# succinctlabs/kzg-rs

Hardware: NVIDIA B200
Metric: blobs verified/sec (verify_blob_kzg_proof_batch) (higher is better)
Workload: dtype u32-limb modular integer (Fr 255-bit / Fp 381-bit) + SHA-256

## Files before the change

include/kzgb200.h:

```cpp
#ifndef KZGB200_H
#define KZGB200_H
#include <stddef.h>
#include <stdint.h>
#ifdef __cplusplus
extern "C" {
#endif

#define KZGB200_OK 0
#define KZGB200_BAD_ARGS 1
#define KZGB200_INTERNAL_ERROR 2
#define KZGB200_INVALID_LENGTH 3
#define KZGB200_INVALID_SETUP 5

#define KZGB200_BYTES_PER_BLOB 131072
#define KZGB200_BYTES_PER_COMMITMENT 48
#define KZGB200_BYTES_PER_PROOF 48
#define KZGB200_BYTES_PER_FIELD_ELEMENT 32
#define KZGB200_PARTIAL_BYTES 352

typedef struct kzgb200_ctx kzgb200_ctx;

int kzgb200_create(kzgb200_ctx** out, int device, const uint8_t* g2_points, size_t g2_points_len);
void kzgb200_destroy(kzgb200_ctx* ctx);
const char* kzgb200_last_error(const kzgb200_ctx* ctx);

int kzgb200_verify_kzg_proof(kzgb200_ctx* ctx, const uint8_t* commitment48, const uint8_t* z32, const uint8_t* y32,
                             const uint8_t* proof48, int* ok);

int kzgb200_verify_blob_kzg_proof(kzgb200_ctx* ctx, const uint8_t* blob, const uint8_t* commitment48,
                                  const uint8_t* proof48, int* ok, uint8_t* z_out, uint8_t* y_out);

int kzgb200_verify_blob_kzg_proof_batch(kzgb200_ctx* ctx, const uint8_t* blobs, size_t n_blobs,
                                        const uint8_t* commitments, size_t n_commitments,
                                        const uint8_t* proofs, size_t n_proofs, int* ok,
                                        uint8_t* z_out, uint8_t* y_out);
int kzgb200_verify_blob_kzg_proof_batch_device(kzgb200_ctx* ctx, const uint8_t* d_blobs, const uint8_t* d_commitments,
                                               const uint8_t* d_proofs, size_t n, int* ok,
                                               uint8_t* d_z_out, uint8_t* d_y_out);

int kzgb200_verify_kzg_proof_many(kzgb200_ctx* ctx, const uint8_t* commitments, const uint8_t* zs, const uint8_t* ys,
                                  const uint8_t* proofs, size_t m, uint8_t* verdicts);

int kzgb200_verify_kzg_proof_batch(kzgb200_ctx* ctx, const uint8_t* commitments104, const uint8_t* zs32, const uint8_t* ys32,
                                   const uint8_t* proofs104, size_t n, int* ok);

int kzgb200_verify_blob_kzg_proof_batch_each(kzgb200_ctx* ctx, const uint8_t* blobs, const uint8_t* commitments, const uint8_t* proofs,
                                             size_t n, uint8_t* verdicts, uint8_t* z_out, uint8_t* y_out);

int kzgb200_compute_challenge(kzgb200_ctx* ctx, const uint8_t* blob, const uint8_t* commitment48, uint8_t* z_out32);
int kzgb200_evaluate_polynomial_in_evaluation_form(kzgb200_ctx* ctx, const uint8_t* blob, const uint8_t* z32, uint8_t* y_out32);

typedef struct kzgb200_group kzgb200_group;
int kzgb200_group_create(kzgb200_group** out, const int* device_ids, int n_devices, const uint8_t* g2_points, size_t g2_points_len,
                         size_t max_blobs_per_device);
int kzgb200_group_join(kzgb200_group** out, const char* session, int rank, int world, int device, const uint8_t* g2_points,
                       size_t g2_points_len, size_t max_blobs_per_rank);
void kzgb200_group_destroy(kzgb200_group* g);
int kzgb200_group_size(const kzgb200_group* g);
int kzgb200_group_local_members(const kzgb200_group* g);
kzgb200_ctx* kzgb200_group_context(kzgb200_group* g, int local_index);
const char* kzgb200_group_last_error(const kzgb200_group* g);
int kzgb200_group_uses_peer_stores(const kzgb200_group* g, int local_index);
int kzgb200_group_verify_blob_kzg_proof_batch(kzgb200_group* g, const uint8_t* blobs, size_t n_blobs, const uint8_t* commitments,
                                              size_t n_commitments, const uint8_t* proofs, size_t n_proofs, int* ok, uint8_t* z_out,
                                              uint8_t* y_out);
int kzgb200_group_verify_shards(kzgb200_group* g, const uint8_t* const* blobs, const uint8_t* const* commitments,
                                const uint8_t* const* proofs, const size_t* n_local, int device_pointers, int* ok,
                                uint8_t* const* z_out, uint8_t* const* y_out);
int kzgb200_group_last_partials(kzgb200_group* g, uint8_t* out, size_t n_ranks);
int kzgb200_group_host_protocol_test(const char* session, int rank, int world, const uint8_t* commitments, const uint8_t* zy,
                                     const uint8_t* proofs, size_t n_local, size_t chunk, uint8_t* digest_out32);

#define KZGB200_TRANSCRIPT_EXACT 0
#define KZGB200_TRANSCRIPT_TREE 1
#define KZGB200_TRANSCRIPT_EXACT_DEVICE 2
int kzgb200_set_transcript_mode(kzgb200_ctx* ctx, int mode);
int kzgb200_last_r(kzgb200_ctx* ctx, uint8_t* r_out32);
int kzgb200_host_sha256(const uint8_t* msg, size_t len, uint8_t* out32, int force_portable);

int kzgb200_last_partial(kzgb200_ctx* ctx, uint8_t* out352);

int kzgb200_harness_generate(kzgb200_ctx* ctx, uint64_t seed, size_t n, int degree, const uint8_t* tau_powers48,
                             uint8_t* d_blobs, uint8_t* d_commitments, uint8_t* d_proofs);
int kzgb200_load_g1_lagrange(kzgb200_ctx* ctx, const uint8_t* g1_lagrange, size_t n_points);
int kzgb200_blob_to_kzg_commitment_batch(kzgb200_ctx* ctx, const uint8_t* d_blobs, size_t n, uint8_t* d_commitments_out);
int kzgb200_compute_blob_kzg_proof_batch(kzgb200_ctx* ctx, const uint8_t* d_blobs, const uint8_t* d_commitments, size_t n,
                                         uint8_t* d_proofs_out);

int kzgb200_load_cell_setup(kzgb200_ctx* ctx, const uint8_t* g1_monomial48, size_t n_points, const uint8_t* g2_tau64_96);
int kzgb200_verify_cell_kzg_proof_batch(kzgb200_ctx* ctx, const uint8_t* commitments, const uint64_t* cell_indices, const uint8_t* cells,
                                        const uint8_t* proofs, size_t n, int* ok);
int kzgb200_verify_cell_kzg_proof_batch_device(kzgb200_ctx* ctx, const uint8_t* d_commitments, const uint64_t* d_cell_indices,
                                               const uint8_t* d_cells, const uint8_t* d_proofs, size_t n, int* ok);
int kzgb200_compute_cells(kzgb200_ctx* ctx, const uint8_t* blob, uint8_t* cells_out);
int kzgb200_compute_cells_batch_device(kzgb200_ctx* ctx, const uint8_t* d_blobs, size_t n, uint8_t* d_cells);
int kzgb200_harness_generate_cells(kzgb200_ctx* ctx, uint64_t seed, size_t n_blobs, int degree, const uint8_t* tau_powers48,
                                   uint8_t* d_cells, uint8_t* d_commitments, uint8_t* d_proofs);

int kzgb200_load_cell_proof_setup(kzgb200_ctx* ctx, const uint8_t* g1_lagrange48, size_t n_points);
int kzgb200_cell_proof_monomial(kzgb200_ctx* ctx, uint8_t* out48, size_t n_points);
int kzgb200_compute_cells_and_kzg_proofs(kzgb200_ctx* ctx, const uint8_t* blob, uint8_t* cells_out, uint8_t* proofs_out);
int kzgb200_compute_cells_and_kzg_proofs_batch_device(kzgb200_ctx* ctx, const uint8_t* d_blobs, size_t n, uint8_t* d_cells, uint8_t* d_proofs);
int kzgb200_recover_cells_and_kzg_proofs(kzgb200_ctx* ctx, const uint64_t* cell_indices, const uint8_t* cells, size_t n_cells,
                                         uint8_t* cells_out, uint8_t* proofs_out);
int kzgb200_recover_cells_and_kzg_proofs_batch_device(kzgb200_ctx* ctx, const uint64_t* cell_indices, size_t n_cells, const uint8_t* d_cells,
                                                      size_t n_blobs, uint8_t* d_cells_out, uint8_t* d_proofs_out);

int kzgb200_set_profiling(kzgb200_ctx* ctx, int on);
int kzgb200_set_slab_tail(kzgb200_ctx* ctx, int on);
int kzgb200_get_phase_ms(kzgb200_ctx* ctx, float* out8);
int kzgb200_debug_final_ticks(kzgb200_ctx* ctx, long long* out14);
int kzgb200_debug_engine_selftest(kzgb200_ctx* ctx, uint32_t seed, int rounds, uint32_t* mismatches32, int* n_programs);
void* kzgb200_stream(kzgb200_ctx* ctx);

typedef struct kzgb200_pipeline kzgb200_pipeline;
int kzgb200_pipeline_create(kzgb200_pipeline** out, int device, const uint8_t* g2_points, size_t g2_points_len, int depth);
void kzgb200_pipeline_destroy(kzgb200_pipeline* p);
int kzgb200_pipeline_depth(const kzgb200_pipeline* p);
kzgb200_ctx* kzgb200_pipeline_context(kzgb200_pipeline* p, int slot);
int kzgb200_pipeline_submit(kzgb200_pipeline* p, const uint8_t* blobs, size_t n_blobs, const uint8_t* commitments,
                            size_t n_commitments, const uint8_t* proofs, size_t n_proofs, uint8_t* z_out, uint8_t* y_out,
                            uint64_t* ticket);
int kzgb200_pipeline_submit_device(kzgb200_pipeline* p, const uint8_t* d_blobs, const uint8_t* d_commitments,
                                   const uint8_t* d_proofs, size_t n, uint8_t* d_z_out, uint8_t* d_y_out, uint64_t* ticket);
int kzgb200_pipeline_wait(kzgb200_pipeline* p, uint64_t ticket, int* ok);

void* kzgb200_alloc_pinned(size_t bytes);
void kzgb200_free_pinned(void* p);

#ifdef __cplusplus
}
#endif
#endif
```

kzg_rs_b200/csrc/common.cuh:

```cuda
#pragma once
#include <cuda_runtime.h>
#include "sha256.cuh"
#include "verify.cuh"
#include "vliw.cuh"
#include "vliw29.cuh"
#include "glv.cuh"

namespace kzgb200 {

constexpr int kFieldElementsPerBlob = 4096;
constexpr int kBytesPerBlob = 4096 * 32;
constexpr uint32_t kErrBlob = 1, kErrCommitment = 2, kErrProof = 4, kErrScalar = 8;
struct ZY { Fr z, y; };

struct DeviceTables {
    Fr twiddle[2048];
    Fr twiddle_po[128][32];
    PairingTables pairing;
    vliw29::LineCoeffs29 lines29[2][kMillerSteps];
    G1Affine gen_table[64][15];
    uint32_t setup_ok;
};

#ifndef KSHA_THREADS
#define KSHA_THREADS 32
#endif
constexpr int kShaThreads = KSHA_THREADS;
constexpr int kEvalThreads = 128;
constexpr int kLeavesPerThread = kFieldElementsPerBlob / kEvalThreads;
constexpr int kTreeGroup = 16;
constexpr int kTreeMid = 32;
constexpr int kWindows = 16, kBuckets = 256, kMsmSets = 3, kDigitRows = 4 * kWindows;
constexpr int kMinSlice = 8, kMsmRows = kMsmSets * 2 * kWindows;
constexpr int kWinLanes = kBuckets;
constexpr int kWinSmemBytes = kWinLanes * 144;
constexpr int kCombineThreads = 544;
constexpr int kCombineSmemBytes = 48 * 1024;
constexpr int kFinalThreads = 64;
constexpr int kPairThreads = 768;
constexpr int kManyThreads = 512, kManyGroups = 28;
constexpr int kManyCtasPerSm = 1;
constexpr int kManyWarps = 4;
constexpr int kHarnessMaxDegree = 16;
constexpr int kLagWindows = 32, kLagEntries = 255;
constexpr int kCellsPerExtBlob = 128, kFieldElementsPerCell = 64, kBytesPerCell = 2048;
constexpr int kCellNttThreads = 512;
constexpr int kCellNttSmemBytes = kFieldElementsPerBlob * 32;
constexpr int kCellAggSlices = 16;
constexpr int kCellHarnessMaxDegree = 192;

__device__ __forceinline__ Fr load_fe_be(const uint4* p) {
    uint4 hi = __ldg(p), lo = __ldg(p + 1);
    Fr f;
    f.l[7] = sha_bswap(hi.x); f.l[6] = sha_bswap(hi.y); f.l[5] = sha_bswap(hi.z); f.l[4] = sha_bswap(hi.w);
    f.l[3] = sha_bswap(lo.x); f.l[2] = sha_bswap(lo.y); f.l[1] = sha_bswap(lo.z); f.l[0] = sha_bswap(lo.w);
    return f;
}
__device__ __forceinline__ Fr ldg_fr(const Fr* p) {
    const uint4* q = reinterpret_cast<const uint4*>(p);
    uint4 a = __ldg(q), b = __ldg(q + 1);
    Fr f;
    f.l[0] = a.x; f.l[1] = a.y; f.l[2] = a.z; f.l[3] = a.w; f.l[4] = b.x; f.l[5] = b.y; f.l[6] = b.z; f.l[7] = b.w;
    return f;
}

struct Partial {
    G1 a, b;
    Fr ry;
    uint32_t err;
    uint32_t pad[7];
};

struct FinalSmem {
    G1 sm[kFinalThreads];
    unsigned char pad[20 * 1024];
};
struct PairSmem {
    f29::F29 regs[vliw29::kTotalRegs];
    vliw29::SharedTables stab;
};
struct FinalPts { G1Affine pts[2]; uint32_t go; };

constexpr int kManyStride = vliw::kTotalRegsThr * 12 + 1;
constexpr int kManySmemBytes = kManyGroups * kManyStride * 4 + (int)sizeof(vliw::SharedTables) + vliw::kNumSharedRegs * (int)sizeof(Fp) +
                               kManyGroups * (2 * (int)sizeof(G1Affine) + 2) + 64;
struct CellTables {
    Fr w4096[2048], w4096_inv[2048];
    Fr coset[4096];
    Fr shift64[kCellsPerExtBlob];
    Fr shift_inv[kCellsPerExtBlob];
    Fr w64_inv[kFieldElementsPerCell / 2];
    Fr omega8192, inv64;
    G1Affine tau_tab[kFieldElementsPerCell][4];
    LineCoeffs tau64_lines[kMillerSteps];
    vliw29::LineCoeffs29 lines29[kMillerSteps];
    uint32_t ok;
};
constexpr int kFk20Bases = kFieldElementsPerCell * kCellsPerExtBlob;
constexpr int kFk20Windows = 16, kFk20Entries = 255;
constexpr size_t kFk20TablePoints = (size_t)kFk20Bases * kFk20Windows * kFk20Entries;
constexpr int kExtElements = 2 * kFieldElementsPerBlob;
struct ProofTables {
    Fr w8192[kFieldElementsPerBlob], w8192_inv[kFieldElementsPerBlob];
    Fr pow7[kExtElements];
    Fr pow7_inv[kFieldElementsPerBlob];
    Fr s7_64;
};
__global__ void setup_tables_kernel(DeviceTables* T, const uint8_t* g2_points);
__global__ void setup_lines29_kernel(DeviceTables* T);
constexpr int kChallengeSlabs = 8;
void launch_challenge(int stages, cudaStream_t st, const uint8_t* blobs, const uint8_t* commitments, int n, Fr* z_mont, ZY* zy, Fr* zpow,
                      const uint8_t* slab_flags = nullptr);
__global__ void eval_kernel(const uint8_t* __restrict__ blobs, int n, const Fr* __restrict__ zpow, const DeviceTables* __restrict__ T,
                            ZY* __restrict__ zy, uint32_t* __restrict__ status);
__global__ void g1_decompress_kernel(const uint8_t* __restrict__ commitments, const uint8_t* __restrict__ proofs, int n, G1Affine* __restrict__ C,
                                     G1Affine* __restrict__ P, uint32_t* __restrict__ status, bool with_subgroup_check);
__global__ void g1_subgroup_kernel(const G1Affine* __restrict__ C, const G1Affine* __restrict__ P, int n, uint32_t* __restrict__ status);
__global__ void transcript_schedule_kernel(const uint8_t* __restrict__ commitments, const ZY* __restrict__ zy, const uint8_t* __restrict__ proofs,
                                           uint64_t n, uint32_t* __restrict__ wk, uint64_t first_blk, uint64_t blk_count);
__global__ void transcript_chain_kernel(const uint32_t* __restrict__ wk_all, uint64_t n, Fr* __restrict__ r_mont, uint32_t* __restrict__ state,
                                        uint64_t first_blk, uint64_t blk_count);
__global__ void transcript_words_kernel(const uint8_t* __restrict__ commitments, const ZY* __restrict__ zy, const uint8_t* __restrict__ proofs,
                                        uint64_t first_entry, uint64_t entry_count, uint32_t* __restrict__ words);
__global__ void transcript_tree_leaf_words_kernel(const uint32_t* __restrict__ words, uint64_t n, uint32_t* __restrict__ digests,
                                                  uint64_t first_group, uint64_t group_count);
__global__ void r_from_digest_kernel(const uint32_t* __restrict__ digest, Fr* __restrict__ r_mont);
__global__ void z_setup_kernel(const uint8_t* __restrict__ z_be32, int n, Fr* __restrict__ z_mont, ZY* __restrict__ zy, Fr* __restrict__ zpow,
                               uint32_t* __restrict__ status);
__global__ void import_parsed_kernel(const uint8_t* __restrict__ c104, const uint8_t* __restrict__ p104, const uint8_t* __restrict__ z32,
                                     const uint8_t* __restrict__ y32, int n, G1Affine* __restrict__ C, G1Affine* __restrict__ P,
                                     uint8_t* __restrict__ c48, uint8_t* __restrict__ p48, Fr* __restrict__ z_mont, ZY* __restrict__ zy);
__global__ void msm_scalars_kernel(const Fr* __restrict__ z_mont, const ZY* __restrict__ zy, const Fr* __restrict__ r_mont, uint64_t offset, int n,
                                   uint8_t* __restrict__ digits, Fr* __restrict__ ry);
__global__ void msm_sort_kernel(const uint8_t* __restrict__ digits, int n, uint32_t* __restrict__ order, uint32_t* __restrict__ start);
void launch_msm_bucket(int ctas_per_sm, int n, int slice, cudaStream_t st, const G1Affine* C, const G1Affine* P, const uint32_t* order,
                       const uint32_t* start, G1* halfsum, G1* part);
void launch_msm_bucket_join(int lanes, int n, int slice, cudaStream_t st, const uint32_t* start, const G1* halfsum, const G1* part, G1* buckets);
__global__ void msm_window_kernel(const G1* __restrict__ buckets, G1* __restrict__ windows);
__global__ void msm_combine_kernel(const G1* __restrict__ windows, const Fr* __restrict__ ry, const uint32_t* __restrict__ status, int n,
                                   const DeviceTables* __restrict__ T, Partial* __restrict__ out, uint32_t* flag, uint32_t epoch);
__global__ void wait_flags_kernel(const uint32_t* flags, int count, uint32_t epoch, uint32_t* __restrict__ timed_out);
__global__ void batch_final_kernel(const Partial* __restrict__ parts, int nparts, const DeviceTables* __restrict__ T, uint32_t* __restrict__ result,
                                   FinalPts* __restrict__ out);
__global__ void single_final_kernel(const G1Affine* __restrict__ C, const G1Affine* __restrict__ P, const ZY* __restrict__ zy,
                                    const uint32_t* __restrict__ status, const DeviceTables* __restrict__ T, uint32_t* __restrict__ result,
                                    FinalPts* __restrict__ out);
__global__ void pairing_check_kernel(const FinalPts* __restrict__ in, const DeviceTables* __restrict__ T, const vliw29::LineCoeffs29* __restrict__ lines_b,
                                     uint32_t* __restrict__ result, long long* __restrict__ ticks);
__global__ void engine_selftest_kernel(uint32_t seed, int rounds, f29::F29* __restrict__ ref, uint32_t* __restrict__ mismatches);
inline void launch_batch_final(cudaStream_t st, const Partial* parts, int nparts, const DeviceTables* T, uint32_t* result, unsigned char* scratch512,
                               bool ticks, const vliw29::LineCoeffs29* lines_b = nullptr) {
    FinalPts* fp = reinterpret_cast<FinalPts*>(scratch512 + 256);
    batch_final_kernel<<<1, kFinalThreads, sizeof(FinalSmem), st>>>(parts, nparts, T, result, fp);
    pairing_check_kernel<<<1, kPairThreads, sizeof(PairSmem), st>>>(fp, T, lines_b, result, ticks ? reinterpret_cast<long long*>(scratch512 + 128) : nullptr);
}
__global__ void many_lhs_kernel(const uint8_t* __restrict__ z32, const uint8_t* __restrict__ y32, const G1Affine* __restrict__ C,
                                const G1Affine* __restrict__ P, size_t m, const DeviceTables* __restrict__ T, G1Affine* __restrict__ X,
                                uint32_t* __restrict__ status);
__global__ void many_lhs_zy_kernel(const ZY* __restrict__ zy, const G1Affine* __restrict__ C, const G1Affine* __restrict__ P, size_t m,
                                   const DeviceTables* __restrict__ T, G1Affine* __restrict__ X, const uint32_t* __restrict__ status);
__global__ void many_pairing_kernel(const G1Affine* __restrict__ X, const G1Affine* __restrict__ P, const uint32_t* __restrict__ status, size_t m,
                                    const DeviceTables* __restrict__ T, uint8_t* __restrict__ verdicts);
__global__ void many_pairing_warp_kernel(const G1Affine* __restrict__ X, const G1Affine* __restrict__ P, size_t m, const DeviceTables* __restrict__ T,
                                         uint8_t* __restrict__ verdicts);
__global__ void export_scalars_kernel(const ZY* __restrict__ zy, int n, uint8_t* __restrict__ z_out, uint8_t* __restrict__ y_out);
__global__ void r_to_raw_kernel(const Fr* __restrict__ r_mont, ZY* __restrict__ out);
__global__ void status_or_kernel(const uint32_t* __restrict__ status, int n, uint32_t* __restrict__ out);
__global__ void harness_parse_points_kernel(const uint8_t* bytes, int n, G1Affine* out, uint32_t* bad);
__global__ void harness_blob_kernel(uint64_t seed, int n, int D, const DeviceTables* __restrict__ T, uint8_t* __restrict__ blobs);
__global__ void harness_commit_kernel(uint64_t seed, int n, int D, const G1Affine* __restrict__ M, const Fr* __restrict__ z_mont,
                                      uint8_t* __restrict__ out, int want_proof);
__global__ void lag_parse_kernel(const uint8_t* __restrict__ bytes, G1Affine* __restrict__ out, uint32_t* __restrict__ bad);
__global__ void lag_table_kernel(const G1Affine* __restrict__ L, G1* __restrict__ table);
__global__ void blob_scalars_kernel(const uint8_t* __restrict__ blobs, int n, Fr* __restrict__ scalars, uint32_t* __restrict__ status);
__global__ void quotient_kernel(const uint8_t* __restrict__ blobs, int n, const Fr* __restrict__ z_mont, const ZY* __restrict__ zy,
                                const DeviceTables* __restrict__ T, Fr* __restrict__ scalars);
__global__ void lag_msm_kernel(const Fr* __restrict__ scalars, int n, const G1* __restrict__ table, uint8_t* __restrict__ out48);
__global__ void cell_setup_kernel(CellTables* T, const uint8_t* __restrict__ g2_tau64);
__global__ void cell_setup_points_kernel(CellTables* T, const uint8_t* __restrict__ g1_monomial48);
__global__ void cell_setup_lines29_kernel(CellTables* T);
__global__ void compute_cells_kernel(const uint8_t* __restrict__ blobs, int n, const CellTables* __restrict__ T, uint8_t* __restrict__ cells,
                                     uint32_t* __restrict__ status);
__global__ void compute_cells_coeffs_kernel(const uint8_t* __restrict__ blobs, int n, const CellTables* __restrict__ T, uint8_t* __restrict__ cells,
                                            uint32_t* __restrict__ status, Fr* __restrict__ coeffs);
__global__ void proof_setup_kernel(ProofTables* P);
__global__ void mono_load_kernel(const uint8_t* __restrict__ lag48, G1* __restrict__ a, uint32_t* __restrict__ bad);
__global__ void mono_level_kernel(G1* __restrict__ a, int len, const CellTables* __restrict__ T);
__global__ void mono_finish_kernel(const G1* __restrict__ a, const CellTables* __restrict__ T, G1Affine* __restrict__ mono, uint32_t* __restrict__ bad);
__global__ void mono_compress_kernel(const G1Affine* __restrict__ mono, int n, uint8_t* __restrict__ out48);
__global__ void fk20_w_kernel(const G1Affine* __restrict__ mono, const CellTables* __restrict__ T, G1Affine* __restrict__ W);
__global__ void fk20_table_kernel(const G1Affine* __restrict__ W, G1Affine* __restrict__ tab);
__global__ void fk20_scalars_kernel(const Fr* __restrict__ coeffs, const CellTables* __restrict__ T, Fr* __restrict__ U);
__global__ void fk20_products_kernel(const Fr* __restrict__ U, const G1Affine* __restrict__ tab, G1* __restrict__ V);
__global__ void fk20_proofs_kernel(const G1* __restrict__ V, const CellTables* __restrict__ T, uint8_t* __restrict__ proofs);
__global__ void recover_z_kernel(const uint32_t* __restrict__ missing, int n_missing, const CellTables* __restrict__ T, const ProofTables* __restrict__ P,
                                 Fr* __restrict__ zvals);
__global__ void recover_load_kernel(const uint8_t* __restrict__ cells, int n_cells, const int* __restrict__ pos, const Fr* __restrict__ zvals, int nb,
                                    Fr* __restrict__ A, uint32_t* __restrict__ status);
__global__ void recover_ntt_inv_kernel(Fr* __restrict__ A, const CellTables* __restrict__ T);
__global__ void recover_ntt_div_kernel(Fr* __restrict__ A, const CellTables* __restrict__ T, const Fr* __restrict__ zvals);
__global__ void recover_mid_kernel(Fr* __restrict__ A, const ProofTables* __restrict__ P, int nb);
__global__ void recover_final_kernel(const Fr* __restrict__ A, const ProofTables* __restrict__ P, int nb, Fr* __restrict__ coeffs);
__global__ void recover_blob_kernel(const Fr* __restrict__ coeffs, const CellTables* __restrict__ T, uint8_t* __restrict__ blobs);
__global__ void cell_points_kernel(const uint8_t* __restrict__ bytes, int count, G1Affine* __restrict__ out, uint32_t* __restrict__ status, uint32_t flag);
__global__ void cell_check_kernel(const uint8_t* __restrict__ cells, int n, uint32_t* __restrict__ status);
__global__ void cell_scalars_kernel(const uint32_t* __restrict__ meta, int n, const G1Affine* __restrict__ U, const uint32_t* __restrict__ ustatus,
                                    const CellTables* __restrict__ T, Fr* __restrict__ z_mont, ZY* __restrict__ zy, G1Affine* __restrict__ C,
                                    uint32_t* __restrict__ status);
__global__ void cell_rpow_kernel(const Fr* __restrict__ r_mont, int n, Fr* __restrict__ rk);
__global__ void cell_agg_kernel(const uint8_t* __restrict__ cells, const uint32_t* __restrict__ meta, int n, const Fr* __restrict__ rk, Fr* __restrict__ agg);
__global__ void cell_interp_kernel(const Fr* __restrict__ agg, const uint32_t* __restrict__ meta, int n, const CellTables* __restrict__ T,
                                   Fr* __restrict__ coeffs);
__global__ void cell_rli_kernel(const Fr* __restrict__ coeffs, const CellTables* __restrict__ T, Partial* __restrict__ out);
__global__ void cell_harness_terms_kernel(uint64_t seed, int n, int D, const G1Affine* __restrict__ M, G1* __restrict__ terms);
__global__ void cell_harness_sums_kernel(int n, const G1* __restrict__ terms, G1* __restrict__ sums);
__global__ void cell_harness_points_kernel(int n, const G1* __restrict__ sums, const CellTables* __restrict__ T, uint8_t* __restrict__ commitments,
                                           uint8_t* __restrict__ proofs);
__global__ void cell_harness_eval_kernel(uint64_t seed, int n, int D, const CellTables* __restrict__ T, uint8_t* __restrict__ cells);

}
```

kzg_rs_b200/csrc/k_msm.cu:

```cuda
#include "common.cuh"
#include "coop.cuh"

namespace kzgb200 {

__global__ void __launch_bounds__(128) msm_scalars_kernel(const Fr* __restrict__ z_mont, const ZY* __restrict__ zy, const Fr* __restrict__ r_mont,
                                                          uint64_t offset, int n, uint8_t* __restrict__ digits ,
                                                          Fr* __restrict__ ry) {
    int i = blockIdx.x * blockDim.x + threadIdx.x;
    if (i >= n) return;
    uint64_t e = offset + (uint64_t)i;
    uint32_t ee[2] = {(uint32_t)e, (uint32_t)(e >> 32)};
    Fr ri = r_mont->pow(ee, 64);
    Fr ri_raw = ri.to_raw();
    Fr rz_raw = (ri * z_mont[i]).to_raw();
    ry[i] = ri * zy[i].y;
    uint32_t h[2][2][4];
    glv_split(ri_raw.l, h[0][0], h[0][1]);
    glv_split(rz_raw.l, h[1][0], h[1][1]);
    for (int kind = 0; kind < 2; kind++)
        for (int half = 0; half < 2; half++)
            for (int w = 0; w < kWindows; w++)
                digits[((size_t)(kind * 2 + half) * kWindows + w) * n + i] = (uint8_t)(h[kind][half][w >> 2] >> (8 * (w & 3)));
}
__global__ void __launch_bounds__(256) msm_sort_kernel(const uint8_t* __restrict__ digits, int n, uint32_t* __restrict__ order,
                                                       uint32_t* __restrict__ start) {
    __shared__ uint32_t hist[kBuckets], cursor[kBuckets];
    int row_id = blockIdx.x, t = threadIdx.x;
    const uint8_t* row = digits + (size_t)row_id * n;
    uint32_t* ord = order + (size_t)row_id * n;
    uint32_t* st = start + (size_t)row_id * (kBuckets + 1);
    hist[t] = 0;
    __syncthreads();
    for (int i = t; i < n; i += blockDim.x) atomicAdd(&hist[row[i]], 1u);
    __syncthreads();
    if (t == 0) {
        uint32_t acc = 0;
        for (int b = 0; b < kBuckets; b++) { cursor[b] = acc; st[b] = acc; acc += hist[b]; }
        st[kBuckets] = acc;
    }
    __syncthreads();
    for (int i = t; i < n; i += blockDim.x) ord[atomicAdd(&cursor[row[i]], 1u)] = (uint32_t)i;
}
__device__ __forceinline__ G1Affine ldg_point(const G1Affine* p) {
    const uint32_t* w = reinterpret_cast<const uint32_t*>(p);
    G1Affine a;
#pragma unroll
    for (int k = 0; k < 12; k++) { a.x.l[k] = __ldg(w + k); a.y.l[k] = __ldg(w + 12 + k); }
    a.inf = __ldg(w + 24);
    return a;
}
template <int kCtasPerSm>
__global__ void __launch_bounds__(128, kCtasPerSm) msm_bucket_kernel(const G1Affine* __restrict__ C, const G1Affine* __restrict__ P, int n,
                                                         const uint32_t* __restrict__ order, const uint32_t* __restrict__ start,
                                                         G1* __restrict__ halfsum , G1* __restrict__ part , int slice) {
    const int slices = (n + slice - 1) / slice;
    int tid = blockIdx.x * blockDim.x + threadIdx.x;
    if (tid >= kMsmRows * slices) return;
    int row = tid / slices, s = tid % slices;
    int w = row % kWindows, half = (row / kWindows) & 1, set = row / (2 * kWindows);
    const G1Affine* pts = set == 1 ? C : P;
    int digit_row = ((set == 2 ? 1 : 0) * 2 + half) * kWindows + w;
    const uint32_t* ord = order + (size_t)digit_row * n;
    const uint32_t* st = start + (size_t)digit_row * (kBuckets + 1);
    const uint32_t pos0 = (uint32_t)s * slice, end0 = pos0 + slice < (uint32_t)n ? pos0 + slice : (uint32_t)n;
    int b = 0;
#pragma unroll
    for (int step = 128; step >= 1; step >>= 1) if (b + step <= 255 && __ldg(st + b + step) <= pos0) b += step;
    uint32_t next_boundary = __ldg(st + b + 1);
    G1 acc = G1::identity();
    bool first = true;
    auto flush = [&](int bb) {
        uint32_t lo = __ldg(st + bb), hi = __ldg(st + bb + 1);
        if (bb != 0 && hi > lo) {
            if (lo >= pos0 && hi <= end0) halfsum[(size_t)row * kBuckets + bb] = acc;
            else part[((size_t)row * slices + s) * 2 + (first ? 0 : 1)] = acc;
        }
        first = false;
        acc = G1::identity();
    };
    const uint32_t beta_l[12] = KZG_FP_BETA_M;
    const Fp beta = fp_const(beta_l);
    G1Affine nxt = ldg_point(pts + __ldg(ord + pos0));
    for (uint32_t k = pos0; k < end0; k++) {
        G1Affine q = nxt;
        if (k + 1 < end0) nxt = ldg_point(pts + __ldg(ord + k + 1));
        while (k >= next_boundary) { flush(b); b++; next_boundary = __ldg(st + b + 1); }
        if (b != 0) {
            if (half && !q.inf) { q.x = q.x * beta; q.y = q.y.neg(); }
            acc = acc.add_mixed(q);
        }
    }
    flush(b);
}
void launch_msm_bucket(int ctas_per_sm, int n, int slice, cudaStream_t st, const G1Affine* C, const G1Affine* P, const uint32_t* order,
                       const uint32_t* start, G1* halfsum, G1* part) {
    const int slices = (n + slice - 1) / slice, grid = (kMsmRows * slices + 127) / 128;
    if (ctas_per_sm >= 4) msm_bucket_kernel<4><<<grid, 128, 0, st>>>(C, P, n, order, start, halfsum, part, slice);
    else if (ctas_per_sm == 3) msm_bucket_kernel<3><<<grid, 128, 0, st>>>(C, P, n, order, start, halfsum, part, slice);
    else msm_bucket_kernel<2><<<grid, 128, 0, st>>>(C, P, n, order, start, halfsum, part, slice);
}
__device__ __forceinline__ G1 shfl_xor_point(const G1& p, int m) {
    G1 r;
#pragma unroll
    for (int k = 0; k < 12; k++) {
        r.x.l[k] = __shfl_xor_sync(0xffffffffu, p.x.l[k], m);
        r.y.l[k] = __shfl_xor_sync(0xffffffffu, p.y.l[k], m);
        r.z.l[k] = __shfl_xor_sync(0xffffffffu, p.z.l[k], m);
    }
    return r;
}
template <int kJoinLanes>
__global__ void __launch_bounds__(128) msm_bucket_join_kernel(int n, const uint32_t* __restrict__ start, const G1* __restrict__ halfsum,
                                                              const G1* __restrict__ part, G1* __restrict__ buckets , int slice) {
    const int slices = (n + slice - 1) / slice;
    const uint32_t usl = (uint32_t)slice;
    const int gt = blockIdx.x * blockDim.x + threadIdx.x;
    const int tid = gt / kJoinLanes, j = gt % kJoinLanes;
    int b = tid % kBuckets, w = (tid / kBuckets) % kWindows, set = tid / (kBuckets * kWindows);
    G1 acc = G1::identity();
    if (b != 0) {
        uint32_t lo[2], s0[2], cnt[2];
        int row[2];
#pragma unroll
        for (int half = 0; half < 2; half++) {
            row[half] = (set * 2 + half) * kWindows + w;
            const int digit_row = ((set == 2 ? 1 : 0) * 2 + half) * kWindows + w;
            const uint32_t* st = start + (size_t)digit_row * (kBuckets + 1);
            const uint32_t l = __ldg(st + b), h = __ldg(st + b + 1);
            lo[half] = l; s0[half] = l / usl;
            cnt[half] = h > l ? (h - 1) / usl - l / usl + 1 : 0u;
        }
        const uint32_t total = cnt[0] + cnt[1];
        for (uint32_t i = (uint32_t)j; i < total; i += kJoinLanes) {
            const int half = i >= cnt[0] ? 1 : 0;
            const uint32_t k = half ? i - cnt[0] : i;
            const G1* src;
            if (cnt[half] == 1) src = halfsum + (size_t)row[half] * kBuckets + b;
            else {
                const uint32_t s = s0[half] + k;
                const int slot = (k == 0 && lo[half] != s0[half] * usl) ? 1 : 0;
                src = part + ((size_t)row[half] * slices + s) * 2 + slot;
            }
            acc = acc.add(*src);
        }
    }
#pragma unroll 1
    for (int m = 1; m < kJoinLanes; m <<= 1) {
        const G1 o = shfl_xor_point(acc, m);
        if ((j & (2 * m - 1)) == 0) acc = acc.add(o);
    }
    if (j == 0) buckets[tid] = acc;
}
void launch_msm_bucket_join(int lanes, int n, int slice, cudaStream_t st, const uint32_t* start, const G1* halfsum, const G1* part, G1* buckets) {
    const int items = kMsmSets * kWindows * kBuckets;
    if (lanes >= 8) msm_bucket_join_kernel<8><<<items * 8 / 128, 128, 0, st>>>(n, start, halfsum, part, buckets, slice);
    else if (lanes >= 4) msm_bucket_join_kernel<4><<<items * 4 / 128, 128, 0, st>>>(n, start, halfsum, part, buckets, slice);
    else msm_bucket_join_kernel<2><<<items * 2 / 128, 128, 0, st>>>(n, start, halfsum, part, buckets, slice);
}
static_assert(sizeof(G1) * kWinLanes == kWinSmemBytes, "keep kWinSmemBytes (common.cuh) in step with G1");
__global__ void __launch_bounds__(kWinLanes) msm_window_kernel(const G1* __restrict__ buckets, G1* __restrict__ windows ) {
    extern __shared__ __align__(16) unsigned char dyn_smem[];
    G1* sm = reinterpret_cast<G1*>(dyn_smem);
    const int l = threadIdx.x, sw = blockIdx.x;
    G1 mine = buckets[(size_t)sw * kBuckets + l];
#pragma unroll 1
    for (int d = 1; d < kWinLanes; d <<= 1) {
        sm[l] = mine;
        __syncthreads();
        if (l + d < kWinLanes) mine = mine.add(sm[l + d]);
        __syncthreads();
    }
    sm[l] = l ? mine : G1::identity();
    __syncthreads();
#pragma unroll 1
    for (int span = kWinLanes / 2; span >= 1; span >>= 1) {
        if (l < span) sm[l] = sm[l].add(sm[l + span]);
        __syncthreads();
    }
    if (l == 0) windows[sw] = sm[0];
}
constexpr int kCombEngine = 384, kCombHelpers = 160;
constexpr int kCombRegs = 96;
static_assert(kCombEngine + kCombHelpers == kCombineThreads, "thread split of msm_combine_kernel");
struct CombineSmem {
    f29::F29 regs[kMsmSets][kCombRegs];
    f29::F29 win[kMsmSets][kWindows][3];
    vliw29::SharedTables stab;
};
static_assert(sizeof(CombineSmem) <= kCombineSmemBytes, "keep kCombineSmemBytes (common.cuh) in step with CombineSmem");
__global__ void __launch_bounds__(kCombineThreads) msm_combine_kernel(const G1* __restrict__ windows, const Fr* __restrict__ ry, const uint32_t* __restrict__ status,
                                                                      int n, const DeviceTables* __restrict__ T, Partial* __restrict__ out, uint32_t* flag, uint32_t epoch) {
    extern __shared__ __align__(16) unsigned char dyn_smem[];
    CombineSmem& S = *reinterpret_cast<CombineSmem*>(dyn_smem);
    __shared__ uint32_t s_err, s_fallback;
    __shared__ uint8_t s_wid[kMsmSets][kWindows];
    __shared__ Fr s_ry[kCombHelpers];
    __shared__ CoopPoint cp[3];
    __shared__ G1 s_sg[64];
    const int t = threadIdx.x;
    if (t == 0) { s_err = 0; s_fallback = 0; }
    __syncthreads();
    if (t < kCombEngine) {
        auto ebar = [] { asm volatile("bar.sync 2, %0;" ::"n"(kCombEngine) : "memory"); };
        {
            const vliw29::Tables src = vliw29::default_tables();
            for (int i = t; i < vliw29::kNumMul * 4; i += kCombEngine) (&S.stab.mul[0][0])[i] = (&src.mul[0][0])[i];
            for (int i = t; i < vliw29::kNumLin * 4; i += kCombEngine) (&S.stab.lin[0][0])[i] = (&src.lin[0][0])[i];
            for (int i = t; i < vliw29::kNumTerm; i += kCombEngine) S.stab.term[i] = src.term[i];
            for (int i = t; i < vliw29::kNumLevel; i += kCombEngine) S.stab.level[i] = src.level[i];
            for (int i = t; i < vliw29::kNumPrograms; i += kCombEngine) S.stab.prog[i] = src.prog[i];
            if (t < 16) S.stab.p29[t] = t < 14 ? (int32_t)f29::p29_rt(t) : 0;
        }
        for (int i = t; i < kMsmSets * kWindows * 3; i += kCombEngine) {
            const int sw = i / 3, c = i % 3;
            const G1& w = windows[sw];
            S.win[sw / kWindows][sw % kWindows][c] = f29::from_fp(c == 0 ? w.x : (c == 1 ? w.y : w.z));
            if (c == 2) s_wid[sw / kWindows][sw % kWindows] = w.z.is_zero() ? 1 : 0;
        }
        for (int i = t; i < kMsmSets * kCombRegs; i += kCombEngine) S.regs[i / kCombRegs][i % kCombRegs] = f29::f29_zero();
        ebar();
        vliw29::Lanes L{t, kCombEngine, vliw29::Tables{S.stab.mul, S.stab.lin, S.stab.term, S.stab.level, S.stab.prog}, nullptr, S.stab.p29};
        L.groups = kMsmSets; L.gstride = kCombRegs; L.bar_id = 2; L.bar_threads = kCombEngine;
        f29::F29* regs = &S.regs[0][0];
        bool acc_id[kMsmSets] = {true, true, true};
        for (int w = kWindows - 1; w >= 0; w--) {
            if (w != kWindows - 1) for (int k = 0; k < 8; k++) vliw29::run(vliw29::kProg_g1_dbl, regs, L);
            for (int i = t; i < kMsmSets * 3 * 4; i += kCombEngine) {
                const int g = i / 12, c = (i / 4) % 3, q = i % 4;
                reinterpret_cast<uint4*>(&S.regs[g][3 + c])[q] = reinterpret_cast<const uint4*>(&S.win[g][w][c])[q];
                reinterpret_cast<uint4*>(&S.regs[g][90 + c])[q] = reinterpret_cast<const uint4*>(&S.regs[g][c])[q];
            }
            ebar();
            vliw29::run(vliw29::kProg_g1_add, regs, L);
            for (int i = t; i < kMsmSets * 3 * 4; i += kCombEngine) {
                const int g = i / 12, c = (i / 4) % 3, q = i % 4;
                if (s_wid[g][w]) reinterpret_cast<uint4*>(&S.regs[g][c])[q] = reinterpret_cast<const uint4*>(&S.regs[g][90 + c])[q];
                else if (acc_id[g]) reinterpret_cast<uint4*>(&S.regs[g][c])[q] = reinterpret_cast<const uint4*>(&S.regs[g][3 + c])[q];
            }
            if (t < kMsmSets && !s_wid[t][w] && !acc_id[t]) {
                if (vliw29::canonical_signed(S.regs[t][6]).is_zero()) s_fallback = 1;
            }
#pragma unroll
            for (int g = 0; g < kMsmSets; g++) acc_id[g] = acc_id[g] && s_wid[g][w];
            ebar();
        }
        if (t < kMsmSets * 3) {
            const int g = t / 3, c = t % 3;
            Fp v = Fp::from_raw(vliw29::canonical_signed(S.regs[g][c]));
            if (acc_id[g]) v = c == 2 ? Fp::zero() : Fp::one();
            cp[g].v[c] = v;
        }
        ebar();
        if (s_fallback && t < 32 * kMsmSets) {
            const int warp = t >> 5, lane = t & 31;
            CoopPoint* s = &cp[warp];
            __syncwarp();
            if (lane == 0) { s->v[0] = Fp::one(); s->v[1] = Fp::one(); s->v[2] = Fp::zero(); }
            __syncwarp();
            for (int w = kWindows - 1; w >= 0; w--) {
                if (w != kWindows - 1) for (int k = 0; k < 8; k++) coop_dbl(s, lane);
                coop_add(s, windows[warp * kWindows + w], lane);
            }
        }
    } else {
        const int h = t - kCombEngine;
        uint32_t e = 0;
        Fr acc_ry = Fr::zero();
        for (int i = h; i < n; i += kCombHelpers) { e |= status[i]; acc_ry = acc_ry.add_inl(ry[i]); }
        if (e) atomicOr(&s_err, e);
        s_ry[h] = acc_ry;
        asm volatile("bar.sync 1, %0;" ::"n"(kCombHelpers) : "memory");
        for (int span = 128; span >= 1; span >>= 1) {
            if (h < span && h + span < kCombHelpers) s_ry[h] = s_ry[h].add_inl(s_ry[h + span]);
            asm volatile("bar.sync 1, %0;" ::"n"(kCombHelpers) : "memory");
        }
        if (h < 64) {
            const Fr sv = s_ry[0];
            const uint32_t d = (sv.l[h / 8] >> (4 * (h % 8))) & 15u;
            s_sg[h] = d ? G1::from_affine(T->gen_table[h][d - 1]) : G1::identity();
        }
        asm volatile("bar.sync 1, %0;" ::"n"(kCombHelpers) : "memory");
        for (int span = 32; span >= 1; span >>= 1) {
            if (h < span) s_sg[h] = s_sg[h].add(s_sg[h + span]);
            asm volatile("bar.sync 1, %0;" ::"n"(kCombHelpers) : "memory");
        }
    }
    __syncthreads();
    const int warp = t >> 5, lane = t & 31;
    if (warp == 1) {
        G1 q = {cp[2].v[0], cp[2].v[1], cp[2].v[2]};
        coop_add(&cp[1], q, lane);
        coop_add(&cp[1], s_sg[0].neg(), lane);
    }
    if (warp < 2 && lane == 0) { G1 r = {cp[warp].v[0], cp[warp].v[1], cp[warp].v[2]}; if (warp == 1) out->b = r; else out->a = r; }
    if (t == 0) { out->ry = Fr::zero(); out->err = s_err; }
    if (flag) {
        __threadfence_system();
        __syncthreads();
        if (t == 0) { *reinterpret_cast<volatile uint32_t*>(flag) = epoch; __threadfence_system(); }
    }
}

}
```

kzg_rs_b200/csrc/kzgb200.cu:

```cuda
#include <new>
#include "runtime.cuh"

using namespace kzgb200;

namespace kzgb200 {
CopyPool::CopyPool(int nthreads) {
    for (int i = 0; i < nthreads; i++) threads.emplace_back([this] {
        uint64_t seen = 0;
        for (;;) {
            {
                std::unique_lock<std::mutex> lk(m);
                cv.wait(lk, [&] { return stop || gen != seen; });
                if (stop) return;
                seen = gen;
            }
            work(seen);
        }
    });
}
CopyPool::~CopyPool() {
    { std::lock_guard<std::mutex> lk(m); stop = true; }
    cv.notify_all();
    for (auto& t : threads) t.join();
}
bool CopyPool::grab(size_t* off, size_t* len) {
    std::lock_guard<std::mutex> lk(m);
    if (next >= pieces) return false;
    *off = next++ * piece;
    *len = bytes - *off < piece ? bytes - *off : piece;
    return true;
}
void CopyPool::work(uint64_t) {
    size_t off, len, mine = 0;
    while (grab(&off, &len)) { memcpy(dst + off, src + off, len); mine++; }
    if (mine) {
        std::lock_guard<std::mutex> lk(m);
        done += mine;
        if (done == pieces) cv_done.notify_all();
    }
}
void CopyPool::copy(uint8_t* d, const uint8_t* s, size_t n) {
    if (!n) return;
    {
        std::lock_guard<std::mutex> lk(m);
        dst = d; src = s; bytes = n; pieces = (n + piece - 1) / piece; next = 0; done = 0; gen++;
    }
    cv.notify_all();
    work(0);
    std::unique_lock<std::mutex> lk(m);
    cv_done.wait(lk, [&] { return done == pieces; });
}

void phase_begin(kzgb200_ctx* ctx, int ph, cudaStream_t st) { if (ctx->profile && !ctx->ph_started[ph]) { cudaEventRecord(ctx->ev_s[ph], st); ctx->ph_started[ph] = true; } }
void phase_end(kzgb200_ctx* ctx, int ph, cudaStream_t st) { if (ctx->profile) cudaEventRecord(ctx->ev_e[ph], st); }
void collect_phase_times(kzgb200_ctx* ctx) {
    if (!ctx->profile) return;
    cudaDeviceSynchronize();
    for (int i = 0; i < 8; i++) { ctx->phase_ms[i] = 0; if (ctx->ph_started[i]) cudaEventElapsedTime(&ctx->phase_ms[i], ctx->ev_s[i], ctx->ev_e[i]); }
}

int ensure_capacity(kzgb200_ctx* ctx, size_t n, bool need_blob_staging) {
    if (n > ctx->cap) {
        size_t c = n;
        CK(regrow(ctx->d_c, c * 48)); CK(regrow(ctx->d_p, c * 48));
        CK(regrow(ctx->d_z_mont, c)); CK(regrow(ctx->d_zy, c)); CK(regrow(ctx->d_zpow, c * 13));
        CK(regrow(ctx->d_C, c)); CK(regrow(ctx->d_P, c));
        CK(regrow(ctx->d_status, c)); CK(regrow(ctx->d_ry, c));
        CK(regrow(ctx->d_digits, c * kDigitRows)); CK(regrow(ctx->d_order, c * kDigitRows));
        CK(regrow(ctx->d_zout, c * 32)); CK(regrow(ctx->d_yout, c * 32));
        CK(regrow(ctx->d_part, (size_t)kMsmRows * ((c + kMinSlice - 1) / kMinSlice) * 2));
        ctx->cap = c;
    }
    if (n > ctx->host_cap) {
        for (uint8_t** p : {&ctx->h_zy, &ctx->h_c, &ctx->h_p}) { if (*p) cudaFreeHost(*p); *p = nullptr; }
        CK(cudaMallocHost(&ctx->h_zy, n * 64)); CK(cudaMallocHost(&ctx->h_c, n * 48)); CK(cudaMallocHost(&ctx->h_p, n * 48));
        ctx->host_cap = n;
    }
    if (need_blob_staging && n > ctx->blob_cap) {
        CK(regrow(ctx->d_blobs, n * (size_t)kBytesPerBlob));
        ctx->blob_cap = n;
    }
    return KZGB200_OK;
}

void hash_transcript_header(HostSha256* s, uint64_t n) {
    uint8_t hdr[32] = {'R', 'C', 'K', 'Z', 'G', 'B', 'A', 'T', 'C', 'H', '_', '_', '_', 'V', '1', '_', 0, 0, 0, 0, 0, 0, 0x10, 0x00};
    for (int i = 0; i < 8; i++) hdr[24 + i] = (uint8_t)(n >> (56 - 8 * i));
    host_sha256_init(s);
    host_sha256_update(s, hdr, 32);
}
void hash_entries(HostSha256* s, const uint8_t* c, const uint8_t* zy, const uint8_t* p, size_t lo, size_t cnt) {
    uint8_t buf[64 * 160];
    for (size_t i = lo; i < lo + cnt;) {
        size_t m = lo + cnt - i < 64 ? lo + cnt - i : 64;
        for (size_t k = 0; k < m; k++, i++) {
            uint8_t* e = buf + 160 * k;
            memcpy(e, c + 48 * i, 48);
            memcpy(e + 48, zy + 64 * i, 64);
            memcpy(e + 112, p + 48 * i, 48);
        }
        host_sha256_update(s, buf, 160 * m);
    }
}
static size_t tree_groups(size_t n) { return (n + kTreeGroup - 1) / kTreeGroup; }
static int transcript_begin(kzgb200_ctx* ctx, size_t n, const uint8_t* d_c, const uint8_t* d_p, const uint8_t* hc, const uint8_t* hp) {
    ctx->tr_n = n; ctx->tr_done = 0; ctx->tr_next_chunk = 0; ctx->tr_enqueued = 0; ctx->tr_active = true;
    ctx->tr_c = hc; ctx->tr_p = hp;
    const int mode = ctx->transcript_mode;
    size_t words = 0;
    if (mode == KZGB200_TRANSCRIPT_TREE) words = n * 40 + tree_groups(n) * 8;
    else if (mode == KZGB200_TRANSCRIPT_EXACT_DEVICE) words = ((32 + n * 160 + 9 + 63) / 64) * 64;
    if (words > ctx->wk_cap) { CK(regrow(ctx->d_wk, words)); ctx->wk_cap = words; }
    if (mode == KZGB200_TRANSCRIPT_EXACT_DEVICE) return KZGB200_OK;
    hash_transcript_header(&ctx->tr_sha, n);
    if (mode == KZGB200_TRANSCRIPT_EXACT && !hc) {
        CK(cudaStreamWaitEvent(ctx->s_d2h, ctx->ev_begin, 0));
        CK(cudaMemcpyAsync(ctx->h_c, d_c, n * 48, cudaMemcpyDeviceToHost, ctx->s_d2h));
        CK(cudaMemcpyAsync(ctx->h_p, d_p, n * 48, cudaMemcpyDeviceToHost, ctx->s_d2h));
        ctx->tr_c = ctx->h_c; ctx->tr_p = ctx->h_p;
    }
    return KZGB200_OK;
}
static int transcript_enqueue_chunk(kzgb200_ctx* ctx, int c, const uint8_t* d_c, const uint8_t* d_p) {
    const size_t n = ctx->tr_n, lo = ctx->chunks[c].lo, cnt = ctx->chunks[c].cnt, end = lo + cnt;
    switch (ctx->transcript_mode) {
    case KZGB200_TRANSCRIPT_EXACT:
        CK(cudaStreamWaitEvent(ctx->s_d2h, ctx->ev_zy[c], 0));
        CK(cudaMemcpyAsync(ctx->h_zy + lo * 64, ctx->d_zy + lo, cnt * 64, cudaMemcpyDeviceToHost, ctx->s_d2h));
        CK(cudaEventRecord(ctx->ev_zyh[c], ctx->s_d2h));
        break;
    case KZGB200_TRANSCRIPT_TREE: {
        size_t g0 = lo / kTreeGroup, g1 = end >= n ? tree_groups(n) : end / kTreeGroup;
        uint32_t *words = ctx->d_wk, *digests = ctx->d_wk + n * 40;
        transcript_words_kernel<<<(unsigned)((cnt * 40 + 255) / 256), 256, 0, ctx->stream>>>(d_c, ctx->d_zy, d_p, lo, cnt, words);
        if (g1 > g0) transcript_tree_leaf_words_kernel<<<(unsigned)((g1 - g0 + 63) / 64), 64, 0, ctx->stream>>>(words, (uint64_t)n, digests, g0, g1 - g0);
        CK(cudaEventRecord(ctx->ev_leaf, ctx->stream));
        CK(cudaStreamWaitEvent(ctx->s_d2h, ctx->ev_leaf, 0));
        if (g1 > g0) CK(cudaMemcpyAsync(ctx->h_zy + g0 * 32, digests + g0 * 8, (g1 - g0) * 32, cudaMemcpyDeviceToHost, ctx->s_d2h));
        CK(cudaEventRecord(ctx->ev_zyh[c], ctx->s_d2h));
        break;
    }
    default: {
        size_t nblk = (32 + n * 160 + 9 + 63) / 64;
        size_t ready = end >= n ? nblk : (32 + end * 160) / 64;
        if (ready > ctx->tr_done) {
            size_t k = ready - ctx->tr_done;
            transcript_schedule_kernel<<<(unsigned)((k + 127) / 128), 128, 0, ctx->stream>>>(d_c, ctx->d_zy, d_p, (uint64_t)n, ctx->d_wk, ctx->tr_done, k);
            transcript_chain_kernel<<<1, 32, 0, ctx->stream>>>(ctx->d_wk, (uint64_t)n, ctx->d_r, ctx->d_chain_state, ctx->tr_done, k);
            ctx->tr_done = ready;
        }
    }
    }
    CK(cudaGetLastError());
    ctx->tr_enqueued = c + 1;
    return KZGB200_OK;
}
int transcript_progress(kzgb200_ctx* ctx, bool block) {
    if (!ctx->tr_active) return KZGB200_OK;
    if (ctx->transcript_mode == KZGB200_TRANSCRIPT_EXACT_DEVICE) { ctx->tr_next_chunk = ctx->tr_enqueued; return KZGB200_OK; }
    while (ctx->tr_next_chunk < ctx->tr_enqueued) {
        int c = ctx->tr_next_chunk;
        if (block) CK(cudaEventSynchronize(ctx->ev_zyh[c]));
        else {
            cudaError_t e = cudaEventQuery(ctx->ev_zyh[c]);
            if (e == cudaErrorNotReady) break;
            CK(e);
        }
        size_t lo = ctx->chunks[c].lo, cnt = ctx->chunks[c].cnt, end = lo + cnt;
        if (ctx->chunk_sink) ctx->chunk_sink(ctx->chunk_sink_arg, c);
        else if (ctx->transcript_mode == KZGB200_TRANSCRIPT_EXACT) hash_entries(&ctx->tr_sha, ctx->tr_c, ctx->h_zy, ctx->tr_p, lo, cnt);
        else {
            size_t g0 = lo / kTreeGroup, g1 = end >= ctx->tr_n ? tree_groups(ctx->tr_n) : end / kTreeGroup;
            host_sha256_update(&ctx->tr_sha, ctx->h_zy + g0 * 32, (g1 - g0) * 32);
        }
        ctx->tr_next_chunk++;
    }
    return KZGB200_OK;
}
int upload_r_digest(kzgb200_ctx* ctx, const uint8_t digest[32]) {
    memcpy(ctx->h_digest, digest, 32);
    CK(cudaMemcpyAsync(ctx->d_digest, ctx->h_digest, 32, cudaMemcpyHostToDevice, ctx->stream));
    r_from_digest_kernel<<<1, 1, 0, ctx->stream>>>(ctx->d_digest, ctx->d_r);
    CK(cudaGetLastError());
    return KZGB200_OK;
}
int transcript_finish(kzgb200_ctx* ctx) {
    if (ctx->transcript_mode != KZGB200_TRANSCRIPT_EXACT_DEVICE) {
        uint8_t digest[32];
        host_sha256_final(&ctx->tr_sha, digest);
        int rc = upload_r_digest(ctx, digest);
        if (rc) return rc;
    }
    phase_end(ctx, kPhTranscript, ctx->stream);
    ctx->tr_active = false;
    return KZGB200_OK;
}

static int plan_chunks(kzgb200_ctx* ctx, size_t n, bool host_blobs, bool transcript) {
    int k = 0;
    if (host_blobs) {
        size_t chunk = (n + kMaxChunks - 1) / kMaxChunks;
        if (chunk < kMinChunk) chunk = kMinChunk;
        chunk = (chunk + kTreeGroup - 1) / kTreeGroup * kTreeGroup;
        for (size_t lo = 0; lo < n; lo += chunk) ctx->chunks[k++] = {lo, n - lo < chunk ? n - lo : chunk};
    } else if (!transcript || n < 2048 || ctx->transcript_mode == KZGB200_TRANSCRIPT_TREE) {
        ctx->chunks[k++] = {0, n};
    } else if (ctx->transcript_mode == KZGB200_TRANSCRIPT_EXACT_DEVICE) {
        size_t chunk = ((n + 7) / 8 + kTreeGroup - 1) / kTreeGroup * kTreeGroup;
        for (size_t lo = 0; lo < n; lo += chunk) ctx->chunks[k++] = {lo, n - lo < chunk ? n - lo : chunk};
    } else {
        size_t lo = 0, quarter = n / 4 / kTreeGroup * kTreeGroup;
        while (lo < n) {
            size_t rem = n - lo, take = k < 3 ? quarter : rem / 2 / kTreeGroup * kTreeGroup;
            if (take < 256) take = 256;
            if (rem - (take < rem ? take : rem) < 256 || k == kMaxChunks - 1) take = rem;
            ctx->chunks[k++] = {lo, take};
            lo += take;
        }
    }
    ctx->nchunks = k;
    return k;
}
static bool host_pointer_is_pinned(const void* p) {
    cudaPointerAttributes a;
    if (cudaPointerGetAttributes(&a, p) != cudaSuccess) { cudaGetLastError(); return false; }
    return a.type == cudaMemoryTypeHost;
}
static int h2d_blobs(kzgb200_ctx* ctx, uint8_t* d_dst, const uint8_t* h_src, size_t bytes, bool direct) {
    if (direct) { CK(cudaMemcpyAsync(d_dst, h_src, bytes, cudaMemcpyHostToDevice, ctx->s_copy)); return KZGB200_OK; }
    if (!ctx->pool) {
        unsigned hw = std::thread::hardware_concurrency();
        int t = hw >= 16 ? 7 : (hw >= 8 ? 3 : 1);
        if (const char* v = getenv("KZGB200_COPY_THREADS")) t = atoi(v) > 0 ? atoi(v) - 1 : 0;
        ctx->pool = new CopyPool(t);
        for (int b = 0; b < kzgb200_ctx::kStageBufs; b++) {
            CK(cudaMallocHost(&ctx->h_stage[b], kzgb200_ctx::kStageBytes));
            CK(cudaEventCreateWithFlags(&ctx->ev_stage[b], cudaEventDisableTiming));
        }
    }
    for (size_t off = 0; off < bytes; off += kzgb200_ctx::kStageBytes) {
        size_t len = bytes - off < kzgb200_ctx::kStageBytes ? bytes - off : kzgb200_ctx::kStageBytes;
        int b = ctx->stage_next;
        ctx->stage_next = (b + 1) % kzgb200_ctx::kStageBufs;
        CK(cudaEventSynchronize(ctx->ev_stage[b]));
        ctx->pool->copy(ctx->h_stage[b], h_src + off, len);
        CK(cudaMemcpyAsync(d_dst + off, ctx->h_stage[b], len, cudaMemcpyHostToDevice, ctx->s_copy));
        CK(cudaEventRecord(ctx->ev_stage[b], ctx->s_copy));
        int rc = transcript_progress(ctx, false);
        if (rc) return rc;
    }
    return KZGB200_OK;
}
int launch_phase1(kzgb200_ctx* ctx, const uint8_t* d_blobs, const uint8_t* h_blobs, const uint8_t* d_c, const uint8_t* d_p, size_t n,
                  bool transcript, bool defer_subgroup, const uint8_t* hc, const uint8_t* hp) {
    for (int i = 0; i < 8; i++) ctx->ph_started[i] = false;
    const int nchunks = plan_chunks(ctx, n, h_blobs != nullptr, transcript);
    ctx->tr_next_chunk = 0; ctx->tr_enqueued = 0; ctx->tr_active = false;
    CK(cudaStreamWaitEvent(ctx->stream, ctx->ev_parse, 0));
    CK(cudaMemsetAsync(ctx->d_status, 0, n * sizeof(uint32_t), ctx->stream));
    CK(cudaEventRecord(ctx->ev_begin, ctx->stream));
    if (transcript) { int rc = transcript_begin(ctx, n, d_c, d_p, hc, hp); if (rc) return rc; }
    bool direct = true, registered = false;
    if (h_blobs) {
        CK(cudaStreamWaitEvent(ctx->s_copy, ctx->ev_begin, 0));
        if (!host_pointer_is_pinned(h_blobs)) {
            direct = ctx->pageable_mode != 0;
            if (ctx->pageable_mode == 2) registered = cudaHostRegister(const_cast<uint8_t*>(h_blobs), n * (size_t)kBytesPerBlob, cudaHostRegisterDefault) == cudaSuccess;
            if (ctx->pageable_mode == 2 && !registered) cudaGetLastError();
        }
    }
    auto launch_parse = [&]() -> int {
        CK(cudaStreamWaitEvent(ctx->s_aux, ctx->ev_begin, 0));
        phase_begin(ctx, kPhParse, ctx->s_aux);
        g1_decompress_kernel<<<(2 * (int)n + 127) / 128, 128, 0, ctx->s_aux>>>(d_c, d_p, (int)n, ctx->d_C, ctx->d_P, ctx->d_status, ctx->parse_fused != 0);
        CK(cudaEventRecord(ctx->ev_decomp, ctx->s_aux));
        if (defer_subgroup && !ctx->parse_fused) { ctx->subgroup_pending = true; phase_end(ctx, kPhParse, ctx->s_aux); return KZGB200_OK; }
        if (!ctx->parse_fused) g1_subgroup_kernel<<<(2 * (int)n + 255) / 256, 256, 0, ctx->s_aux>>>(ctx->d_C, ctx->d_P, (int)n, ctx->d_status);
        phase_end(ctx, kPhParse, ctx->s_aux);
        CK(cudaEventRecord(ctx->ev_parse, ctx->s_aux));
        return KZGB200_OK;
    };
    if (ctx->parse_first) { int rc = launch_parse(); if (rc) return rc; }
    if (!h_blobs) {
        cudaStream_t s0 = ctx->s_work[0];
        CK(cudaStreamWaitEvent(s0, ctx->ev_begin, 0));
        phase_begin(ctx, kPhChallenge, s0);
        launch_challenge(ctx->sha_stages, s0, d_blobs, d_c, (int)n, ctx->d_z_mont, ctx->d_zy, ctx->d_zpow);
        phase_end(ctx, kPhChallenge, s0);
        CK(cudaEventRecord(ctx->ev_sha_all, s0));
        if (!ctx->parse_first) { int rc = launch_parse(); if (rc) return rc; }
        for (int c = 0; c < nchunks; c++) {
            size_t lo = ctx->chunks[c].lo, cnt = ctx->chunks[c].cnt;
            cudaStream_t sw = ctx->s_work[c & 1];
            if (c & 1) CK(cudaStreamWaitEvent(sw, ctx->ev_sha_all, 0));
            phase_begin(ctx, kPhEval, sw);
            eval_kernel<<<(int)cnt, kEvalThreads, 0, sw>>>(d_blobs + lo * kBytesPerBlob, (int)cnt, ctx->d_zpow + lo * 13, ctx->tables, ctx->d_zy + lo, ctx->d_status + lo);
            if (c == nchunks - 1) phase_end(ctx, kPhEval, sw);
            CK(cudaEventRecord(ctx->ev_zy[c], sw));
            CK(cudaStreamWaitEvent(ctx->stream, ctx->ev_zy[c], 0));
            if (transcript && c == nchunks - 1) phase_begin(ctx, kPhTranscript, ctx->stream);
            if (transcript) { int rc = transcript_enqueue_chunk(ctx, c, d_c, d_p); if (rc) return rc; }
        }
    } else {
        for (int c = 0; c < nchunks; c++) {
            size_t lo = ctx->chunks[c].lo, cnt = ctx->chunks[c].cnt;
            cudaStream_t sw = ctx->s_work[c % kWorkStreams];
            int rc = KZGB200_OK;
            const bool slabs = direct && ctx->slab_tail && nchunks > 1 && c == nchunks - 1 && cnt >= 64;
            uint8_t* slab_flags = ctx->d_scratch + 480;
            if (slabs) {
                const size_t sb = kBytesPerBlob / kChallengeSlabs;
                CK(cudaMemcpyAsync(slab_flags, ctx->h_flags, kChallengeSlabs, cudaMemcpyHostToDevice, ctx->s_copy));
                for (int q = 0; q < kChallengeSlabs; q++) {
                    CK(cudaMemcpy2DAsync(const_cast<uint8_t*>(d_blobs) + lo * kBytesPerBlob + q * sb, kBytesPerBlob, h_blobs + lo * kBytesPerBlob + q * sb,
                                         kBytesPerBlob, sb, cnt, cudaMemcpyHostToDevice, ctx->s_copy));
                    CK(cudaMemcpyAsync(slab_flags + q, ctx->h_flags + 8, 1, cudaMemcpyHostToDevice, ctx->s_copy));
                    if (q == 0) CK(cudaEventRecord(ctx->ev_h2d[c], ctx->s_copy));
                }
            } else {
                rc = h2d_blobs(ctx, const_cast<uint8_t*>(d_blobs) + lo * kBytesPerBlob, h_blobs + lo * kBytesPerBlob, cnt * (size_t)kBytesPerBlob, direct);
                if (rc) return rc;
                CK(cudaEventRecord(ctx->ev_h2d[c], ctx->s_copy));
            }
            CK(cudaStreamWaitEvent(sw, ctx->ev_h2d[c], 0));
            CK(cudaStreamWaitEvent(sw, ctx->ev_begin, 0));
            phase_begin(ctx, kPhChallenge, sw);
            launch_challenge(ctx->sha_stages, sw, d_blobs + lo * kBytesPerBlob, d_c + lo * 48, (int)cnt, ctx->d_z_mont + lo,
                             ctx->d_zy + lo, ctx->d_zpow + lo * 13, slabs ? slab_flags : nullptr);
            phase_end(ctx, kPhChallenge, sw);
            phase_begin(ctx, kPhEval, sw);
            eval_kernel<<<(int)cnt, kEvalThreads, 0, sw>>>(d_blobs + lo * kBytesPerBlob, (int)cnt, ctx->d_zpow + lo * 13, ctx->tables, ctx->d_zy + lo, ctx->d_status + lo);
            phase_end(ctx, kPhEval, sw);
            CK(cudaEventRecord(ctx->ev_zy[c], sw));
            CK(cudaStreamWaitEvent(ctx->stream, ctx->ev_zy[c], 0));
            if (c == 0 && !ctx->parse_first) { rc = launch_parse(); if (rc) return rc; }
            if (transcript && c == nchunks - 1) phase_begin(ctx, kPhTranscript, ctx->stream);
            if (transcript) { rc = transcript_enqueue_chunk(ctx, c, d_c, d_p); if (rc) return rc; }
        }
    }
    CK(cudaStreamWaitEvent(ctx->stream, ctx->ev_decomp, 0));
    CK(cudaGetLastError());
    if (registered) {
        CK(cudaStreamSynchronize(ctx->s_copy));
        cudaHostUnregister(const_cast<uint8_t*>(h_blobs));
    }
    ctx->cur_c = d_c; ctx->cur_p = d_p; ctx->cur_n = n;
    return KZGB200_OK;
}
static int msm_slice_len(const kzgb200_ctx* ctx, int n) {
    if (ctx->msm_slice > 0) return ctx->msm_slice < kMinSlice ? kMinSlice : ctx->msm_slice;
    const double wave = (double)ctx->msm_occ * ctx->num_sms * 128, work = (double)kMsmRows * n;
    int waves = (int)(work / 16.0 / wave + 0.5);
    if (waves < 1) waves = 1;
    int slice = (int)((work + waves * wave - 1) / (waves * wave));
    return slice < kMinSlice ? kMinSlice : slice;
}
int launch_lincomb(kzgb200_ctx* ctx, size_t offset, Partial* d_out, bool wait_subgroup, uint32_t* d_flag, uint32_t epoch) {
    int n = (int)ctx->cur_n;
    phase_begin(ctx, kPhLincomb, ctx->stream);
    msm_scalars_kernel<<<(n + 127) / 128, 128, 0, ctx->stream>>>(ctx->d_z_mont, ctx->d_zy, ctx->d_r, (uint64_t)offset, n, ctx->d_digits, ctx->d_ry);
    msm_sort_kernel<<<kDigitRows, 256, 0, ctx->stream>>>(ctx->d_digits, n, ctx->d_order, ctx->d_start);
    {
        const int slice = msm_slice_len(ctx, n);
        launch_msm_bucket(ctx->msm_occ, n, slice, ctx->stream, ctx->d_C, ctx->d_P, ctx->d_order, ctx->d_start, ctx->d_halfsum, ctx->d_part);
        launch_msm_bucket_join(ctx->msm_join, n, slice, ctx->stream, ctx->d_start, ctx->d_halfsum, ctx->d_part, ctx->d_buckets);
    }
    phase_end(ctx, kPhLincomb, ctx->stream);
    phase_begin(ctx, kPhReduce, ctx->stream);
    msm_window_kernel<<<kMsmSets * kWindows, kWinLanes, kWinSmemBytes, ctx->stream>>>(ctx->d_buckets, ctx->d_windows);
    if (ctx->subgroup_pending) {
        CK(cudaEventRecord(ctx->ev_bucket, ctx->stream));
        CK(cudaStreamWaitEvent(ctx->s_aux, ctx->ev_bucket, 0));
        if (ctx->profile) cudaEventRecord(ctx->ev_s[7], ctx->s_aux);
        g1_subgroup_kernel<<<ctx->num_sms - kTailSms, 256, kTailHogSmem, ctx->s_aux>>>(ctx->d_C, ctx->d_P, n, ctx->d_status);
        if (ctx->profile) { cudaEventRecord(ctx->ev_e[7], ctx->s_aux); ctx->ph_started[7] = true; }
        CK(cudaEventRecord(ctx->ev_parse, ctx->s_aux));
        ctx->subgroup_pending = false;
    }
    if (wait_subgroup) CK(cudaStreamWaitEvent(ctx->stream, ctx->ev_parse, 0));
    msm_combine_kernel<<<1, kCombineThreads, kCombineSmemBytes, ctx->stream>>>(ctx->d_windows, ctx->d_ry, ctx->d_status, n, ctx->tables, d_out, d_flag, epoch);
    phase_end(ctx, kPhReduce, ctx->stream);
    CK(cudaGetLastError());
    return KZGB200_OK;
}
int read_result(kzgb200_ctx* ctx, int* ok) {
    CK(cudaMemcpyAsync(ctx->h_result, ctx->d_result, 12, cudaMemcpyDeviceToHost, ctx->stream));
    CK(cudaStreamSynchronize(ctx->stream));
    if (ctx->h_result[0] == kBadArgs || ctx->h_result[2]) return KZGB200_BAD_ARGS;
    *ok = ctx->h_result[0] == kTrue ? 1 : 0;
    return KZGB200_OK;
}
int export_zy(kzgb200_ctx* ctx, size_t n, uint8_t* d_z, uint8_t* d_y) {
    if (!d_z && !d_y) return KZGB200_OK;
    export_scalars_kernel<<<((int)n + 127) / 128, 128, 0, ctx->stream>>>(ctx->d_zy, (int)n, d_z, d_y);
    CK(cudaGetLastError());
    return KZGB200_OK;
}
}

extern "C" int kzgb200_create(kzgb200_ctx** out, int device, const uint8_t* g2_points, size_t g2_points_len) {
    if (!out) return KZGB200_BAD_ARGS;
    *out = nullptr;
    if (!g2_points || g2_points_len != 192) return KZGB200_INVALID_SETUP;
    kzgb200_ctx* ctx = new (std::nothrow) kzgb200_ctx();
    if (!ctx) return KZGB200_INTERNAL_ERROR;
    ctx->device = device;
    DeviceGuard dev;
    auto fail = [&](int rc) { fprintf(stderr, "kzgb200_create: %s\n", ctx->err); kzgb200_destroy(ctx); return rc; };
    int rc = [&]() -> int {
        CK(cudaSetDevice(device));
        CK(cudaDeviceGetAttribute(&ctx->num_sms, cudaDevAttrMultiProcessorCount, device));
        int prio_lo = 0, prio_hi = 0;
        CK(cudaDeviceGetStreamPriorityRange(&prio_lo, &prio_hi));
        CK(cudaStreamCreateWithPriority(&ctx->stream, cudaStreamNonBlocking, prio_hi));
        { const char* v = getenv("KZGB200_PARSE_PRIO"); CK(cudaStreamCreateWithPriority(&ctx->s_aux, cudaStreamNonBlocking, v && atoi(v) ? prio_hi : prio_lo)); }
        if (const char* v = getenv("KZGB200_PARSE_FIRST")) ctx->parse_first = atoi(v);
        if (const char* v = getenv("KZGB200_PARSE_FUSED")) ctx->parse_fused = atoi(v);
        if (const char* v = getenv("KZGB200_DEFER_SUBGROUP")) ctx->defer_subgroup = atoi(v);
        if (const char* v = getenv("KZGB200_SHA_STAGES")) ctx->sha_stages = atoi(v);
        if (const char* v = getenv("KZGB200_SLAB_TAIL")) ctx->slab_tail = atoi(v) != 0;
        if (const char* v = getenv("KZGB200_PAGEABLE")) ctx->pageable_mode = !strcmp(v, "direct") ? 1 : (!strcmp(v, "register") ? 2 : 0);
        if (const char* v = getenv("KZGB200_MSM_SLICE")) ctx->msm_slice = atoi(v);
        if (const char* v = getenv("KZGB200_MSM_JOIN")) ctx->msm_join = atoi(v);
        if (const char* v = getenv("KZGB200_MSM_OCC")) { int o = atoi(v); if (o >= 2 && o <= 4) ctx->msm_occ = o; }
        if (const char* v = getenv("KZGB200_TRANSCRIPT")) ctx->transcript_mode = !strcmp(v, "tree") ? KZGB200_TRANSCRIPT_TREE : (!strcmp(v, "device") ? KZGB200_TRANSCRIPT_EXACT_DEVICE : KZGB200_TRANSCRIPT_EXACT);
        CK(cudaFuncSetAttribute(g1_subgroup_kernel, cudaFuncAttributeMaxDynamicSharedMemorySize, kTailHogSmem));
        CK(cudaStreamCreateWithFlags(&ctx->s_copy, cudaStreamNonBlocking));
        CK(cudaStreamCreateWithPriority(&ctx->s_d2h, cudaStreamNonBlocking, prio_hi));
        for (auto& w : ctx->s_work) CK(cudaStreamCreateWithPriority(&w, cudaStreamNonBlocking, prio_hi));
        for (cudaEvent_t* e : {&ctx->ev_begin, &ctx->ev_parse, &ctx->ev_decomp, &ctx->ev_bucket, &ctx->ev_sha_all, &ctx->ev_leaf})
            CK(cudaEventCreateWithFlags(e, cudaEventDisableTiming));
        for (auto& e : ctx->ev_h2d) CK(cudaEventCreateWithFlags(&e, cudaEventDisableTiming));
        for (auto& e : ctx->ev_zy) CK(cudaEventCreateWithFlags(&e, cudaEventDisableTiming));
        for (auto& e : ctx->ev_zyh) CK(cudaEventCreateWithFlags(&e, cudaEventDisableTiming));
        CK(cudaMalloc(&ctx->d_chain_state, 32));
        CK(cudaMalloc(&ctx->d_scratch, 512));
        CK(cudaMalloc(&ctx->d_digest, 32));
        CK(cudaFuncSetAttribute(batch_final_kernel, cudaFuncAttributeMaxDynamicSharedMemorySize, (int)sizeof(FinalSmem)));
        CK(cudaFuncSetAttribute(single_final_kernel, cudaFuncAttributeMaxDynamicSharedMemorySize, (int)sizeof(FinalSmem)));
        CK(cudaFuncSetAttribute(pairing_check_kernel, cudaFuncAttributeMaxDynamicSharedMemorySize, (int)sizeof(PairSmem)));
        CK(cudaFuncSetAttribute(msm_combine_kernel, cudaFuncAttributeMaxDynamicSharedMemorySize, kCombineSmemBytes));
        CK(cudaFuncSetAttribute(many_pairing_kernel, cudaFuncAttributeMaxDynamicSharedMemorySize, kManySmemBytes));
        CK(cudaFuncSetAttribute(many_pairing_warp_kernel, cudaFuncAttributeMaxDynamicSharedMemorySize, kManySmemBytes));
        CK(cudaMalloc(&ctx->tables, sizeof(DeviceTables)));
        CK(cudaMalloc(&ctx->d_r, sizeof(Fr)));
        CK(cudaMalloc(&ctx->d_partial, sizeof(Partial)));
        CK(cudaMalloc(&ctx->d_result, 16));
        CK(cudaMalloc(&ctx->d_start, kDigitRows * (kBuckets + 1) * sizeof(uint32_t)));
        CK(cudaMalloc(&ctx->d_buckets, kMsmSets * kWindows * kBuckets * sizeof(G1)));
        CK(cudaMalloc(&ctx->d_halfsum, kMsmRows * kBuckets * sizeof(G1)));
        CK(cudaMalloc(&ctx->d_windows, kMsmSets * kWindows * sizeof(G1)));
        CK(cudaMallocHost(&ctx->h_result, 16));
        CK(cudaMallocHost(&ctx->h_flags, 16));
        memset(ctx->h_flags, 0, 8); memset(ctx->h_flags + 8, 1, 8);
        CK(cudaMallocHost(&ctx->h_digest, 32));
        CK(cudaMallocHost(&ctx->h_partial, sizeof(Partial)));
        uint8_t* d_g2 = nullptr;
        CK(cudaMalloc(&d_g2, 192));
        CK(cudaMemcpyAsync(d_g2, g2_points, 192, cudaMemcpyHostToDevice, ctx->stream));
        setup_tables_kernel<<<(8192 + 4096) / 128, 128, 0, ctx->stream>>>(ctx->tables, d_g2);
        setup_lines29_kernel<<<(2 * kMillerSteps * 6 + 127) / 128, 128, 0, ctx->stream>>>(ctx->tables);
        CK(cudaGetLastError());
        uint32_t ok = 0;
        CK(cudaMemcpyAsync(&ok, &ctx->tables->setup_ok, 4, cudaMemcpyDeviceToHost, ctx->stream));
        CK(cudaStreamSynchronize(ctx->stream));
        cudaFree(d_g2);
        return ok ? KZGB200_OK : KZGB200_INVALID_SETUP;
    }();
    if (rc != KZGB200_OK) return fail(rc);
    *out = ctx;
    return KZGB200_OK;
}

static void cell_destroy(kzgb200_ctx* ctx);
extern "C" void kzgb200_destroy(kzgb200_ctx* ctx) {
    if (!ctx) return;
    DeviceGuard dev(ctx->device);
    cudaDeviceSynchronize();
    cell_destroy(ctx);
    delete ctx->pool;
    for (cudaStream_t st : {ctx->s_aux, ctx->s_copy, ctx->s_d2h, ctx->s_work[0], ctx->s_work[1], ctx->s_work[2], ctx->s_work[3]}) if (st) cudaStreamDestroy(st);
    for (cudaEvent_t e : {ctx->ev_begin, ctx->ev_parse, ctx->ev_decomp, ctx->ev_bucket, ctx->ev_sha_all, ctx->ev_leaf}) if (e) cudaEventDestroy(e);
    for (auto e : ctx->ev_h2d) if (e) cudaEventDestroy(e);
    for (auto e : ctx->ev_zy) if (e) cudaEventDestroy(e);
    for (auto e : ctx->ev_zyh) if (e) cudaEventDestroy(e);
    for (auto e : ctx->ev_s) if (e) cudaEventDestroy(e);
    for (auto e : ctx->ev_e) if (e) cudaEventDestroy(e);
    for (auto e : ctx->ev_stage) if (e) cudaEventDestroy(e);
    void* ptrs[] = {ctx->tables, ctx->d_blobs, ctx->d_c, ctx->d_p, ctx->d_z_mont, ctx->d_zy, ctx->d_C, ctx->d_P, ctx->d_status,
                    ctx->d_ry, ctx->d_r, ctx->d_partial, ctx->d_result, ctx->d_zout, ctx->d_yout, ctx->d_many, ctx->d_wk,
                    ctx->d_digits, ctx->d_order, ctx->d_start, ctx->d_buckets, ctx->d_halfsum, ctx->d_part, ctx->d_windows, ctx->d_lag_table, ctx->d_scalars, ctx->d_zpow,
                    ctx->d_chain_state, ctx->d_scratch, ctx->d_digest};
    for (void* p : ptrs) if (p) cudaFree(p);
    void* hptrs[] = {ctx->h_flags, ctx->h_result, ctx->h_digest, ctx->h_partial, ctx->h_zy, ctx->h_c, ctx->h_p, ctx->h_stage[0], ctx->h_stage[1], ctx->h_stage[2], ctx->h_stage[3]};
    for (void* p : hptrs) if (p) cudaFreeHost(p);
    if (ctx->stream) cudaStreamDestroy(ctx->stream);
    delete ctx;
}

extern "C" const char* kzgb200_last_error(const kzgb200_ctx* ctx) { return ctx ? ctx->err : "null context"; }

constexpr size_t kManyBytesPerTuple = 3 * sizeof(G1Affine) + 4 + 160 + 4;
static int launch_many_pairings(kzgb200_ctx* ctx, const G1Affine* X, const G1Affine* P, const uint32_t* status, size_t m, uint8_t* dv) {
    size_t nbatch = (m + kManyGroups - 1) / kManyGroups;
    const size_t slots = (size_t)ctx->num_sms * kManyCtasPerSm;
    unsigned grid = (unsigned)(nbatch < slots ? nbatch : slots);
    many_pairing_kernel<<<grid, kManyThreads, kManySmemBytes, ctx->stream>>>(X, P, status, m, ctx->tables, dv);
    size_t nw = (m + kManyWarps - 1) / kManyWarps;
    many_pairing_warp_kernel<<<(unsigned)(nw < (size_t)ctx->num_sms ? nw : (size_t)ctx->num_sms), 32 * kManyWarps, kManySmemBytes, ctx->stream>>>(X, P, m, ctx->tables, dv);
    CK(cudaGetLastError());
    return KZGB200_OK;
}
static int batch_locked(kzgb200_ctx* ctx, const uint8_t* d_blobs, const uint8_t* h_blobs, const uint8_t* d_c, const uint8_t* d_p, size_t n, int* ok,
                        uint8_t* d_z_out, uint8_t* d_y_out, const uint8_t* hc, const uint8_t* hp) {
    const bool defer = n >= 2 && ctx->defer_subgroup;
    int rc = launch_phase1(ctx, d_blobs, h_blobs, d_c, d_p, n, n >= 2, defer, hc, hp);
    if (rc) return rc;
    if ((rc = export_zy(ctx, n, d_z_out, d_y_out))) return rc;
    if (n == 1) {
        phase_begin(ctx, kPhFinal, ctx->stream);
        CK(cudaStreamWaitEvent(ctx->stream, ctx->ev_parse, 0));
        FinalPts* fp = reinterpret_cast<FinalPts*>(ctx->d_scratch + 256);
        single_final_kernel<<<1, kFinalThreads, sizeof(FinalSmem), ctx->stream>>>(ctx->d_C, ctx->d_P, ctx->d_zy, ctx->d_status, ctx->tables, ctx->d_result, fp);
        pairing_check_kernel<<<1, kPairThreads, sizeof(PairSmem), ctx->stream>>>(fp, ctx->tables, nullptr, ctx->d_result, nullptr);
    } else {
        if ((rc = transcript_progress(ctx, true))) return rc;
        if ((rc = transcript_finish(ctx))) return rc;
        if ((rc = launch_lincomb(ctx, 0, ctx->d_partial, !defer))) return rc;
        phase_begin(ctx, kPhFinal, ctx->stream);
        launch_batch_final(ctx->stream, ctx->d_partial, 1, ctx->tables, ctx->d_result, ctx->d_scratch, true);
    }
    phase_end(ctx, kPhFinal, ctx->stream);
    CK(cudaStreamWaitEvent(ctx->stream, ctx->ev_parse, 0));
    status_or_kernel<<<1, 256, 0, ctx->stream>>>(ctx->d_status, (int)n, ctx->d_result + 2);
    CK(cudaGetLastError());
    rc = read_result(ctx, ok);
    collect_phase_times(ctx);
    return rc;
}

extern "C" int kzgb200_verify_blob_kzg_proof_batch_device(kzgb200_ctx* ctx, const uint8_t* d_blobs, const uint8_t* d_commitments,
                                                          const uint8_t* d_proofs, size_t n, int* ok, uint8_t* d_z_out, uint8_t* d_y_out) {
    if (!ctx || !ok || n == 0 || n > 0x7fffffff / 2) return KZGB200_BAD_ARGS;
    std::lock_guard<std::mutex> g(ctx->lock);
    DeviceGuard dev(ctx->device);
    int rc = ensure_capacity(ctx, n, false);
    if (rc) return rc;
    return batch_locked(ctx, d_blobs, nullptr, d_commitments, d_proofs, n, ok, d_z_out, d_y_out, nullptr, nullptr);
}

extern "C" int kzgb200_verify_blob_kzg_proof_batch(kzgb200_ctx* ctx, const uint8_t* blobs, size_t n_blobs, const uint8_t* commitments,
                                                   size_t n_commitments, const uint8_t* proofs, size_t n_proofs, int* ok,
                                                   uint8_t* z_out, uint8_t* y_out) {
    if (!ctx || !ok) return KZGB200_BAD_ARGS;
    if (n_blobs == 0) { *ok = 1; return KZGB200_OK; }
    if (n_blobs == 1) {
        if (n_commitments < 1 || n_proofs < 1) return KZGB200_BAD_ARGS;
    } else {
        if (n_blobs != n_commitments) return KZGB200_INVALID_LENGTH;
        if (n_blobs != n_proofs) return KZGB200_INVALID_LENGTH;
    }
    if (n_blobs > 0x7fffffff / 2) return KZGB200_BAD_ARGS;
    std::lock_guard<std::mutex> g(ctx->lock);
    DeviceGuard dev(ctx->device);
    size_t n = n_blobs;
    int rc = ensure_capacity(ctx, n, true);
    if (rc) return rc;
    CK(cudaMemcpyAsync(ctx->d_c, commitments, n * 48, cudaMemcpyHostToDevice, ctx->stream));
    CK(cudaMemcpyAsync(ctx->d_p, proofs, n * 48, cudaMemcpyHostToDevice, ctx->stream));
    rc = batch_locked(ctx, ctx->d_blobs, blobs, ctx->d_c, ctx->d_p, n, ok, z_out ? ctx->d_zout : nullptr, y_out ? ctx->d_yout : nullptr, commitments, proofs);
    if (rc == KZGB200_OK) {
        if (z_out) CK(cudaMemcpyAsync(z_out, ctx->d_zout, n * 32, cudaMemcpyDeviceToHost, ctx->stream));
        if (y_out) CK(cudaMemcpyAsync(y_out, ctx->d_yout, n * 32, cudaMemcpyDeviceToHost, ctx->stream));
        CK(cudaStreamSynchronize(ctx->stream));
    }
    return rc;
}

extern "C" int kzgb200_verify_blob_kzg_proof(kzgb200_ctx* ctx, const uint8_t* blob, const uint8_t* commitment48, const uint8_t* proof48,
                                             int* ok, uint8_t* z_out, uint8_t* y_out) {
    return kzgb200_verify_blob_kzg_proof_batch(ctx, blob, 1, commitment48, 1, proof48, 1, ok, z_out, y_out);
}

extern "C" int kzgb200_verify_blob_kzg_proof_batch_each(kzgb200_ctx* ctx, const uint8_t* blobs, const uint8_t* commitments, const uint8_t* proofs,
                                                        size_t n, uint8_t* verdicts, uint8_t* z_out, uint8_t* y_out) {
    if (!ctx || (n && (!blobs || !commitments || !proofs || !verdicts)) || n > 0x7fffffff / 2) return KZGB200_BAD_ARGS;
    if (n == 0) return KZGB200_OK;
    std::lock_guard<std::mutex> g(ctx->lock);
    DeviceGuard dev(ctx->device);
    int rc = ensure_capacity(ctx, n, true);
    if (rc) return rc;
    CK(cudaMemcpyAsync(ctx->d_c, commitments, n * 48, cudaMemcpyHostToDevice, ctx->stream));
    CK(cudaMemcpyAsync(ctx->d_p, proofs, n * 48, cudaMemcpyHostToDevice, ctx->stream));
    if ((rc = launch_phase1(ctx, ctx->d_blobs, blobs, ctx->d_c, ctx->d_p, n, n >= 2, false, commitments, proofs))) return rc;
    if ((rc = export_zy(ctx, n, z_out ? ctx->d_zout : nullptr, y_out ? ctx->d_yout : nullptr))) return rc;
    int ok = 0;
    bool all_true = false;
    if (n >= 2) {
        if ((rc = transcript_progress(ctx, true))) return rc;
        if ((rc = transcript_finish(ctx))) return rc;
        if ((rc = launch_lincomb(ctx, 0, ctx->d_partial, true))) return rc;
        launch_batch_final(ctx->stream, ctx->d_partial, 1, ctx->tables, ctx->d_result, ctx->d_scratch, false);
        status_or_kernel<<<1, 256, 0, ctx->stream>>>(ctx->d_status, (int)n, ctx->d_result + 2);
        CK(cudaGetLastError());
        rc = read_result(ctx, &ok);
        if (rc != KZGB200_OK && rc != KZGB200_BAD_ARGS) return rc;
        all_true = rc == KZGB200_OK && ok == 1;
    }
    if (all_true) memset(verdicts, 1, n);
    else {
        CK(cudaStreamWaitEvent(ctx->stream, ctx->ev_parse, 0));
        if (n > ctx->many_cap) { CK(regrow(ctx->d_many, n * kManyBytesPerTuple)); ctx->many_cap = n; }
        G1Affine* X = reinterpret_cast<G1Affine*>(ctx->d_many);
        uint8_t* dv = ctx->d_many + n * sizeof(G1Affine);
        many_lhs_zy_kernel<<<(unsigned)((n + 127) / 128), 128, 0, ctx->stream>>>(ctx->d_zy, ctx->d_C, ctx->d_P, n, ctx->tables, X, ctx->d_status);
        if ((rc = launch_many_pairings(ctx, X, ctx->d_P, ctx->d_status, n, dv))) return rc;
        CK(cudaMemcpyAsync(verdicts, dv, n, cudaMemcpyDeviceToHost, ctx->stream));
    }
    if (z_out) CK(cudaMemcpyAsync(z_out, ctx->d_zout, n * 32, cudaMemcpyDeviceToHost, ctx->stream));
    if (y_out) CK(cudaMemcpyAsync(y_out, ctx->d_yout, n * 32, cudaMemcpyDeviceToHost, ctx->stream));
    CK(cudaStreamSynchronize(ctx->stream));
    return KZGB200_OK;
}

extern "C" int kzgb200_verify_kzg_proof_batch(kzgb200_ctx* ctx, const uint8_t* commitments104, const uint8_t* zs32, const uint8_t* ys32,
                                              const uint8_t* proofs104, size_t n, int* ok) {
    if (!ctx || !ok || (n && (!commitments104 || !zs32 || !ys32 || !proofs104)) || n > 0x7fffffff / 2) return KZGB200_BAD_ARGS;
    if (n == 0) { *ok = 1; return KZGB200_OK; }
    std::lock_guard<std::mutex> g(ctx->lock);
    DeviceGuard dev(ctx->device);
    int rc = ensure_capacity(ctx, n, false);
    if (rc) return rc;
    if (n > ctx->many_cap) { CK(regrow(ctx->d_many, n * kManyBytesPerTuple)); ctx->many_cap = n; }
    uint8_t *dc = ctx->d_many, *dp = dc + n * 104, *dz = dp + n * 104, *dy = dz + n * 32;
    for (int i = 0; i < 8; i++) ctx->ph_started[i] = false;
    CK(cudaStreamWaitEvent(ctx->stream, ctx->ev_parse, 0));
    CK(cudaMemcpyAsync(dc, commitments104, n * 104, cudaMemcpyHostToDevice, ctx->stream));
    CK(cudaMemcpyAsync(dp, proofs104, n * 104, cudaMemcpyHostToDevice, ctx->stream));
    CK(cudaMemcpyAsync(dz, zs32, n * 32, cudaMemcpyHostToDevice, ctx->stream));
    CK(cudaMemcpyAsync(dy, ys32, n * 32, cudaMemcpyHostToDevice, ctx->stream));
    CK(cudaMemsetAsync(ctx->d_status, 0, n * sizeof(uint32_t), ctx->stream));
    import_parsed_kernel<<<(unsigned)((2 * n + 127) / 128), 128, 0, ctx->stream>>>(dc, dp, dz, dy, (int)n, ctx->d_C, ctx->d_P, ctx->d_c, ctx->d_p, ctx->d_z_mont, ctx->d_zy);
    CK(cudaGetLastError());
    CK(cudaEventRecord(ctx->ev_begin, ctx->stream));
    ctx->chunks[0] = {0, n}; ctx->nchunks = 1;
    ctx->cur_c = ctx->d_c; ctx->cur_p = ctx->d_p; ctx->cur_n = n; ctx->subgroup_pending = false;
    if ((rc = transcript_begin(ctx, n, ctx->d_c, ctx->d_p, nullptr, nullptr))) return rc;
    CK(cudaEventRecord(ctx->ev_zy[0], ctx->stream));
    if ((rc = transcript_enqueue_chunk(ctx, 0, ctx->d_c, ctx->d_p))) return rc;
    if ((rc = transcript_progress(ctx, true))) return rc;
    if ((rc = transcript_finish(ctx))) return rc;
    if ((rc = launch_lincomb(ctx, 0, ctx->d_partial, false))) return rc;
    launch_batch_final(ctx->stream, ctx->d_partial, 1, ctx->tables, ctx->d_result, ctx->d_scratch, false);
    CK(cudaMemsetAsync(ctx->d_result + 2, 0, 4, ctx->stream));
    CK(cudaGetLastError());
    return read_result(ctx, ok);
}

extern "C" int kzgb200_compute_challenge(kzgb200_ctx* ctx, const uint8_t* blob, const uint8_t* commitment48, uint8_t* z_out32) {
    if (!ctx || !blob || !commitment48 || !z_out32) return KZGB200_BAD_ARGS;
    std::lock_guard<std::mutex> g(ctx->lock);
    DeviceGuard dev(ctx->device);
    int rc = ensure_capacity(ctx, 1, true);
    if (rc) return rc;
    CK(cudaStreamWaitEvent(ctx->stream, ctx->ev_parse, 0));
    CK(cudaMemcpyAsync(ctx->d_blobs, blob, kBytesPerBlob, cudaMemcpyHostToDevice, ctx->stream));
    CK(cudaMemcpyAsync(ctx->d_c, commitment48, 48, cudaMemcpyHostToDevice, ctx->stream));
    launch_challenge(ctx->sha_stages, ctx->stream, ctx->d_blobs, ctx->d_c, 1, ctx->d_z_mont, ctx->d_zy, ctx->d_zpow);
    export_scalars_kernel<<<1, 32, 0, ctx->stream>>>(ctx->d_zy, 1, ctx->d_zout, nullptr);
    CK(cudaGetLastError());
    CK(cudaMemcpyAsync(z_out32, ctx->d_zout, 32, cudaMemcpyDeviceToHost, ctx->stream));
    CK(cudaStreamSynchronize(ctx->stream));
    return KZGB200_OK;
}
extern "C" int kzgb200_evaluate_polynomial_in_evaluation_form(kzgb200_ctx* ctx, const uint8_t* blob, const uint8_t* z32, uint8_t* y_out32) {
    if (!ctx || !blob || !z32 || !y_out32) return KZGB200_BAD_ARGS;
    std::lock_guard<std::mutex> g(ctx->lock);
    DeviceGuard dev(ctx->device);
    int rc = ensure_capacity(ctx, 1, true);
    if (rc) return rc;
    CK(cudaStreamWaitEvent(ctx->stream, ctx->ev_parse, 0));
    CK(cudaMemcpyAsync(ctx->d_blobs, blob, kBytesPerBlob, cudaMemcpyHostToDevice, ctx->stream));
    CK(cudaMemcpyAsync(ctx->d_zout, z32, 32, cudaMemcpyHostToDevice, ctx->stream));
    CK(cudaMemsetAsync(ctx->d_status, 0, 4, ctx->stream));
    z_setup_kernel<<<1, 32, 0, ctx->stream>>>(ctx->d_zout, 1, ctx->d_z_mont, ctx->d_zy, ctx->d_zpow, ctx->d_status);
    eval_kernel<<<1, kEvalThreads, 0, ctx->stream>>>(ctx->d_blobs, 1, ctx->d_zpow, ctx->tables, ctx->d_zy, ctx->d_status);
    export_scalars_kernel<<<1, 32, 0, ctx->stream>>>(ctx->d_zy, 1, nullptr, ctx->d_yout);
    CK(cudaGetLastError());
    CK(cudaMemcpyAsync(y_out32, ctx->d_yout, 32, cudaMemcpyDeviceToHost, ctx->stream));
    CK(cudaMemcpyAsync(ctx->h_result, ctx->d_status, 4, cudaMemcpyDeviceToHost, ctx->stream));
    CK(cudaStreamSynchronize(ctx->stream));
    return ctx->h_result[0] ? KZGB200_BAD_ARGS : KZGB200_OK;
}

extern "C" int kzgb200_verify_kzg_proof_many(kzgb200_ctx* ctx, const uint8_t* commitments, const uint8_t* zs, const uint8_t* ys,
                                             const uint8_t* proofs, size_t m, uint8_t* verdicts) {
    if (!ctx || (m && (!commitments || !zs || !ys || !proofs || !verdicts))) return KZGB200_BAD_ARGS;
    if (m == 0) return KZGB200_OK;
    std::lock_guard<std::mutex> g(ctx->lock);
    DeviceGuard dev(ctx->device);
    const size_t kChunk = (size_t)1 << 20, c = m < kChunk ? m : kChunk;
    if (c > ctx->many_cap) { CK(regrow(ctx->d_many, c * kManyBytesPerTuple)); ctx->many_cap = c; }
    G1Affine *dC = reinterpret_cast<G1Affine*>(ctx->d_many), *dP = dC + c, *dX = dP + c;
    uint32_t* dst = reinterpret_cast<uint32_t*>(dX + c);
    uint8_t *dc = reinterpret_cast<uint8_t*>(dst + c), *dp = dc + c * 48, *dz = dp + c * 48, *dy = dz + c * 32, *dv = dy + c * 32;
    CK(cudaStreamWaitEvent(ctx->stream, ctx->ev_parse, 0));
    for (int i = 0; i < 8; i++) ctx->ph_started[i] = false;
    for (size_t lo = 0; lo < m; lo += c) {
        size_t cnt = m - lo < c ? m - lo : c;
        CK(cudaMemcpyAsync(dc, commitments + lo * 48, cnt * 48, cudaMemcpyHostToDevice, ctx->stream));
        CK(cudaMemcpyAsync(dz, zs + lo * 32, cnt * 32, cudaMemcpyHostToDevice, ctx->stream));
        CK(cudaMemcpyAsync(dy, ys + lo * 32, cnt * 32, cudaMemcpyHostToDevice, ctx->stream));
        CK(cudaMemcpyAsync(dp, proofs + lo * 48, cnt * 48, cudaMemcpyHostToDevice, ctx->stream));
        CK(cudaMemsetAsync(dst, 0, cnt * 4, ctx->stream));
        phase_begin(ctx, kPhParse, ctx->stream);
        g1_decompress_kernel<<<(unsigned)((2 * cnt + 127) / 128), 128, 0, ctx->stream>>>(dc, dp, (int)cnt, dC, dP, dst, false);
        g1_subgroup_kernel<<<(unsigned)((2 * cnt + 255) / 256), 256, 0, ctx->stream>>>(dC, dP, (int)cnt, dst);
        phase_end(ctx, kPhParse, ctx->stream);
        phase_begin(ctx, kPhLincomb, ctx->stream);
        many_lhs_kernel<<<(unsigned)((cnt + 127) / 128), 128, 0, ctx->stream>>>(dz, dy, dC, dP, cnt, ctx->tables, dX, dst);
        phase_end(ctx, kPhLincomb, ctx->stream);
        phase_begin(ctx, kPhFinal, ctx->stream);
        { int rc = launch_many_pairings(ctx, dX, dP, dst, cnt, dv); if (rc) return rc; }
        phase_end(ctx, kPhFinal, ctx->stream);
        CK(cudaMemcpyAsync(verdicts + lo, dv, cnt, cudaMemcpyDeviceToHost, ctx->stream));
    }
    CK(cudaStreamSynchronize(ctx->stream));
    collect_phase_times(ctx);
    return KZGB200_OK;
}

extern "C" int kzgb200_verify_kzg_proof(kzgb200_ctx* ctx, const uint8_t* commitment48, const uint8_t* z32, const uint8_t* y32,
                                        const uint8_t* proof48, int* ok) {
    if (!ok) return KZGB200_BAD_ARGS;
    uint8_t v = 0;
    int rc = kzgb200_verify_kzg_proof_many(ctx, commitment48, z32, y32, proof48, 1, &v);
    if (rc) return rc;
    if (v == kBadArgs) return KZGB200_BAD_ARGS;
    *ok = v == kTrue;
    return KZGB200_OK;
}

extern "C" int kzgb200_host_sha256(const uint8_t* msg, size_t len, uint8_t* out32, int force_portable) {
    host_sha256_force_portable(force_portable);
    HostSha256 s;
    host_sha256_init(&s);
    host_sha256_update(&s, msg, len);
    host_sha256_final(&s, out32);
    int used = host_sha256_uses_shani();
    host_sha256_force_portable(0);
    return used;
}

extern "C" int kzgb200_harness_generate(kzgb200_ctx* ctx, uint64_t seed, size_t n, int degree, const uint8_t* tau_powers48,
                                        uint8_t* d_blobs, uint8_t* d_commitments, uint8_t* d_proofs) {
    if (!ctx || n == 0 || degree < 2 || degree > kHarnessMaxDegree || !tau_powers48) return KZGB200_BAD_ARGS;
    std::lock_guard<std::mutex> g(ctx->lock);
    DeviceGuard dev(ctx->device);
    int rc = ensure_capacity(ctx, n, false);
    if (rc) return rc;
    uint8_t* d_bytes = nullptr; G1Affine* d_M = nullptr; uint32_t* d_bad = nullptr; uint32_t bad = 0;
    CK(cudaMalloc(&d_bytes, degree * 48)); CK(cudaMalloc(&d_M, degree * sizeof(G1Affine))); CK(cudaMalloc(&d_bad, 4));
    CK(cudaMemsetAsync(d_bad, 0, 4, ctx->stream));
    CK(cudaMemcpyAsync(d_bytes, tau_powers48, degree * 48, cudaMemcpyHostToDevice, ctx->stream));
    harness_parse_points_kernel<<<1, 32, 0, ctx->stream>>>(d_bytes, degree, d_M, d_bad);
    int ni = (int)n;
    harness_blob_kernel<<<ni, 128, 0, ctx->stream>>>(seed, ni, degree, ctx->tables, d_blobs);
    harness_commit_kernel<<<(ni + 63) / 64, 64, 0, ctx->stream>>>(seed, ni, degree, d_M, nullptr, d_commitments, 0);
    launch_challenge(ctx->sha_stages, ctx->stream, d_blobs, d_commitments, ni, ctx->d_z_mont, ctx->d_zy, ctx->d_zpow);
    harness_commit_kernel<<<(ni + 63) / 64, 64, 0, ctx->stream>>>(seed, ni, degree, d_M, ctx->d_z_mont, d_proofs, 1);
    CK(cudaGetLastError());
    CK(cudaMemcpyAsync(&bad, d_bad, 4, cudaMemcpyDeviceToHost, ctx->stream));
    CK(cudaStreamSynchronize(ctx->stream));
    cudaFree(d_bytes); cudaFree(d_M); cudaFree(d_bad);
    return bad ? KZGB200_BAD_ARGS : KZGB200_OK;
}
extern "C" int kzgb200_set_transcript_mode(kzgb200_ctx* ctx, int mode) {
    if (!ctx || (mode != KZGB200_TRANSCRIPT_EXACT && mode != KZGB200_TRANSCRIPT_TREE && mode != KZGB200_TRANSCRIPT_EXACT_DEVICE)) return KZGB200_BAD_ARGS;
    std::lock_guard<std::mutex> g(ctx->lock);
    ctx->transcript_mode = mode;
    return KZGB200_OK;
}
extern "C" int kzgb200_last_r(kzgb200_ctx* ctx, uint8_t* r_out32) {
    if (!ctx || !r_out32) return KZGB200_BAD_ARGS;
    std::lock_guard<std::mutex> g(ctx->lock);
    DeviceGuard dev(ctx->device);
    ZY* tmp = reinterpret_cast<ZY*>(ctx->d_scratch);
    uint8_t* d_out = ctx->d_scratch + sizeof(ZY);
    r_to_raw_kernel<<<1, 1, 0, ctx->stream>>>(ctx->d_r, tmp);
    export_scalars_kernel<<<1, 1, 0, ctx->stream>>>(tmp, 1, d_out, nullptr);
    CK(cudaGetLastError());
    CK(cudaMemcpyAsync(r_out32, d_out, 32, cudaMemcpyDeviceToHost, ctx->stream));
    CK(cudaStreamSynchronize(ctx->stream));
    return KZGB200_OK;
}
extern "C" int kzgb200_last_partial(kzgb200_ctx* ctx, uint8_t* out352) {
    if (!ctx || !out352) return KZGB200_BAD_ARGS;
    std::lock_guard<std::mutex> g(ctx->lock);
    DeviceGuard dev(ctx->device);
    CK(cudaMemcpyAsync(out352, ctx->d_partial, sizeof(Partial), cudaMemcpyDeviceToHost, ctx->stream));
    CK(cudaStreamSynchronize(ctx->stream));
    return KZGB200_OK;
}
extern "C" int kzgb200_set_profiling(kzgb200_ctx* ctx, int on) {
    if (!ctx) return KZGB200_BAD_ARGS;
    std::lock_guard<std::mutex> g(ctx->lock);
    DeviceGuard dev(ctx->device);
    if (on) { for (auto& e : ctx->ev_s) if (!e) CK(cudaEventCreate(&e)); for (auto& e : ctx->ev_e) if (!e) CK(cudaEventCreate(&e)); }
    ctx->profile = on != 0;
    return KZGB200_OK;
}
extern "C" int kzgb200_get_phase_ms(kzgb200_ctx* ctx, float* out7) {
    if (!ctx || !out7) return KZGB200_BAD_ARGS;
    for (int i = 0; i < 8; i++) out7[i] = ctx->phase_ms[i];
    return KZGB200_OK;
}
extern "C" int kzgb200_load_g1_lagrange(kzgb200_ctx* ctx, const uint8_t* g1_lagrange, size_t n_points) {
    if (!ctx || !g1_lagrange || n_points != (size_t)kFieldElementsPerBlob) return KZGB200_INVALID_SETUP;
    std::lock_guard<std::mutex> g(ctx->lock);
    DeviceGuard dev(ctx->device);
    if (ctx->d_lag_table) return KZGB200_OK;
    uint8_t* d_bytes = nullptr; G1Affine* d_L = nullptr; uint32_t* d_bad = nullptr; uint32_t bad = 0;
    CK(cudaMalloc(&d_bytes, n_points * 48)); CK(cudaMalloc(&d_L, n_points * sizeof(G1Affine))); CK(cudaMalloc(&d_bad, 4));
    CK(cudaMalloc(&ctx->d_lag_table, (size_t)kFieldElementsPerBlob * kLagWindows * kLagEntries * sizeof(G1)));
    CK(cudaMemsetAsync(d_bad, 0, 4, ctx->stream));
    CK(cudaMemcpyAsync(d_bytes, g1_lagrange, n_points * 48, cudaMemcpyHostToDevice, ctx->stream));
    lag_parse_kernel<<<(kFieldElementsPerBlob + 127) / 128, 128, 0, ctx->stream>>>(d_bytes, d_L, d_bad);
    lag_table_kernel<<<(kFieldElementsPerBlob * kLagWindows + 127) / 128, 128, 0, ctx->stream>>>(d_L, ctx->d_lag_table);
    CK(cudaGetLastError());
    CK(cudaMemcpyAsync(&bad, d_bad, 4, cudaMemcpyDeviceToHost, ctx->stream));
    CK(cudaStreamSynchronize(ctx->stream));
    cudaFree(d_bytes); cudaFree(d_L); cudaFree(d_bad);
    if (bad) { cudaFree(ctx->d_lag_table); ctx->d_lag_table = nullptr; return KZGB200_INVALID_SETUP; }
    return KZGB200_OK;
}
static int commit_or_prove(kzgb200_ctx* ctx, const uint8_t* d_blobs, const uint8_t* d_commitments, size_t n, uint8_t* d_out, int want_proof) {
    if (!ctx->d_lag_table) return KZGB200_INVALID_SETUP;
    const size_t kChunk = 1024;
    int rc = ensure_capacity(ctx, n < kChunk ? n : kChunk, false);
    if (rc) return rc;
    if (!ctx->d_scalars) CK(cudaMalloc(&ctx->d_scalars, kChunk * (size_t)kFieldElementsPerBlob * sizeof(Fr)));
    uint32_t any_bad = 0;
    for (size_t lo = 0; lo < n; lo += kChunk) {
        int cnt = (int)(n - lo < kChunk ? n - lo : kChunk);
        const uint8_t* blobs = d_blobs + lo * kBytesPerBlob;
        CK(cudaMemsetAsync(ctx->d_status, 0, cnt * sizeof(uint32_t), ctx->stream));
        if (!want_proof) {
            blob_scalars_kernel<<<(unsigned)(((size_t)cnt * kFieldElementsPerBlob + 127) / 128), 128, 0, ctx->stream>>>(blobs, cnt, ctx->d_scalars, ctx->d_status);
        } else {
            launch_challenge(ctx->sha_stages, ctx->stream, blobs, d_commitments + lo * 48, cnt, ctx->d_z_mont, ctx->d_zy, ctx->d_zpow);
            eval_kernel<<<cnt, kEvalThreads, 0, ctx->stream>>>(blobs, cnt, ctx->d_zpow, ctx->tables, ctx->d_zy, ctx->d_status);
            quotient_kernel<<<cnt, kEvalThreads, 0, ctx->stream>>>(blobs, cnt, ctx->d_z_mont, ctx->d_zy, ctx->tables, ctx->d_scalars);
        }
        lag_msm_kernel<<<cnt, 256, 0, ctx->stream>>>(ctx->d_scalars, cnt, ctx->d_lag_table, d_out + lo * 48);
        status_or_kernel<<<1, 256, 0, ctx->stream>>>(ctx->d_status, cnt, ctx->d_result);
        CK(cudaGetLastError());
        CK(cudaMemcpyAsync(ctx->h_result, ctx->d_result, 4, cudaMemcpyDeviceToHost, ctx->stream));
        CK(cudaStreamSynchronize(ctx->stream));
        any_bad |= ctx->h_result[0];
    }
    return any_bad ? KZGB200_BAD_ARGS : KZGB200_OK;
}
extern "C" int kzgb200_blob_to_kzg_commitment_batch(kzgb200_ctx* ctx, const uint8_t* d_blobs, size_t n, uint8_t* d_commitments_out) {
    if (!ctx || !d_blobs || !d_commitments_out || n == 0) return KZGB200_BAD_ARGS;
    std::lock_guard<std::mutex> g(ctx->lock);
    DeviceGuard dev(ctx->device);
    return commit_or_prove(ctx, d_blobs, nullptr, n, d_commitments_out, 0);
}
extern "C" int kzgb200_compute_blob_kzg_proof_batch(kzgb200_ctx* ctx, const uint8_t* d_blobs, const uint8_t* d_commitments, size_t n,
                                                    uint8_t* d_proofs_out) {
    if (!ctx || !d_blobs || !d_commitments || !d_proofs_out || n == 0) return KZGB200_BAD_ARGS;
    std::lock_guard<std::mutex> g(ctx->lock);
    DeviceGuard dev(ctx->device);
    return commit_or_prove(ctx, d_blobs, d_commitments, n, d_proofs_out, 1);
}
extern "C" int kzgb200_debug_final_ticks(kzgb200_ctx* ctx, long long* out14) {
    if (!ctx || !out14) return KZGB200_BAD_ARGS;
    std::lock_guard<std::mutex> g(ctx->lock);
    DeviceGuard dev(ctx->device);
    CK(cudaMemcpy(out14, ctx->d_scratch + 128, 112, cudaMemcpyDeviceToHost));
    return KZGB200_OK;
}
extern "C" int kzgb200_set_slab_tail(kzgb200_ctx* ctx, int on) {
    if (!ctx) return KZGB200_BAD_ARGS;
    std::lock_guard<std::mutex> g(ctx->lock);
    ctx->slab_tail = on != 0;
    return KZGB200_OK;
}
extern "C" int kzgb200_debug_engine_selftest(kzgb200_ctx* ctx, uint32_t seed, int rounds, uint32_t* mismatches32, int* n_programs) {
    if (!ctx || !mismatches32 || !n_programs || rounds < 1) return KZGB200_BAD_ARGS;
    std::lock_guard<std::mutex> g(ctx->lock);
    DeviceGuard dev(ctx->device);
    f29::F29* d_ref = nullptr; uint32_t* d_mis = nullptr;
    CK(cudaMalloc(&d_ref, sizeof(f29::F29) * vliw29::kTotalRegs));
    CK(cudaMalloc(&d_mis, 32 * sizeof(uint32_t)));
    CK(cudaMemsetAsync(d_mis, 0, 32 * sizeof(uint32_t), ctx->stream));
    CK(cudaFuncSetAttribute(engine_selftest_kernel, cudaFuncAttributeMaxDynamicSharedMemorySize, (int)sizeof(PairSmem)));
    engine_selftest_kernel<<<1, kPairThreads, sizeof(PairSmem), ctx->stream>>>(seed, rounds, d_ref, d_mis);
    CK(cudaGetLastError());
    CK(cudaMemcpyAsync(mismatches32, d_mis, 32 * sizeof(uint32_t), cudaMemcpyDeviceToHost, ctx->stream));
    CK(cudaStreamSynchronize(ctx->stream));
    cudaFree(d_ref); cudaFree(d_mis);
    *n_programs = vliw29::kNumPrograms;
    static_assert(vliw29::kNumPrograms <= 32, "mismatch array");
    return KZGB200_OK;
}
extern "C" void* kzgb200_stream(kzgb200_ctx* ctx) { return ctx ? (void*)ctx->stream : nullptr; }

extern "C" void* kzgb200_alloc_pinned(size_t bytes) {
    void* p = nullptr;
    return cudaMallocHost(&p, bytes) == cudaSuccess ? p : nullptr;
}
extern "C" void kzgb200_free_pinned(void* p) { if (p) cudaFreeHost(p); }

static void proof_destroy(CellCtx* c) {
    void* d[] = {c->ptables, c->d_mono, c->d_fk_tab, c->d_pcoef, c->d_fkU, c->d_A, c->d_V, c->d_rblobs, c->d_rin, c->d_pout, c->d_pos, c->d_missing, c->d_z};
    for (void* p : d) if (p) cudaFree(p);
    c->ptables = nullptr; c->d_mono = c->d_fk_tab = nullptr; c->d_pcoef = c->d_fkU = c->d_A = c->d_z = nullptr; c->d_V = nullptr;
    c->d_rblobs = c->d_rin = c->d_pout = nullptr; c->d_pos = nullptr; c->d_missing = nullptr; c->proof_cap = 0;
}
static void cell_destroy(kzgb200_ctx* ctx) {
    CellCtx* c = ctx->cells;
    if (!c) return;
    void* d[] = {c->tables, c->d_cells, c->d_p, c->d_uc, c->d_meta, c->d_ustatus, c->d_U, c->d_rk, c->d_agg, c->d_coeffs, c->d_part, c->d_ext};
    for (void* p : d) if (p) cudaFree(p);
    void* h[] = {c->h_meta, c->h_uc, c->h_c, c->h_cells, c->h_p, c->h_idx};
    for (void* p : h) if (p) cudaFreeHost(p);
    for (cudaEvent_t e : {c->ev_r, c->ev_rli}) if (e) cudaEventDestroy(e);
    proof_destroy(c);
    delete c;
    ctx->cells = nullptr;
}

extern "C" int kzgb200_load_cell_setup(kzgb200_ctx* ctx, const uint8_t* g1_monomial48, size_t n_points, const uint8_t* g2_tau64_96) {
    if (!ctx) return KZGB200_BAD_ARGS;
    if (!g1_monomial48 || n_points < (size_t)kFieldElementsPerCell || !g2_tau64_96) return KZGB200_INVALID_SETUP;
    std::lock_guard<std::mutex> g(ctx->lock);
    DeviceGuard dev(ctx->device);
    if (ctx->cells) return KZGB200_OK;
    CellCtx* c = new (std::nothrow) CellCtx();
    if (!c) return KZGB200_INTERNAL_ERROR;
    ctx->cells = c;
    uint8_t* d_bytes = nullptr;
    uint32_t ok = 0;
    int rc = [&]() -> int {
        CK(cudaMalloc(&c->tables, sizeof(CellTables)));
        CK(cudaMalloc(&d_bytes, kFieldElementsPerCell * 48 + 96));
        CK(cudaMemcpyAsync(d_bytes, g1_monomial48, kFieldElementsPerCell * 48, cudaMemcpyHostToDevice, ctx->stream));
        CK(cudaMemcpyAsync(d_bytes + kFieldElementsPerCell * 48, g2_tau64_96, 96, cudaMemcpyHostToDevice, ctx->stream));
        cell_setup_kernel<<<4096 / 128, 128, 0, ctx->stream>>>(c->tables, d_bytes + kFieldElementsPerCell * 48);
        cell_setup_points_kernel<<<kFieldElementsPerCell * 4 / 64, 64, 0, ctx->stream>>>(c->tables, d_bytes);
        cell_setup_lines29_kernel<<<(kMillerSteps * 6 + 127) / 128, 128, 0, ctx->stream>>>(c->tables);
        CK(cudaGetLastError());
        CK(cudaMemcpyAsync(&ok, &c->tables->ok, 4, cudaMemcpyDeviceToHost, ctx->stream));
        CK(cudaStreamSynchronize(ctx->stream));
        CK(cudaFuncSetAttribute(compute_cells_kernel, cudaFuncAttributeMaxDynamicSharedMemorySize, kCellNttSmemBytes));
        CK(cudaMalloc(&c->d_agg, (size_t)kCellsPerExtBlob * kCellAggSlices * kFieldElementsPerCell * sizeof(Fr)));
        CK(cudaMalloc(&c->d_coeffs, (size_t)kCellsPerExtBlob * kFieldElementsPerCell * sizeof(Fr)));
        CK(cudaMalloc(&c->d_part, 2 * sizeof(Partial)));
        CK(cudaEventCreateWithFlags(&c->ev_r, cudaEventDisableTiming));
        CK(cudaEventCreateWithFlags(&c->ev_rli, cudaEventDisableTiming));
        return KZGB200_OK;
    }();
    if (d_bytes) cudaFree(d_bytes);
    if (rc == KZGB200_OK && !ok) rc = KZGB200_INVALID_SETUP;
    if (rc != KZGB200_OK) cell_destroy(ctx);
    return rc;
}

static int cell_capacity(kzgb200_ctx* ctx, size_t n, bool host_inputs, bool device_inputs) {
    CellCtx* c = ctx->cells;
    int rc = ensure_capacity(ctx, n, false);
    if (rc) return rc;
    if (n > c->cap) {
        CK(regrow(c->d_meta, 3 * n + kCellsPerExtBlob + 1)); CK(regrow(c->d_ustatus, n)); CK(regrow(c->d_uc, n * 48));
        CK(regrow(c->d_U, n)); CK(regrow(c->d_rk, n));
        if (c->d_cells) { cudaFree(c->d_cells); c->d_cells = nullptr; }
        if (c->d_p) { cudaFree(c->d_p); c->d_p = nullptr; }
        c->cap = n;
        c->slot.assign(1, 0);
    }
    if (host_inputs && !c->d_cells) { CK(cudaMalloc(&c->d_cells, c->cap * kBytesPerCell)); CK(cudaMalloc(&c->d_p, c->cap * 48)); }
    if (n > c->host_cap) {
        for (void* p : {(void*)c->h_meta, (void*)c->h_uc, (void*)c->h_c, (void*)c->h_cells, (void*)c->h_p, (void*)c->h_idx}) if (p) cudaFreeHost(p);
        c->h_meta = nullptr; c->h_uc = c->h_c = c->h_cells = c->h_p = nullptr; c->h_idx = nullptr;
        CK(cudaMallocHost(&c->h_meta, (3 * n + kCellsPerExtBlob + 1) * 4)); CK(cudaMallocHost(&c->h_uc, n * 48));
        c->host_cap = n;
    }
    if (device_inputs && !c->h_cells) {
        CK(cudaMallocHost(&c->h_c, c->host_cap * 48)); CK(cudaMallocHost(&c->h_cells, c->host_cap * kBytesPerCell));
        CK(cudaMallocHost(&c->h_p, c->host_cap * 48)); CK(cudaMallocHost(&c->h_idx, c->host_cap * 8));
    }
    return KZGB200_OK;
}

static size_t cell_plan(CellCtx* c, const uint8_t* commitments, const uint64_t* idx, size_t n) {
    uint32_t* meta = c->h_meta;
    uint32_t *cidx = meta + n, *order = meta + 2 * n, *start = meta + 3 * n;
    size_t tsize = 1;
    while (tsize < 2 * n) tsize <<= 1;
    if (c->slot.size() < tsize) c->slot.resize(tsize);
    std::fill(c->slot.begin(), c->slot.begin() + tsize, 0u);
    size_t m = 0;
    for (size_t k = 0; k < n; k++) {
        const uint8_t* key = commitments + 48 * k;
        uint64_t h;
        memcpy(&h, key + 8, 8);
        size_t s = (size_t)(h * 0x9e3779b97f4a7c15ull) & (tsize - 1);
        for (;; s = (s + 1) & (tsize - 1)) {
            const uint32_t u = c->slot[s];
            if (!u) { c->slot[s] = (uint32_t)(m + 1); memcpy(c->h_uc + 48 * m, key, 48); cidx[k] = (uint32_t)m++; break; }
            if (!memcmp(c->h_uc + 48 * (u - 1), key, 48)) { cidx[k] = u - 1; break; }
        }
        meta[k] = (uint32_t)idx[k];
    }
    for (int i = 0; i <= kCellsPerExtBlob; i++) start[i] = 0;
    for (size_t k = 0; k < n; k++) start[meta[k] + 1]++;
    for (int i = 0; i < kCellsPerExtBlob; i++) start[i + 1] += start[i];
    std::vector<uint32_t> cur(start, start + kCellsPerExtBlob);
    for (size_t k = 0; k < n; k++) order[cur[meta[k]]++] = (uint32_t)k;
    return m;
}
static void cell_transcript(uint8_t digest[32], const uint8_t* uc, size_t m, const uint32_t* cidx, const uint64_t* idx, const uint8_t* cells,
                            const uint8_t* proofs, size_t n) {
    HostSha256 s;
    host_sha256_init(&s);
    uint8_t hdr[48] = {'R', 'C', 'K', 'Z', 'G', 'C', 'B', 'A', 'T', 'C', 'H', '_', '_', 'V', '1', '_'};
    const uint64_t v[4] = {(uint64_t)kFieldElementsPerBlob, (uint64_t)kFieldElementsPerCell, (uint64_t)m, (uint64_t)n};
    for (int w = 0; w < 4; w++) for (int i = 0; i < 8; i++) hdr[16 + 8 * w + i] = (uint8_t)(v[w] >> (56 - 8 * i));
    host_sha256_update(&s, hdr, 48);
    host_sha256_update(&s, uc, m * 48);
    constexpr size_t kEntry = 16 + kBytesPerCell + 48, kBatch = 16;
    std::vector<uint8_t> buf(kEntry * kBatch);
    for (size_t k = 0; k < n;) {
        size_t cnt = n - k < kBatch ? n - k : kBatch;
        for (size_t e = 0; e < cnt; e++, k++) {
            uint8_t* p = buf.data() + kEntry * e;
            for (int i = 0; i < 8; i++) { p[i] = (uint8_t)((uint64_t)cidx[k] >> (56 - 8 * i)); p[8 + i] = (uint8_t)(idx[k] >> (56 - 8 * i)); }
            memcpy(p + 16, cells + k * kBytesPerCell, kBytesPerCell);
            memcpy(p + 16 + kBytesPerCell, proofs + 48 * k, 48);
        }
        host_sha256_update(&s, buf.data(), kEntry * cnt);
    }
    host_sha256_final(&s, digest);
}

static int cell_verify_locked(kzgb200_ctx* ctx, const uint8_t* hc, const uint64_t* hidx, const uint8_t* hcells, const uint8_t* hp,
                              const uint8_t* d_cells, const uint8_t* d_p, size_t n, int* ok, bool copy_inputs) {
    CellCtx* c = ctx->cells;
    for (size_t k = 0; k < n; k++) if (hidx[k] >= (uint64_t)kCellsPerExtBlob) return KZGB200_BAD_ARGS;
    const size_t m = cell_plan(c, hc, hidx, n);
    uint8_t digest[32];
    std::thread hasher(cell_transcript, digest, c->h_uc, m, c->h_meta + n, hidx, hcells, hp, n);
    const int ni = (int)n, mi = (int)m;
    int rc = [&]() -> int {
        for (int i = 0; i < 8; i++) ctx->ph_started[i] = false;
        CK(cudaStreamWaitEvent(ctx->stream, ctx->ev_parse, 0));
        CK(cudaMemsetAsync(ctx->d_status, 0, n * sizeof(uint32_t), ctx->stream));
        CK(cudaMemsetAsync(c->d_ustatus, 0, m * sizeof(uint32_t), ctx->stream));
        CK(cudaMemcpyAsync(c->d_meta, c->h_meta, (3 * n + kCellsPerExtBlob + 1) * 4, cudaMemcpyHostToDevice, ctx->stream));
        CK(cudaMemcpyAsync(c->d_uc, c->h_uc, m * 48, cudaMemcpyHostToDevice, ctx->stream));
        if (copy_inputs) {
            CK(cudaMemcpyAsync(c->d_p, hp, n * 48, cudaMemcpyHostToDevice, ctx->stream));
            CK(cudaMemcpyAsync(c->d_cells, hcells, n * kBytesPerCell, cudaMemcpyHostToDevice, ctx->stream));
            d_cells = c->d_cells; d_p = c->d_p;
        }
        phase_begin(ctx, kPhParse, ctx->stream);
        cell_points_kernel<<<(mi + 127) / 128, 128, 0, ctx->stream>>>(c->d_uc, mi, c->d_U, c->d_ustatus, kErrCommitment);
        cell_points_kernel<<<(ni + 127) / 128, 128, 0, ctx->stream>>>(d_p, ni, ctx->d_P, ctx->d_status, kErrProof);
        cell_check_kernel<<<(unsigned)(((size_t)n * kFieldElementsPerCell + 255) / 256), 256, 0, ctx->stream>>>(d_cells, ni, ctx->d_status);
        cell_scalars_kernel<<<(ni + 127) / 128, 128, 0, ctx->stream>>>(c->d_meta, ni, c->d_U, c->d_ustatus, c->tables, ctx->d_z_mont, ctx->d_zy,
                                                                        ctx->d_C, ctx->d_status);
        phase_end(ctx, kPhParse, ctx->stream);
        CK(cudaGetLastError());
        return KZGB200_OK;
    }();
    hasher.join();
    if (rc) return rc;
    phase_begin(ctx, kPhTranscript, ctx->stream);
    if ((rc = upload_r_digest(ctx, digest))) return rc;
    phase_end(ctx, kPhTranscript, ctx->stream);
    CK(cudaEventRecord(c->ev_r, ctx->stream));
    CK(cudaStreamWaitEvent(ctx->s_aux, c->ev_r, 0));
    cell_rpow_kernel<<<(ni + 127) / 128, 128, 0, ctx->s_aux>>>(ctx->d_r, ni, c->d_rk);
    cell_agg_kernel<<<dim3(kCellsPerExtBlob, kCellAggSlices), kFieldElementsPerCell, 0, ctx->s_aux>>>(d_cells, c->d_meta, ni, c->d_rk, c->d_agg);
    cell_interp_kernel<<<kCellsPerExtBlob, kFieldElementsPerCell, 0, ctx->s_aux>>>(c->d_agg, c->d_meta, ni, c->tables, c->d_coeffs);
    cell_rli_kernel<<<1, 256, 0, ctx->s_aux>>>(c->d_coeffs, c->tables, c->d_part + 1);
    CK(cudaGetLastError());
    CK(cudaEventRecord(c->ev_rli, ctx->s_aux));
    ctx->cur_c = nullptr; ctx->cur_p = d_p; ctx->cur_n = n; ctx->subgroup_pending = false;
    if ((rc = launch_lincomb(ctx, 0, c->d_part, false))) return rc;
    CK(cudaStreamWaitEvent(ctx->stream, c->ev_rli, 0));
    phase_begin(ctx, kPhFinal, ctx->stream);
    launch_batch_final(ctx->stream, c->d_part, 2, ctx->tables, ctx->d_result, ctx->d_scratch, false, c->tables->lines29);
    phase_end(ctx, kPhFinal, ctx->stream);
    CK(cudaGetLastError());
    rc = read_result(ctx, ok);
    collect_phase_times(ctx);
    return rc;
}

extern "C" int kzgb200_verify_cell_kzg_proof_batch(kzgb200_ctx* ctx, const uint8_t* commitments, const uint64_t* cell_indices, const uint8_t* cells,
                                                   const uint8_t* proofs, size_t n, int* ok) {
    if (!ctx || !ok || (n && (!commitments || !cell_indices || !cells || !proofs)) || n > 0x7fffffff / 2) return KZGB200_BAD_ARGS;
    if (!ctx->cells) return KZGB200_INVALID_SETUP;
    if (n == 0) { *ok = 1; return KZGB200_OK; }
    std::lock_guard<std::mutex> g(ctx->lock);
    DeviceGuard dev(ctx->device);
    int rc = cell_capacity(ctx, n, true, false);
    if (rc) return rc;
    return cell_verify_locked(ctx, commitments, cell_indices, cells, proofs, nullptr, nullptr, n, ok, true);
}

extern "C" int kzgb200_verify_cell_kzg_proof_batch_device(kzgb200_ctx* ctx, const uint8_t* d_commitments, const uint64_t* d_cell_indices,
                                                          const uint8_t* d_cells, const uint8_t* d_proofs, size_t n, int* ok) {
    if (!ctx || !ok || (n && (!d_commitments || !d_cell_indices || !d_cells || !d_proofs)) || n > 0x7fffffff / 2) return KZGB200_BAD_ARGS;
    if (!ctx->cells) return KZGB200_INVALID_SETUP;
    if (n == 0) { *ok = 1; return KZGB200_OK; }
    std::lock_guard<std::mutex> g(ctx->lock);
    DeviceGuard dev(ctx->device);
    int rc = cell_capacity(ctx, n, false, true);
    if (rc) return rc;
    CellCtx* c = ctx->cells;
    CK(cudaStreamWaitEvent(ctx->s_d2h, ctx->ev_parse, 0));
    CK(cudaMemcpyAsync(c->h_idx, d_cell_indices, n * 8, cudaMemcpyDeviceToHost, ctx->s_d2h));
    CK(cudaMemcpyAsync(c->h_c, d_commitments, n * 48, cudaMemcpyDeviceToHost, ctx->s_d2h));
    CK(cudaMemcpyAsync(c->h_p, d_proofs, n * 48, cudaMemcpyDeviceToHost, ctx->s_d2h));
    CK(cudaMemcpyAsync(c->h_cells, d_cells, n * kBytesPerCell, cudaMemcpyDeviceToHost, ctx->s_d2h));
    CK(cudaStreamSynchronize(ctx->s_d2h));
    return cell_verify_locked(ctx, c->h_c, c->h_idx, c->h_cells, c->h_p, d_cells, d_proofs, n, ok, false);
}

static int compute_cells_locked(kzgb200_ctx* ctx, const uint8_t* d_blobs, size_t n, uint8_t* d_out) {
    int rc = ensure_capacity(ctx, n, false);
    if (rc) return rc;
    CK(cudaStreamWaitEvent(ctx->stream, ctx->ev_parse, 0));
    CK(cudaMemsetAsync(ctx->d_status, 0, n * sizeof(uint32_t), ctx->stream));
    compute_cells_kernel<<<(unsigned)n, kCellNttThreads, kCellNttSmemBytes, ctx->stream>>>(d_blobs, (int)n, ctx->cells->tables, d_out, ctx->d_status);
    status_or_kernel<<<1, 256, 0, ctx->stream>>>(ctx->d_status, (int)n, ctx->d_result);
    CK(cudaGetLastError());
    CK(cudaMemcpyAsync(ctx->h_result, ctx->d_result, 4, cudaMemcpyDeviceToHost, ctx->stream));
    CK(cudaStreamSynchronize(ctx->stream));
    return ctx->h_result[0] ? KZGB200_BAD_ARGS : KZGB200_OK;
}
extern "C" int kzgb200_compute_cells(kzgb200_ctx* ctx, const uint8_t* blob, uint8_t* cells_out) {
    if (!ctx || !blob || !cells_out) return KZGB200_BAD_ARGS;
    if (!ctx->cells) return KZGB200_INVALID_SETUP;
    std::lock_guard<std::mutex> g(ctx->lock);
    DeviceGuard dev(ctx->device);
    int rc = ensure_capacity(ctx, 1, true);
    if (rc) return rc;
    CellCtx* c = ctx->cells;
    if (!c->d_ext) CK(cudaMalloc(&c->d_ext, (size_t)kCellsPerExtBlob * kBytesPerCell));
    CK(cudaStreamWaitEvent(ctx->stream, ctx->ev_parse, 0));
    CK(cudaMemcpyAsync(ctx->d_blobs, blob, kBytesPerBlob, cudaMemcpyHostToDevice, ctx->stream));
    if ((rc = compute_cells_locked(ctx, ctx->d_blobs, 1, c->d_ext))) return rc;
    CK(cudaMemcpyAsync(cells_out, c->d_ext, (size_t)kCellsPerExtBlob * kBytesPerCell, cudaMemcpyDeviceToHost, ctx->stream));
    CK(cudaStreamSynchronize(ctx->stream));
    return KZGB200_OK;
}
extern "C" int kzgb200_compute_cells_batch_device(kzgb200_ctx* ctx, const uint8_t* d_blobs, size_t n, uint8_t* d_cells) {
    if (!ctx || (n && (!d_blobs || !d_cells)) || n > 0x7fffffff / 2) return KZGB200_BAD_ARGS;
    if (!ctx->cells) return KZGB200_INVALID_SETUP;
    if (n == 0) return KZGB200_OK;
    std::lock_guard<std::mutex> g(ctx->lock);
    DeviceGuard dev(ctx->device);
    return compute_cells_locked(ctx, d_blobs, n, d_cells);
}

extern "C" int kzgb200_harness_generate_cells(kzgb200_ctx* ctx, uint64_t seed, size_t n_blobs, int degree, const uint8_t* tau_powers48,
                                              uint8_t* d_cells, uint8_t* d_commitments, uint8_t* d_proofs) {
    if (!ctx || n_blobs == 0 || n_blobs > (1u << 20) || degree <= 2 * kFieldElementsPerCell || degree > kCellHarnessMaxDegree || !tau_powers48 ||
        !d_cells || !d_commitments || !d_proofs)
        return KZGB200_BAD_ARGS;
    if (!ctx->cells) return KZGB200_INVALID_SETUP;
    std::lock_guard<std::mutex> g(ctx->lock);
    DeviceGuard dev(ctx->device);
    const int n = (int)n_blobs;
    uint8_t* d_bytes = nullptr; G1Affine* d_M = nullptr; uint32_t* d_bad = nullptr; G1 *d_terms = nullptr, *d_sums = nullptr;
    uint32_t bad = 0;
    int rc = [&]() -> int {
        CK(cudaMalloc(&d_bytes, degree * 48)); CK(cudaMalloc(&d_M, degree * sizeof(G1Affine))); CK(cudaMalloc(&d_bad, 4));
        CK(cudaMalloc(&d_terms, (size_t)n * 6 * 64 * sizeof(G1))); CK(cudaMalloc(&d_sums, (size_t)n * 6 * sizeof(G1)));
        CK(cudaMemsetAsync(d_bad, 0, 4, ctx->stream));
        CK(cudaMemcpyAsync(d_bytes, tau_powers48, degree * 48, cudaMemcpyHostToDevice, ctx->stream));
        harness_parse_points_kernel<<<(degree + 31) / 32, 32, 0, ctx->stream>>>(d_bytes, degree, d_M, d_bad);
        cell_harness_eval_kernel<<<dim3(kCellsPerExtBlob * kFieldElementsPerCell / 128, n), 128, 0, ctx->stream>>>(seed, n, degree, ctx->cells->tables, d_cells);
        cell_harness_terms_kernel<<<(n * 6 * 64 + 127) / 128, 128, 0, ctx->stream>>>(seed, n, degree, d_M, d_terms);
        cell_harness_sums_kernel<<<(n * 6 + 127) / 128, 128, 0, ctx->stream>>>(n, d_terms, d_sums);
        cell_harness_points_kernel<<<(n * (kCellsPerExtBlob + 1) + 127) / 128, 128, 0, ctx->stream>>>(n, d_sums, ctx->cells->tables, d_commitments, d_proofs);
        CK(cudaGetLastError());
        CK(cudaMemcpyAsync(&bad, d_bad, 4, cudaMemcpyDeviceToHost, ctx->stream));
        CK(cudaStreamSynchronize(ctx->stream));
        return KZGB200_OK;
    }();
    for (void* p : {(void*)d_bytes, (void*)d_M, (void*)d_bad, (void*)d_terms, (void*)d_sums}) if (p) cudaFree(p);
    if (rc) return rc;
    return bad ? KZGB200_BAD_ARGS : KZGB200_OK;
}

constexpr size_t kProofChunk = 512;

extern "C" int kzgb200_load_cell_proof_setup(kzgb200_ctx* ctx, const uint8_t* g1_lagrange48, size_t n_points) {
    if (!ctx) return KZGB200_BAD_ARGS;
    if (!g1_lagrange48 || n_points != (size_t)kFieldElementsPerBlob) return KZGB200_INVALID_SETUP;
    std::lock_guard<std::mutex> g(ctx->lock);
    DeviceGuard dev(ctx->device);
    CellCtx* c = ctx->cells;
    if (!c) return KZGB200_INVALID_SETUP;
    if (c->d_fk_tab) return KZGB200_OK;
    uint8_t* d_bytes = nullptr; G1* d_a = nullptr; G1Affine* d_W = nullptr; uint32_t* d_bad = nullptr;
    uint32_t bad = 0;
    int rc = [&]() -> int {
        CK(cudaMalloc(&c->ptables, sizeof(ProofTables)));
        CK(cudaMalloc(&c->d_mono, kFieldElementsPerBlob * sizeof(G1Affine)));
        CK(cudaMalloc(&d_bytes, kFieldElementsPerBlob * 48)); CK(cudaMalloc(&d_a, kFieldElementsPerBlob * sizeof(G1)));
        CK(cudaMalloc(&d_W, kFk20Bases * sizeof(G1Affine))); CK(cudaMalloc(&d_bad, 4));
        CK(cudaMemsetAsync(d_bad, 0, 4, ctx->stream));
        CK(cudaMemcpyAsync(d_bytes, g1_lagrange48, kFieldElementsPerBlob * 48, cudaMemcpyHostToDevice, ctx->stream));
        proof_setup_kernel<<<kExtElements / 128, 128, 0, ctx->stream>>>(c->ptables);
        mono_load_kernel<<<kFieldElementsPerBlob / 128, 128, 0, ctx->stream>>>(d_bytes, d_a, d_bad);
        for (int len = 2; len <= kFieldElementsPerBlob; len <<= 1)
            mono_level_kernel<<<kFieldElementsPerBlob / 2 / 128, 128, 0, ctx->stream>>>(d_a, len, c->tables);
        mono_finish_kernel<<<kFieldElementsPerBlob / 128, 128, 0, ctx->stream>>>(d_a, c->tables, c->d_mono, d_bad);
        CK(cudaGetLastError());
        CK(cudaMemcpyAsync(&bad, d_bad, 4, cudaMemcpyDeviceToHost, ctx->stream));
        CK(cudaStreamSynchronize(ctx->stream));
        if (bad) return KZGB200_INVALID_SETUP;
        CK(cudaMalloc(&c->d_fk_tab, kFk20TablePoints * sizeof(G1Affine)));
        fk20_w_kernel<<<kFieldElementsPerCell, 64, 0, ctx->stream>>>(c->d_mono, c->tables, d_W);
        fk20_table_kernel<<<kFk20Bases * kFk20Windows / 128, 128, 0, ctx->stream>>>(d_W, c->d_fk_tab);
        CK(cudaGetLastError());
        CK(cudaFuncSetAttribute(compute_cells_coeffs_kernel, cudaFuncAttributeMaxDynamicSharedMemorySize, kCellNttSmemBytes));
        CK(cudaFuncSetAttribute(recover_ntt_inv_kernel, cudaFuncAttributeMaxDynamicSharedMemorySize, kCellNttSmemBytes));
        CK(cudaFuncSetAttribute(recover_ntt_div_kernel, cudaFuncAttributeMaxDynamicSharedMemorySize, kCellNttSmemBytes));
        CK(cudaFuncSetAttribute(recover_blob_kernel, cudaFuncAttributeMaxDynamicSharedMemorySize, kCellNttSmemBytes));
        CK(cudaMalloc(&c->d_rin, (size_t)kCellsPerExtBlob * kBytesPerCell)); CK(cudaMalloc(&c->d_pout, (size_t)kCellsPerExtBlob * 48));
        CK(cudaMalloc(&c->d_pos, kCellsPerExtBlob * sizeof(int))); CK(cudaMalloc(&c->d_missing, kCellsPerExtBlob * sizeof(uint32_t)));
        CK(cudaMalloc(&c->d_z, 2 * kCellsPerExtBlob * sizeof(Fr)));
        CK(cudaStreamSynchronize(ctx->stream));
        return KZGB200_OK;
    }();
    for (void* p : {(void*)d_bytes, (void*)d_a, (void*)d_W, (void*)d_bad}) if (p) cudaFree(p);
    if (rc != KZGB200_OK) proof_destroy(c);
    return rc;
}

extern "C" int kzgb200_cell_proof_monomial(kzgb200_ctx* ctx, uint8_t* out48, size_t n_points) {
    if (!ctx || !out48 || n_points > (size_t)kFieldElementsPerBlob) return KZGB200_BAD_ARGS;
    if (!ctx->cells || !ctx->cells->d_fk_tab) return KZGB200_INVALID_SETUP;
    if (n_points == 0) return KZGB200_OK;
    std::lock_guard<std::mutex> g(ctx->lock);
    DeviceGuard dev(ctx->device);
    uint8_t* d_out = nullptr;
    int rc = [&]() -> int {
        CK(cudaMalloc(&d_out, n_points * 48));
        mono_compress_kernel<<<(unsigned)((n_points + 127) / 128), 128, 0, ctx->stream>>>(ctx->cells->d_mono, (int)n_points, d_out);
        CK(cudaGetLastError());
        CK(cudaMemcpyAsync(out48, d_out, n_points * 48, cudaMemcpyDeviceToHost, ctx->stream));
        CK(cudaStreamSynchronize(ctx->stream));
        return KZGB200_OK;
    }();
    if (d_out) cudaFree(d_out);
    return rc;
}

static int proof_workspace(kzgb200_ctx* ctx, size_t n) {
    CellCtx* c = ctx->cells;
    const size_t nb = n < kProofChunk ? n : kProofChunk;
    if (nb <= c->proof_cap) return KZGB200_OK;
    c->proof_cap = 0;
    CK(regrow(c->d_pcoef, nb * kFieldElementsPerBlob)); CK(regrow(c->d_fkU, nb * kFk20Bases)); CK(regrow(c->d_A, nb * kExtElements));
    CK(regrow(c->d_V, nb * kCellsPerExtBlob)); CK(regrow(c->d_rblobs, nb * kBytesPerBlob));
    c->proof_cap = nb;
    return KZGB200_OK;
}
static int fk20_launch(kzgb200_ctx* ctx, const uint8_t* d_blobs, size_t n, uint8_t* d_cells, uint8_t* d_proofs, uint32_t* status) {
    CellCtx* c = ctx->cells;
    cudaStream_t st = ctx->stream;
    for (size_t lo = 0; lo < n; lo += kProofChunk) {
        const int cnt = (int)(n - lo < kProofChunk ? n - lo : kProofChunk);
        phase_begin(ctx, 0, st);
        compute_cells_coeffs_kernel<<<cnt, kCellNttThreads, kCellNttSmemBytes, st>>>(d_blobs + lo * kBytesPerBlob, cnt, c->tables,
                                                                                    d_cells + lo * kCellsPerExtBlob * kBytesPerCell, status + lo, c->d_pcoef);
        phase_end(ctx, 0, st);
        phase_begin(ctx, 1, st);
        fk20_scalars_kernel<<<dim3(kFieldElementsPerCell, cnt), 64, 0, st>>>(c->d_pcoef, c->tables, c->d_fkU);
        fk20_products_kernel<<<dim3(kCellsPerExtBlob, cnt), 64, 0, st>>>(c->d_fkU, c->d_fk_tab, c->d_V);
        phase_end(ctx, 1, st);
        phase_begin(ctx, 2, st);
        fk20_proofs_kernel<<<cnt, 64, 0, st>>>(c->d_V, c->tables, d_proofs + lo * kCellsPerExtBlob * 48);
        phase_end(ctx, 2, st);
    }
    CK(cudaGetLastError());
    return KZGB200_OK;
}
static int proof_begin(kzgb200_ctx* ctx, size_t n) {
    for (int i = 0; i < 8; i++) ctx->ph_started[i] = false;
    int rc = ensure_capacity(ctx, n, false);
    if (!rc) rc = proof_workspace(ctx, n);
    if (rc) return rc;
    CK(cudaStreamWaitEvent(ctx->stream, ctx->ev_parse, 0));
    CK(cudaMemsetAsync(ctx->d_status, 0, n * sizeof(uint32_t), ctx->stream));
    return KZGB200_OK;
}
static int proof_result(kzgb200_ctx* ctx, size_t n) {
    status_or_kernel<<<1, 256, 0, ctx->stream>>>(ctx->d_status, (int)n, ctx->d_result);
    CK(cudaGetLastError());
    CK(cudaMemcpyAsync(ctx->h_result, ctx->d_result, 4, cudaMemcpyDeviceToHost, ctx->stream));
    CK(cudaStreamSynchronize(ctx->stream));
    collect_phase_times(ctx);
    return ctx->h_result[0] ? KZGB200_BAD_ARGS : KZGB200_OK;
}
static bool proof_ready(kzgb200_ctx* ctx) { return ctx->cells && ctx->cells->d_fk_tab; }

extern "C" int kzgb200_compute_cells_and_kzg_proofs(kzgb200_ctx* ctx, const uint8_t* blob, uint8_t* cells_out, uint8_t* proofs_out) {
    if (!ctx || !blob || !cells_out || !proofs_out) return KZGB200_BAD_ARGS;
    if (!proof_ready(ctx)) return KZGB200_INVALID_SETUP;
    std::lock_guard<std::mutex> g(ctx->lock);
    DeviceGuard dev(ctx->device);
    int rc = ensure_capacity(ctx, 1, true);
    if (!rc) rc = proof_begin(ctx, 1);
    if (rc) return rc;
    CellCtx* c = ctx->cells;
    if (!c->d_ext) CK(cudaMalloc(&c->d_ext, (size_t)kCellsPerExtBlob * kBytesPerCell));
    CK(cudaMemcpyAsync(ctx->d_blobs, blob, kBytesPerBlob, cudaMemcpyHostToDevice, ctx->stream));
    if ((rc = fk20_launch(ctx, ctx->d_blobs, 1, c->d_ext, c->d_pout, ctx->d_status))) return rc;
    if ((rc = proof_result(ctx, 1))) return rc;
    CK(cudaMemcpyAsync(cells_out, c->d_ext, (size_t)kCellsPerExtBlob * kBytesPerCell, cudaMemcpyDeviceToHost, ctx->stream));
    CK(cudaMemcpyAsync(proofs_out, c->d_pout, (size_t)kCellsPerExtBlob * 48, cudaMemcpyDeviceToHost, ctx->stream));
    CK(cudaStreamSynchronize(ctx->stream));
    return KZGB200_OK;
}
extern "C" int kzgb200_compute_cells_and_kzg_proofs_batch_device(kzgb200_ctx* ctx, const uint8_t* d_blobs, size_t n, uint8_t* d_cells, uint8_t* d_proofs) {
    if (!ctx || (n && (!d_blobs || !d_cells || !d_proofs)) || n > 0x7fffffff / 2) return KZGB200_BAD_ARGS;
    if (!proof_ready(ctx)) return KZGB200_INVALID_SETUP;
    if (n == 0) return KZGB200_OK;
    std::lock_guard<std::mutex> g(ctx->lock);
    DeviceGuard dev(ctx->device);
    int rc = proof_begin(ctx, n);
    if (!rc) rc = fk20_launch(ctx, d_blobs, n, d_cells, d_proofs, ctx->d_status);
    return rc ? rc : proof_result(ctx, n);
}

static int recover_plan(const uint64_t* idx, size_t n_cells, int* pos, uint32_t* missing, int* n_missing) {
    if (!idx || n_cells < (size_t)kCellsPerExtBlob / 2 || n_cells > (size_t)kCellsPerExtBlob) return KZGB200_BAD_ARGS;
    for (int k = 0; k < kCellsPerExtBlob; k++) pos[k] = -1;
    for (size_t j = 0; j < n_cells; j++) {
        if (idx[j] >= (uint64_t)kCellsPerExtBlob || pos[idx[j]] >= 0) return KZGB200_BAD_ARGS;
        pos[idx[j]] = (int)j;
    }
    *n_missing = 0;
    for (int k = 0; k < kCellsPerExtBlob; k++) if (pos[k] < 0) missing[(*n_missing)++] = (uint32_t)k;
    return KZGB200_OK;
}
static int recover_launch(kzgb200_ctx* ctx, const int* pos, const uint32_t* missing, int n_missing, const uint8_t* d_in, size_t n_cells, size_t nb,
                          uint8_t* d_cells_out, uint8_t* d_proofs_out) {
    CellCtx* c = ctx->cells;
    cudaStream_t st = ctx->stream;
    CK(cudaMemcpyAsync(c->d_pos, pos, kCellsPerExtBlob * sizeof(int), cudaMemcpyHostToDevice, st));
    if (n_missing) CK(cudaMemcpyAsync(c->d_missing, missing, n_missing * sizeof(uint32_t), cudaMemcpyHostToDevice, st));
    recover_z_kernel<<<1, 2 * kCellsPerExtBlob, 0, st>>>(c->d_missing, n_missing, c->tables, c->ptables, c->d_z);
    for (size_t lo = 0; lo < nb; lo += kProofChunk) {
        const int cnt = (int)(nb - lo < kProofChunk ? nb - lo : kProofChunk);
        phase_begin(ctx, 3, st);
        recover_load_kernel<<<(unsigned)((size_t)cnt * kExtElements / 256), 256, 0, st>>>(d_in + lo * n_cells * kBytesPerCell, (int)n_cells, c->d_pos,
                                                                                         c->d_z, cnt, c->d_A, ctx->d_status + lo);
        recover_ntt_inv_kernel<<<dim3(2, cnt), kCellNttThreads, kCellNttSmemBytes, st>>>(c->d_A, c->tables);
        recover_mid_kernel<<<(unsigned)((size_t)cnt * kFieldElementsPerBlob / 256), 256, 0, st>>>(c->d_A, c->ptables, cnt);
        recover_ntt_div_kernel<<<dim3(2, cnt), kCellNttThreads, kCellNttSmemBytes, st>>>(c->d_A, c->tables, c->d_z);
        recover_final_kernel<<<(unsigned)((size_t)cnt * kFieldElementsPerBlob / 256), 256, 0, st>>>(c->d_A, c->ptables, cnt, c->d_pcoef);
        recover_blob_kernel<<<cnt, kCellNttThreads, kCellNttSmemBytes, st>>>(c->d_pcoef, c->tables, c->d_rblobs);
        phase_end(ctx, 3, st);
        CK(cudaGetLastError());
        int rc = fk20_launch(ctx, c->d_rblobs, cnt, d_cells_out + lo * kCellsPerExtBlob * kBytesPerCell, d_proofs_out + lo * kCellsPerExtBlob * 48,
                             ctx->d_status + lo);
        if (rc) return rc;
    }
    return KZGB200_OK;
}
extern "C" int kzgb200_recover_cells_and_kzg_proofs(kzgb200_ctx* ctx, const uint64_t* cell_indices, const uint8_t* cells, size_t n_cells,
                                                    uint8_t* cells_out, uint8_t* proofs_out) {
    if (!ctx || !cells || !cells_out || !proofs_out) return KZGB200_BAD_ARGS;
    if (!proof_ready(ctx)) return KZGB200_INVALID_SETUP;
    int pos[kCellsPerExtBlob], n_missing = 0;
    uint32_t missing[kCellsPerExtBlob];
    int rc = recover_plan(cell_indices, n_cells, pos, missing, &n_missing);
    if (rc) return rc;
    std::lock_guard<std::mutex> g(ctx->lock);
    DeviceGuard dev(ctx->device);
    if ((rc = proof_begin(ctx, 1))) return rc;
    CellCtx* c = ctx->cells;
    if (!c->d_ext) CK(cudaMalloc(&c->d_ext, (size_t)kCellsPerExtBlob * kBytesPerCell));
    CK(cudaMemcpyAsync(c->d_rin, cells, n_cells * kBytesPerCell, cudaMemcpyHostToDevice, ctx->stream));
    if ((rc = recover_launch(ctx, pos, missing, n_missing, c->d_rin, n_cells, 1, c->d_ext, c->d_pout))) return rc;
    if ((rc = proof_result(ctx, 1))) return rc;
    CK(cudaMemcpyAsync(cells_out, c->d_ext, (size_t)kCellsPerExtBlob * kBytesPerCell, cudaMemcpyDeviceToHost, ctx->stream));
    CK(cudaMemcpyAsync(proofs_out, c->d_pout, (size_t)kCellsPerExtBlob * 48, cudaMemcpyDeviceToHost, ctx->stream));
    CK(cudaStreamSynchronize(ctx->stream));
    return KZGB200_OK;
}
extern "C" int kzgb200_recover_cells_and_kzg_proofs_batch_device(kzgb200_ctx* ctx, const uint64_t* cell_indices, size_t n_cells, const uint8_t* d_cells,
                                                                 size_t n_blobs, uint8_t* d_cells_out, uint8_t* d_proofs_out) {
    if (!ctx || (n_blobs && (!d_cells || !d_cells_out || !d_proofs_out)) || n_blobs > 0x7fffffff / 2) return KZGB200_BAD_ARGS;
    if (!proof_ready(ctx)) return KZGB200_INVALID_SETUP;
    int pos[kCellsPerExtBlob], n_missing = 0;
    uint32_t missing[kCellsPerExtBlob];
    int rc = recover_plan(cell_indices, n_cells, pos, missing, &n_missing);
    if (rc || n_blobs == 0) return rc;
    std::lock_guard<std::mutex> g(ctx->lock);
    DeviceGuard dev(ctx->device);
    if ((rc = proof_begin(ctx, n_blobs))) return rc;
    if ((rc = recover_launch(ctx, pos, missing, n_missing, d_cells, n_cells, n_blobs, d_cells_out, d_proofs_out))) return rc;
    return proof_result(ctx, n_blobs);
}
```

kzg_rs_b200/csrc/pipeline.cpp:

```cpp
#include <condition_variable>
#include <cstdint>
#include <deque>
#include <map>
#include <mutex>
#include <new>
#include <set>
#include <thread>
#include <vector>
#include "../../include/kzgb200.h"

namespace {
struct Job {
    uint64_t ticket;
    const uint8_t *blobs, *commitments, *proofs;
    size_t n_blobs, n_commitments, n_proofs;
    uint8_t *z_out, *y_out;
    bool device;
};
struct Done { int rc, ok; };
}

struct kzgb200_pipeline {
    std::vector<kzgb200_ctx*> ctx;
    std::vector<std::thread> workers;
    std::mutex m;
    std::condition_variable cv_job, cv_done;
    std::deque<Job> queue;
    std::map<uint64_t, Done> done;
    std::set<uint64_t> live;
    uint64_t next_ticket = 1;
    size_t in_flight = 0;
    size_t waiters = 0;
    bool stop = false;

    void work(size_t slot) {
        for (;;) {
            Job j;
            {
                std::unique_lock<std::mutex> lk(m);
                cv_job.wait(lk, [&] { return stop || !queue.empty(); });
                if (queue.empty()) return;
                j = queue.front();
                queue.pop_front();
            }
            Done d{KZGB200_INTERNAL_ERROR, 0};
            if (j.device)
                d.rc = kzgb200_verify_blob_kzg_proof_batch_device(ctx[slot], j.blobs, j.commitments, j.proofs, j.n_blobs, &d.ok, j.z_out, j.y_out);
            else
                d.rc = kzgb200_verify_blob_kzg_proof_batch(ctx[slot], j.blobs, j.n_blobs, j.commitments, j.n_commitments, j.proofs, j.n_proofs,
                                                           &d.ok, j.z_out, j.y_out);
            {
                std::lock_guard<std::mutex> lk(m);
                done[j.ticket] = d;
                in_flight--;
            }
            cv_done.notify_all();
        }
    }
};

extern "C" int kzgb200_pipeline_create(kzgb200_pipeline** out, int device, const uint8_t* g2_points, size_t g2_points_len, int depth) {
    if (!out || depth < 1 || depth > 8) return KZGB200_BAD_ARGS;
    *out = nullptr;
    kzgb200_pipeline* p = new (std::nothrow) kzgb200_pipeline();
    if (!p) return KZGB200_INTERNAL_ERROR;
    for (int i = 0; i < depth; i++) {
        kzgb200_ctx* c = nullptr;
        int rc = kzgb200_create(&c, device, g2_points, g2_points_len);
        if (rc == KZGB200_OK && depth > 1) kzgb200_set_slab_tail(c, 0);
        if (rc != KZGB200_OK) {
            for (kzgb200_ctx* x : p->ctx) kzgb200_destroy(x);
            delete p;
            return rc;
        }
        p->ctx.push_back(c);
    }
    for (int i = 0; i < depth; i++) p->workers.emplace_back([p, i] { p->work((size_t)i); });
    *out = p;
    return KZGB200_OK;
}

extern "C" void kzgb200_pipeline_destroy(kzgb200_pipeline* p) {
    if (!p) return;
    {
        std::lock_guard<std::mutex> lk(p->m);
        p->stop = true;
    }
    p->cv_job.notify_all();
    p->cv_done.notify_all();
    for (std::thread& t : p->workers) t.join();
    {
        std::unique_lock<std::mutex> lk(p->m);
        p->cv_done.notify_all();
        p->cv_done.wait(lk, [&] { return p->waiters == 0; });
    }
    for (kzgb200_ctx* c : p->ctx) kzgb200_destroy(c);
    delete p;
}

extern "C" int kzgb200_pipeline_depth(const kzgb200_pipeline* p) { return p ? (int)p->ctx.size() : 0; }

extern "C" kzgb200_ctx* kzgb200_pipeline_context(kzgb200_pipeline* p, int slot) {
    return (p && slot >= 0 && (size_t)slot < p->ctx.size()) ? p->ctx[(size_t)slot] : nullptr;
}

static int submit(kzgb200_pipeline* p, Job j, uint64_t* ticket) {
    if (!p || !ticket) return KZGB200_BAD_ARGS;
    {
        std::unique_lock<std::mutex> lk(p->m);
        if (p->stop) return KZGB200_BAD_ARGS;
        p->waiters++;
        p->cv_done.wait(lk, [&] { return p->stop || p->in_flight < p->ctx.size(); });
        p->waiters--;
        if (p->stop) { p->cv_done.notify_all(); return KZGB200_BAD_ARGS; }
        j.ticket = *ticket = p->next_ticket++;
        p->queue.push_back(j);
        p->live.insert(j.ticket);
        p->in_flight++;
    }
    p->cv_job.notify_one();
    return KZGB200_OK;
}

extern "C" int kzgb200_pipeline_submit(kzgb200_pipeline* p, const uint8_t* blobs, size_t n_blobs, const uint8_t* commitments,
                                       size_t n_commitments, const uint8_t* proofs, size_t n_proofs, uint8_t* z_out, uint8_t* y_out,
                                       uint64_t* ticket) {
    return submit(p, Job{0, blobs, commitments, proofs, n_blobs, n_commitments, n_proofs, z_out, y_out, false}, ticket);
}

extern "C" int kzgb200_pipeline_submit_device(kzgb200_pipeline* p, const uint8_t* d_blobs, const uint8_t* d_commitments,
                                              const uint8_t* d_proofs, size_t n, uint8_t* d_z_out, uint8_t* d_y_out, uint64_t* ticket) {
    return submit(p, Job{0, d_blobs, d_commitments, d_proofs, n, n, n, d_z_out, d_y_out, true}, ticket);
}

extern "C" int kzgb200_pipeline_wait(kzgb200_pipeline* p, uint64_t ticket, int* ok) {
    if (!p || !ok) return KZGB200_BAD_ARGS;
    std::unique_lock<std::mutex> lk(p->m);
    if (!p->live.erase(ticket)) return KZGB200_BAD_ARGS;
    p->waiters++;
    p->cv_done.wait(lk, [&] { return p->done.count(ticket) != 0; });
    Done d = p->done[ticket];
    p->done.erase(ticket);
    p->waiters--;
    if (p->stop) p->cv_done.notify_all();
    *ok = d.ok;
    return d.rc;
}
```

kzg_rs_b200/csrc/runtime.cuh:

```cuda
#pragma once
#include <cuda_runtime.h>
#include <condition_variable>
#include <cstdio>
#include <cstdlib>
#include <cstring>
#include <mutex>
#include <thread>
#include <vector>
#include "../../include/kzgb200.h"
#include "common.cuh"
#include "host_sha256.h"

namespace kzgb200 {

constexpr int kTailSms = 8;
constexpr int kTailHogSmem = 200 * 1024;
constexpr int kTailPadSmem = 28 * 1024;
static_assert(sizeof(FinalSmem) >= (size_t)kTailPadSmem && sizeof(PairSmem) >= (size_t)kTailPadSmem, "the final-check kernels must not fit beside a subgroup-check CTA");
static_assert(sizeof(Partial) == KZGB200_PARTIAL_BYTES, "Partial layout is part of the ABI");
static_assert(sizeof(ZY) == 64, "ZY layout is part of the ABI");

enum Phase { kPhParse = 0, kPhChallenge, kPhEval, kPhTranscript, kPhLincomb, kPhReduce, kPhFinal, kPhCount };
constexpr int kMaxChunks = 64, kWorkStreams = 4;
constexpr size_t kMinChunk = 1024;
struct Chunk { size_t lo, cnt; };

struct CopyPool {
    std::vector<std::thread> threads;
    std::mutex m;
    std::condition_variable cv, cv_done;
    const uint8_t* src = nullptr;
    uint8_t* dst = nullptr;
    size_t bytes = 0, piece = 1 << 20, next = 0, pieces = 0, done = 0;
    uint64_t gen = 0;
    bool stop = false;
    explicit CopyPool(int nthreads);
    ~CopyPool();
    void copy(uint8_t* d, const uint8_t* s, size_t n);
    void work(uint64_t seen);
    bool grab(size_t* off, size_t* len);
};

struct CellCtx {
    CellTables* tables = nullptr;
    size_t cap = 0, blob_cap = 0;
    uint8_t *d_cells = nullptr, *d_p = nullptr, *d_uc = nullptr;
    uint32_t *d_meta = nullptr, *d_ustatus = nullptr;
    G1Affine* d_U = nullptr;
    Fr *d_rk = nullptr, *d_agg = nullptr, *d_coeffs = nullptr;
    Partial* d_part = nullptr;
    uint8_t* d_ext = nullptr;
    size_t host_cap = 0;
    uint32_t* h_meta = nullptr;
    uint8_t *h_uc = nullptr, *h_c = nullptr, *h_cells = nullptr, *h_p = nullptr;
    uint64_t* h_idx = nullptr;
    std::vector<uint32_t> slot;
    cudaEvent_t ev_r = nullptr, ev_rli = nullptr;
    ProofTables* ptables = nullptr;
    G1Affine *d_mono = nullptr, *d_fk_tab = nullptr;
    size_t proof_cap = 0;
    Fr *d_pcoef = nullptr, *d_fkU = nullptr, *d_A = nullptr;
    G1* d_V = nullptr;
    uint8_t* d_rblobs = nullptr;
    uint8_t *d_rin = nullptr, *d_pout = nullptr;
    int* d_pos = nullptr;
    uint32_t* d_missing = nullptr;
    Fr* d_z = nullptr;
};

}

struct kzgb200_ctx {
    int device = 0;
    cudaStream_t stream = nullptr;
    kzgb200::DeviceTables* tables = nullptr;
    size_t cap = 0, blob_cap = 0, many_cap = 0, host_cap = 0;
    uint8_t *d_blobs = nullptr, *d_c = nullptr, *d_p = nullptr;
    kzgb200::Fr* d_z_mont = nullptr;
    kzgb200::Fr* d_zpow = nullptr;
    kzgb200::ZY* d_zy = nullptr;
    kzgb200::G1Affine *d_C = nullptr, *d_P = nullptr;
    uint32_t* d_status = nullptr;
    kzgb200::Fr *d_ry = nullptr, *d_r = nullptr;
    uint8_t* d_digits = nullptr;
    uint32_t *d_order = nullptr, *d_start = nullptr;
    kzgb200::G1 *d_buckets = nullptr, *d_windows = nullptr;
    kzgb200::G1 *d_halfsum = nullptr, *d_part = nullptr;
    kzgb200::Partial* d_partial = nullptr;
    uint32_t* d_result = nullptr;
    uint8_t *d_zout = nullptr, *d_yout = nullptr;
    uint8_t* d_many = nullptr;
    kzgb200::G1* d_lag_table = nullptr;
    kzgb200::Fr* d_scalars = nullptr;
    uint32_t* d_wk = nullptr;
    size_t wk_cap = 0;
    uint32_t* h_result = nullptr;
    uint8_t *h_zy = nullptr, *h_c = nullptr, *h_p = nullptr, *h_digest = nullptr, *h_partial = nullptr;
    uint32_t* d_digest = nullptr;
    const uint8_t *tr_c = nullptr, *tr_p = nullptr;
    kzgb200::HostSha256 tr_sha;
    size_t tr_n = 0, tr_done = 0;
    int tr_next_chunk = 0;
    int tr_enqueued = 0;
    bool tr_active = false;
    void (*chunk_sink)(void*, int) = nullptr;
    void* chunk_sink_arg = nullptr;
    const uint8_t *cur_c = nullptr, *cur_p = nullptr;
    size_t cur_n = 0;
    kzgb200::Chunk chunks[kzgb200::kMaxChunks];
    int nchunks = 0;
    int transcript_mode = KZGB200_TRANSCRIPT_EXACT;
    int num_sms = 148;
    int msm_occ = 3;
    int msm_join = 2;
    int msm_slice = 0;
    int parse_fused = 0;
    int defer_subgroup = 1;
    bool slab_tail = true;
    int sha_stages = 8;
    int pageable_mode = 0;
    bool subgroup_pending = false;
    int parse_first = 0;
    cudaStream_t s_aux = nullptr, s_copy = nullptr, s_d2h = nullptr, s_work[kzgb200::kWorkStreams] = {nullptr, nullptr, nullptr, nullptr};
    cudaEvent_t ev_begin = nullptr, ev_parse = nullptr, ev_decomp = nullptr, ev_bucket = nullptr, ev_sha_all = nullptr, ev_leaf = nullptr;
    cudaEvent_t ev_h2d[kzgb200::kMaxChunks] = {nullptr}, ev_zy[kzgb200::kMaxChunks] = {nullptr}, ev_zyh[kzgb200::kMaxChunks] = {nullptr};
    uint32_t* d_chain_state = nullptr;
    uint8_t* h_flags = nullptr;
    uint8_t* d_scratch = nullptr;
    static constexpr int kStageBufs = 4;
    static constexpr size_t kStageBytes = 32u << 20;
    uint8_t* h_stage[kStageBufs] = {nullptr};
    cudaEvent_t ev_stage[kStageBufs] = {nullptr};
    int stage_next = 0;
    kzgb200::CopyPool* pool = nullptr;
    bool profile = false;
    cudaEvent_t ev_s[8] = {nullptr}, ev_e[8] = {nullptr};
    bool ph_started[8] = {false};
    float phase_ms[8] = {0};
    kzgb200::CellCtx* cells = nullptr;
    std::mutex lock;
    char err[256] = {0};
};

#define CK(expr)                                                                                   \
    do {                                                                                           \
        cudaError_t e_ = (expr);                                                                   \
        if (e_ != cudaSuccess) {                                                                   \
            snprintf(ctx->err, sizeof(ctx->err), "%s: %s (%s:%d)", #expr, cudaGetErrorString(e_), __FILE__, __LINE__); \
            return KZGB200_INTERNAL_ERROR;                                                         \
        }                                                                                          \
    } while (0)

namespace kzgb200 {

struct DeviceGuard {
    int prev = -1;
    explicit DeviceGuard(int device) { if (cudaGetDevice(&prev) != cudaSuccess) prev = -1; cudaSetDevice(device); }
    DeviceGuard() { if (cudaGetDevice(&prev) != cudaSuccess) prev = -1; }
    ~DeviceGuard() { if (prev >= 0) cudaSetDevice(prev); }
};

template <class T>
inline cudaError_t regrow(T*& p, size_t count) {
    if (p) cudaFree(p);
    p = nullptr;
    return cudaMalloc(reinterpret_cast<void**>(&p), count * sizeof(T));
}

int ensure_capacity(kzgb200_ctx* ctx, size_t n, bool need_blob_staging);
int launch_phase1(kzgb200_ctx* ctx, const uint8_t* d_blobs, const uint8_t* h_blobs, const uint8_t* d_c, const uint8_t* d_p, size_t n,
                  bool transcript, bool defer_subgroup, const uint8_t* hc, const uint8_t* hp);
int transcript_progress(kzgb200_ctx* ctx, bool block);
int transcript_finish(kzgb200_ctx* ctx);
int upload_r_digest(kzgb200_ctx* ctx, const uint8_t digest[32]);
int launch_lincomb(kzgb200_ctx* ctx, size_t offset, Partial* d_out, bool wait_subgroup, uint32_t* d_flag = nullptr, uint32_t epoch = 0);
int read_result(kzgb200_ctx* ctx, int* ok);
int export_zy(kzgb200_ctx* ctx, size_t n, uint8_t* d_z, uint8_t* d_y);
void phase_begin(kzgb200_ctx* ctx, int ph, cudaStream_t st);
void phase_end(kzgb200_ctx* ctx, int ph, cudaStream_t st);
void collect_phase_times(kzgb200_ctx* ctx);
void hash_entries(HostSha256* s, const uint8_t* c, const uint8_t* zy, const uint8_t* p, size_t lo, size_t cnt);
void hash_transcript_header(HostSha256* s, uint64_t n);

}
```

Baseline: 1.593 million.

## Pipeline MSM by window groups across streams with incremental combine

Splits the MSM windows into groups (four by default for large batches) and processes them from high to low windows. Each group's bucket join and window reduction run on separate streams, so the single-CTA combine kernel for one group overlaps the bucket work of the next. Combine state (registers, identity flags, fallback, generator sum) is carried between launches through a device buffer. The cost is extra kernel launches and events, plus state round-trips, for a tail-latency reduction; pipelined multi-context mode forces a single group.

```diff
diff --git a/include/kzgb200.h b/include/kzgb200.h
--- a/include/kzgb200.h
+++ b/include/kzgb200.h
@@ -108,6 +108,7 @@
 
 int kzgb200_set_profiling(kzgb200_ctx* ctx, int on);
 int kzgb200_set_slab_tail(kzgb200_ctx* ctx, int on);
+int kzgb200_set_msm_groups(kzgb200_ctx* ctx, int groups);
 int kzgb200_get_phase_ms(kzgb200_ctx* ctx, float* out8);
 int kzgb200_debug_final_ticks(kzgb200_ctx* ctx, long long* out14);
 int kzgb200_debug_engine_selftest(kzgb200_ctx* ctx, uint32_t seed, int rounds, uint32_t* mismatches32, int* n_programs);
diff --git a/kzg_rs_b200/csrc/common.cuh b/kzg_rs_b200/csrc/common.cuh
--- a/kzg_rs_b200/csrc/common.cuh
+++ b/kzg_rs_b200/csrc/common.cuh
@@ -36,6 +36,7 @@
 constexpr int kWinSmemBytes = kWinLanes * 144;
 constexpr int kCombineThreads = 544;
 constexpr int kCombineSmemBytes = 48 * 1024;
+constexpr int kCombineStateBytes = 19 * 1024;
 constexpr int kFinalThreads = 64;
 constexpr int kPairThreads = 768;
 constexpr int kManyThreads = 512, kManyGroups = 28;
@@ -133,12 +134,14 @@
 __global__ void msm_scalars_kernel(const Fr* __restrict__ z_mont, const ZY* __restrict__ zy, const Fr* __restrict__ r_mont, uint64_t offset, int n,
                                    uint8_t* __restrict__ digits, Fr* __restrict__ ry);
 __global__ void msm_sort_kernel(const uint8_t* __restrict__ digits, int n, uint32_t* __restrict__ order, uint32_t* __restrict__ start);
-void launch_msm_bucket(int ctas_per_sm, int n, int slice, cudaStream_t st, const G1Affine* C, const G1Affine* P, const uint32_t* order,
-                       const uint32_t* start, G1* halfsum, G1* part);
-void launch_msm_bucket_join(int lanes, int n, int slice, cudaStream_t st, const uint32_t* start, const G1* halfsum, const G1* part, G1* buckets);
-__global__ void msm_window_kernel(const G1* __restrict__ buckets, G1* __restrict__ windows);
+void launch_msm_bucket(int ctas_per_sm, int n, int slice, int w_lo, int nw, cudaStream_t st, const G1Affine* C, const G1Affine* P,
+                       const uint32_t* order, const uint32_t* start, G1* halfsum, G1* part);
+void launch_msm_bucket_join(int lanes, int n, int slice, int w_lo, int nw, cudaStream_t st, const uint32_t* start, const G1* halfsum,
+                            const G1* part, G1* buckets);
+__global__ void msm_window_kernel(const G1* __restrict__ buckets, G1* __restrict__ windows, int w_lo, int nw);
 __global__ void msm_combine_kernel(const G1* __restrict__ windows, const Fr* __restrict__ ry, const uint32_t* __restrict__ status, int n,
-                                   const DeviceTables* __restrict__ T, Partial* __restrict__ out, uint32_t* flag, uint32_t epoch);
+                                   const DeviceTables* __restrict__ T, Partial* __restrict__ out, uint32_t* flag, uint32_t epoch,
+                                   int w_lo, int w_hi, void* state );
 __global__ void wait_flags_kernel(const uint32_t* flags, int count, uint32_t epoch, uint32_t* __restrict__ timed_out);
 __global__ void batch_final_kernel(const Partial* __restrict__ parts, int nparts, const DeviceTables* __restrict__ T, uint32_t* __restrict__ result,
                                    FinalPts* __restrict__ out);
diff --git a/kzg_rs_b200/csrc/k_msm.cu b/kzg_rs_b200/csrc/k_msm.cu
--- a/kzg_rs_b200/csrc/k_msm.cu
+++ b/kzg_rs_b200/csrc/k_msm.cu
@@ -52,11 +52,13 @@
 template <int kCtasPerSm>
 __global__ void __launch_bounds__(128, kCtasPerSm) msm_bucket_kernel(const G1Affine* __restrict__ C, const G1Affine* __restrict__ P, int n,
                                                          const uint32_t* __restrict__ order, const uint32_t* __restrict__ start,
-                                                         G1* __restrict__ halfsum , G1* __restrict__ part , int slice) {
+                                                         G1* __restrict__ halfsum , G1* __restrict__ part , int slice,
+                                                         int w_lo, int nw) {
     const int slices = (n + slice - 1) / slice;
     int tid = blockIdx.x * blockDim.x + threadIdx.x;
-    if (tid >= kMsmRows * slices) return;
-    int row = tid / slices, s = tid % slices;
+    if (tid >= kMsmSets * 2 * nw * slices) return;
+    const int lr = tid / slices, s = tid % slices;
+    int row = (lr / nw) * kWindows + w_lo + lr % nw;
     int w = row % kWindows, half = (row / kWindows) & 1, set = row / (2 * kWindows);
     const G1Affine* pts = set == 1 ? C : P;
     int digit_row = ((set == 2 ? 1 : 0) * 2 + half) * kWindows + w;
@@ -92,12 +94,12 @@
     }
     flush(b);
 }
-void launch_msm_bucket(int ctas_per_sm, int n, int slice, cudaStream_t st, const G1Affine* C, const G1Affine* P, const uint32_t* order,
-                       const uint32_t* start, G1* halfsum, G1* part) {
-    const int slices = (n + slice - 1) / slice, grid = (kMsmRows * slices + 127) / 128;
-    if (ctas_per_sm >= 4) msm_bucket_kernel<4><<<grid, 128, 0, st>>>(C, P, n, order, start, halfsum, part, slice);
-    else if (ctas_per_sm == 3) msm_bucket_kernel<3><<<grid, 128, 0, st>>>(C, P, n, order, start, halfsum, part, slice);
-    else msm_bucket_kernel<2><<<grid, 128, 0, st>>>(C, P, n, order, start, halfsum, part, slice);
+void launch_msm_bucket(int ctas_per_sm, int n, int slice, int w_lo, int nw, cudaStream_t st, const G1Affine* C, const G1Affine* P,
+                       const uint32_t* order, const uint32_t* start, G1* halfsum, G1* part) {
+    const int slices = (n + slice - 1) / slice, grid = (kMsmSets * 2 * nw * slices + 127) / 128;
+    if (ctas_per_sm >= 4) msm_bucket_kernel<4><<<grid, 128, 0, st>>>(C, P, n, order, start, halfsum, part, slice, w_lo, nw);
+    else if (ctas_per_sm == 3) msm_bucket_kernel<3><<<grid, 128, 0, st>>>(C, P, n, order, start, halfsum, part, slice, w_lo, nw);
+    else msm_bucket_kernel<2><<<grid, 128, 0, st>>>(C, P, n, order, start, halfsum, part, slice, w_lo, nw);
 }
 __device__ __forceinline__ G1 shfl_xor_point(const G1& p, int m) {
     G1 r;
@@ -111,12 +113,13 @@
 }
 template <int kJoinLanes>
 __global__ void __launch_bounds__(128) msm_bucket_join_kernel(int n, const uint32_t* __restrict__ start, const G1* __restrict__ halfsum,
-                                                              const G1* __restrict__ part, G1* __restrict__ buckets , int slice) {
+                                                              const G1* __restrict__ part, G1* __restrict__ buckets , int slice,
+                                                              int w_lo, int nw) {
     const int slices = (n + slice - 1) / slice;
     const uint32_t usl = (uint32_t)slice;
     const int gt = blockIdx.x * blockDim.x + threadIdx.x;
     const int tid = gt / kJoinLanes, j = gt % kJoinLanes;
-    int b = tid % kBuckets, w = (tid / kBuckets) % kWindows, set = tid / (kBuckets * kWindows);
+    int b = tid % kBuckets, w = w_lo + (tid / kBuckets) % nw, set = tid / (kBuckets * nw);
     G1 acc = G1::identity();
     if (b != 0) {
         uint32_t lo[2], s0[2], cnt[2];
@@ -149,19 +152,20 @@
         const G1 o = shfl_xor_point(acc, m);
         if ((j & (2 * m - 1)) == 0) acc = acc.add(o);
     }
-    if (j == 0) buckets[tid] = acc;
-}
-void launch_msm_bucket_join(int lanes, int n, int slice, cudaStream_t st, const uint32_t* start, const G1* halfsum, const G1* part, G1* buckets) {
-    const int items = kMsmSets * kWindows * kBuckets;
-    if (lanes >= 8) msm_bucket_join_kernel<8><<<items * 8 / 128, 128, 0, st>>>(n, start, halfsum, part, buckets, slice);
-    else if (lanes >= 4) msm_bucket_join_kernel<4><<<items * 4 / 128, 128, 0, st>>>(n, start, halfsum, part, buckets, slice);
-    else msm_bucket_join_kernel<2><<<items * 2 / 128, 128, 0, st>>>(n, start, halfsum, part, buckets, slice);
+    if (j == 0) buckets[((size_t)set * kWindows + w) * kBuckets + b] = acc;
+}
+void launch_msm_bucket_join(int lanes, int n, int slice, int w_lo, int nw, cudaStream_t st, const uint32_t* start, const G1* halfsum,
+                            const G1* part, G1* buckets) {
+    const int items = kMsmSets * nw * kBuckets;
+    if (lanes >= 8) msm_bucket_join_kernel<8><<<items * 8 / 128, 128, 0, st>>>(n, start, halfsum, part, buckets, slice, w_lo, nw);
+    else if (lanes >= 4) msm_bucket_join_kernel<4><<<items * 4 / 128, 128, 0, st>>>(n, start, halfsum, part, buckets, slice, w_lo, nw);
+    else msm_bucket_join_kernel<2><<<items * 2 / 128, 128, 0, st>>>(n, start, halfsum, part, buckets, slice, w_lo, nw);
 }
 static_assert(sizeof(G1) * kWinLanes == kWinSmemBytes, "keep kWinSmemBytes (common.cuh) in step with G1");
-__global__ void __launch_bounds__(kWinLanes) msm_window_kernel(const G1* __restrict__ buckets, G1* __restrict__ windows ) {
+__global__ void __launch_bounds__(kWinLanes) msm_window_kernel(const G1* __restrict__ buckets, G1* __restrict__ windows , int w_lo, int nw) {
     extern __shared__ __align__(16) unsigned char dyn_smem[];
     G1* sm = reinterpret_cast<G1*>(dyn_smem);
-    const int l = threadIdx.x, sw = blockIdx.x;
+    const int l = threadIdx.x, sw = (blockIdx.x / nw) * kWindows + w_lo + blockIdx.x % nw;
     G1 mine = buckets[(size_t)sw * kBuckets + l];
 #pragma unroll 1
     for (int d = 1; d < kWinLanes; d <<= 1) {
@@ -188,17 +192,26 @@
     vliw29::SharedTables stab;
 };
 static_assert(sizeof(CombineSmem) <= kCombineSmemBytes, "keep kCombineSmemBytes (common.cuh) in step with CombineSmem");
+struct CombineState {
+    f29::F29 regs[kMsmSets][kCombRegs];
+    uint32_t acc_id[kMsmSets], fallback;
+    G1 sg;
+};
+static_assert(sizeof(CombineState) <= kCombineStateBytes, "keep kCombineStateBytes (common.cuh) in step with CombineState");
 __global__ void __launch_bounds__(kCombineThreads) msm_combine_kernel(const G1* __restrict__ windows, const Fr* __restrict__ ry, const uint32_t* __restrict__ status,
-                                                                      int n, const DeviceTables* __restrict__ T, Partial* __restrict__ out, uint32_t* flag, uint32_t epoch) {
+                                                                      int n, const DeviceTables* __restrict__ T, Partial* __restrict__ out, uint32_t* flag, uint32_t epoch,
+                                                                      int w_lo, int w_hi, void* state_buf) {
     extern __shared__ __align__(16) unsigned char dyn_smem[];
     CombineSmem& S = *reinterpret_cast<CombineSmem*>(dyn_smem);
+    CombineState& state = *reinterpret_cast<CombineState*>(state_buf);
+    const bool first = w_hi == kWindows, last = w_lo == 0;
     __shared__ uint32_t s_err, s_fallback;
     __shared__ uint8_t s_wid[kMsmSets][kWindows];
     __shared__ Fr s_ry[kCombHelpers];
     __shared__ CoopPoint cp[3];
     __shared__ G1 s_sg[64];
     const int t = threadIdx.x;
-    if (t == 0) { s_err = 0; s_fallback = 0; }
+    if (t == 0) { s_err = 0; s_fallback = first ? 0 : state.fallback; }
     __syncthreads();
     if (t < kCombEngine) {
         auto ebar = [] { asm volatile("bar.sync 2, %0;" ::"n"(kCombEngine) : "memory"); };
@@ -211,19 +224,22 @@
             for (int i = t; i < vliw29::kNumPrograms; i += kCombEngine) S.stab.prog[i] = src.prog[i];
             if (t < 16) S.stab.p29[t] = t < 14 ? (int32_t)f29::p29_rt(t) : 0;
         }
-        for (int i = t; i < kMsmSets * kWindows * 3; i += kCombEngine) {
-            const int sw = i / 3, c = i % 3;
-            const G1& w = windows[sw];
-            S.win[sw / kWindows][sw % kWindows][c] = f29::from_fp(c == 0 ? w.x : (c == 1 ? w.y : w.z));
-            if (c == 2) s_wid[sw / kWindows][sw % kWindows] = w.z.is_zero() ? 1 : 0;
-        }
-        for (int i = t; i < kMsmSets * kCombRegs; i += kCombEngine) S.regs[i / kCombRegs][i % kCombRegs] = f29::f29_zero();
+        const int nw = w_hi - w_lo;
+        for (int i = t; i < kMsmSets * nw * 3; i += kCombEngine) {
+            const int g = i / (3 * nw), wi = w_lo + (i / 3) % nw, c = i % 3;
+            const G1& w = windows[g * kWindows + wi];
+            S.win[g][wi][c] = f29::from_fp(c == 0 ? w.x : (c == 1 ? w.y : w.z));
+            if (c == 2) s_wid[g][wi] = w.z.is_zero() ? 1 : 0;
+        }
+        for (int i = t; i < kMsmSets * kCombRegs; i += kCombEngine) S.regs[i / kCombRegs][i % kCombRegs] = first ? f29::f29_zero() : state.regs[i / kCombRegs][i % kCombRegs];
         ebar();
         vliw29::Lanes L{t, kCombEngine, vliw29::Tables{S.stab.mul, S.stab.lin, S.stab.term, S.stab.level, S.stab.prog}, nullptr, S.stab.p29};
         L.groups = kMsmSets; L.gstride = kCombRegs; L.bar_id = 2; L.bar_threads = kCombEngine;
         f29::F29* regs = &S.regs[0][0];
-        bool acc_id[kMsmSets] = {true, true, true};
-        for (int w = kWindows - 1; w >= 0; w--) {
+        bool acc_id[kMsmSets];
+#pragma unroll
+        for (int g = 0; g < kMsmSets; g++) acc_id[g] = first || state.acc_id[g];
+        for (int w = w_hi - 1; w >= w_lo; w--) {
             if (w != kWindows - 1) for (int k = 0; k < 8; k++) vliw29::run(vliw29::kProg_g1_dbl, regs, L);
             for (int i = t; i < kMsmSets * 3 * 4; i += kCombEngine) {
                 const int g = i / 12, c = (i / 4) % 3, q = i % 4;
@@ -244,14 +260,19 @@
             for (int g = 0; g < kMsmSets; g++) acc_id[g] = acc_id[g] && s_wid[g][w];
             ebar();
         }
-        if (t < kMsmSets * 3) {
+        if (!last) {
+            for (int i = t; i < kMsmSets * kCombRegs; i += kCombEngine) state.regs[i / kCombRegs][i % kCombRegs] = S.regs[i / kCombRegs][i % kCombRegs];
+            if (t < kMsmSets) state.acc_id[t] = acc_id[t];
+            if (t == 0) state.fallback = s_fallback;
+        }
+        else if (t < kMsmSets * 3) {
             const int g = t / 3, c = t % 3;
             Fp v = Fp::from_raw(vliw29::canonical_signed(S.regs[g][c]));
             if (acc_id[g]) v = c == 2 ? Fp::zero() : Fp::one();
             cp[g].v[c] = v;
         }
         ebar();
-        if (s_fallback && t < 32 * kMsmSets) {
+        if (last && s_fallback && t < 32 * kMsmSets) {
             const int warp = t >> 5, lane = t & 31;
             CoopPoint* s = &cp[warp];
             __syncwarp();
@@ -264,28 +285,37 @@
         }
     } else {
         const int h = t - kCombEngine;
-        uint32_t e = 0;
-        Fr acc_ry = Fr::zero();
-        for (int i = h; i < n; i += kCombHelpers) { e |= status[i]; acc_ry = acc_ry.add_inl(ry[i]); }
-        if (e) atomicOr(&s_err, e);
-        s_ry[h] = acc_ry;
-        asm volatile("bar.sync 1, %0;" ::"n"(kCombHelpers) : "memory");
-        for (int span = 128; span >= 1; span >>= 1) {
-            if (h < span && h + span < kCombHelpers) s_ry[h] = s_ry[h].add_inl(s_ry[h + span]);
+        if (last) {
+            uint32_t e = 0;
+            for (int i = h; i < n; i += kCombHelpers) e |= status[i];
+            if (e) atomicOr(&s_err, e);
+        }
+        if (first) {
+            Fr acc_ry = Fr::zero();
+            for (int i = h; i < n; i += kCombHelpers) acc_ry = acc_ry.add_inl(ry[i]);
+            s_ry[h] = acc_ry;
             asm volatile("bar.sync 1, %0;" ::"n"(kCombHelpers) : "memory");
-        }
-        if (h < 64) {
-            const Fr sv = s_ry[0];
-            const uint32_t d = (sv.l[h / 8] >> (4 * (h % 8))) & 15u;
-            s_sg[h] = d ? G1::from_affine(T->gen_table[h][d - 1]) : G1::identity();
-        }
-        asm volatile("bar.sync 1, %0;" ::"n"(kCombHelpers) : "memory");
-        for (int span = 32; span >= 1; span >>= 1) {
-            if (h < span) s_sg[h] = s_sg[h].add(s_sg[h + span]);
+            for (int span = 128; span >= 1; span >>= 1) {
+                if (h < span && h + span < kCombHelpers) s_ry[h] = s_ry[h].add_inl(s_ry[h + span]);
+                asm volatile("bar.sync 1, %0;" ::"n"(kCombHelpers) : "memory");
+            }
+            if (h < 64) {
+                const Fr sv = s_ry[0];
+                const uint32_t d = (sv.l[h / 8] >> (4 * (h % 8))) & 15u;
+                s_sg[h] = d ? G1::from_affine(T->gen_table[h][d - 1]) : G1::identity();
+            }
             asm volatile("bar.sync 1, %0;" ::"n"(kCombHelpers) : "memory");
-        }
-    }
-    __syncthreads();
+            for (int span = 32; span >= 1; span >>= 1) {
+                if (h < span) s_sg[h] = s_sg[h].add(s_sg[h + span]);
+                asm volatile("bar.sync 1, %0;" ::"n"(kCombHelpers) : "memory");
+            }
+            if (!last && h == 0) state.sg = s_sg[0];
+        } else if (last && h == 0) {
+            s_sg[0] = state.sg;
+        }
+    }
+    __syncthreads();
+    if (!last) return;
     const int warp = t >> 5, lane = t & 31;
     if (warp == 1) {
         G1 q = {cp[2].v[0], cp[2].v[1], cp[2].v[2]};
diff --git a/kzg_rs_b200/csrc/kzgb200.cu b/kzg_rs_b200/csrc/kzgb200.cu
--- a/kzg_rs_b200/csrc/kzgb200.cu
+++ b/kzg_rs_b200/csrc/kzgb200.cu
@@ -355,31 +355,54 @@
     int slice = (int)((work + waves * wave - 1) / (waves * wave));
     return slice < kMinSlice ? kMinSlice : slice;
 }
+static int msm_groups(const kzgb200_ctx* ctx, int n) {
+    if (ctx->msm_groups > 0) return ctx->msm_groups;
+    return n >= kMsmPipelineMinBlobs ? kMsmDefaultGroups : 1;
+}
 int launch_lincomb(kzgb200_ctx* ctx, size_t offset, Partial* d_out, bool wait_subgroup, uint32_t* d_flag, uint32_t epoch) {
     int n = (int)ctx->cur_n;
+    const int groups = msm_groups(ctx, n), slice = msm_slice_len(ctx, n);
+    int bound[kWindows + 1] = {0};
+    for (int g = 1; g <= groups; g++) bound[g] = groups == 1 ? kWindows : 1 + (kWindows - 1) * (g - 1) / (groups - 1);
+    const bool pipe = groups > 1;
+    cudaStream_t s_comb = pipe ? ctx->s_comb : ctx->stream;
     phase_begin(ctx, kPhLincomb, ctx->stream);
     msm_scalars_kernel<<<(n + 127) / 128, 128, 0, ctx->stream>>>(ctx->d_z_mont, ctx->d_zy, ctx->d_r, (uint64_t)offset, n, ctx->d_digits, ctx->d_ry);
     msm_sort_kernel<<<kDigitRows, 256, 0, ctx->stream>>>(ctx->d_digits, n, ctx->d_order, ctx->d_start);
-    {
-        const int slice = msm_slice_len(ctx, n);
-        launch_msm_bucket(ctx->msm_occ, n, slice, ctx->stream, ctx->d_C, ctx->d_P, ctx->d_order, ctx->d_start, ctx->d_halfsum, ctx->d_part);
-        launch_msm_bucket_join(ctx->msm_join, n, slice, ctx->stream, ctx->d_start, ctx->d_halfsum, ctx->d_part, ctx->d_buckets);
-    }
-    phase_end(ctx, kPhLincomb, ctx->stream);
-    phase_begin(ctx, kPhReduce, ctx->stream);
-    msm_window_kernel<<<kMsmSets * kWindows, kWinLanes, kWinSmemBytes, ctx->stream>>>(ctx->d_buckets, ctx->d_windows);
-    if (ctx->subgroup_pending) {
-        CK(cudaEventRecord(ctx->ev_bucket, ctx->stream));
-        CK(cudaStreamWaitEvent(ctx->s_aux, ctx->ev_bucket, 0));
-        if (ctx->profile) cudaEventRecord(ctx->ev_s[7], ctx->s_aux);
-        g1_subgroup_kernel<<<ctx->num_sms - kTailSms, 256, kTailHogSmem, ctx->s_aux>>>(ctx->d_C, ctx->d_P, n, ctx->d_status);
-        if (ctx->profile) { cudaEventRecord(ctx->ev_e[7], ctx->s_aux); ctx->ph_started[7] = true; }
-        CK(cudaEventRecord(ctx->ev_parse, ctx->s_aux));
-        ctx->subgroup_pending = false;
-    }
-    if (wait_subgroup) CK(cudaStreamWaitEvent(ctx->stream, ctx->ev_parse, 0));
-    msm_combine_kernel<<<1, kCombineThreads, kCombineSmemBytes, ctx->stream>>>(ctx->d_windows, ctx->d_ry, ctx->d_status, n, ctx->tables, d_out, d_flag, epoch);
-    phase_end(ctx, kPhReduce, ctx->stream);
+    for (int g = groups - 1; g >= 0; g--) {
+        const int w_lo = bound[g], nw = bound[g + 1] - bound[g];
+        cudaStream_t sw = pipe ? ctx->s_msm[g % kMsmStreams] : ctx->stream;
+        launch_msm_bucket(ctx->msm_occ, n, slice, w_lo, nw, ctx->stream, ctx->d_C, ctx->d_P, ctx->d_order, ctx->d_start, ctx->d_halfsum, ctx->d_part);
+        if (pipe) {
+            CK(cudaEventRecord(ctx->ev_msm_bk[g], ctx->stream));
+            CK(cudaStreamWaitEvent(sw, ctx->ev_msm_bk[g], 0));
+        }
+        launch_msm_bucket_join(ctx->msm_join, n, slice, w_lo, nw, sw, ctx->d_start, ctx->d_halfsum, ctx->d_part, ctx->d_buckets);
+        msm_window_kernel<<<kMsmSets * nw, kWinLanes, kWinSmemBytes, sw>>>(ctx->d_buckets, ctx->d_windows, w_lo, nw);
+        if (g == 0) phase_end(ctx, kPhLincomb, sw);
+        if (pipe) {
+            CK(cudaEventRecord(ctx->ev_msm_win[g], sw));
+            CK(cudaStreamWaitEvent(s_comb, ctx->ev_msm_win[g], 0));
+        }
+        if (g == 0 && ctx->subgroup_pending) {
+            CK(cudaEventRecord(ctx->ev_bucket, sw));
+            CK(cudaStreamWaitEvent(ctx->s_aux, ctx->ev_bucket, 0));
+            if (ctx->profile) cudaEventRecord(ctx->ev_s[7], ctx->s_aux);
+            g1_subgroup_kernel<<<ctx->num_sms - kTailSms, 256, kTailHogSmem, ctx->s_aux>>>(ctx->d_C, ctx->d_P, n, ctx->d_status);
+            if (ctx->profile) { cudaEventRecord(ctx->ev_e[7], ctx->s_aux); ctx->ph_started[7] = true; }
+            CK(cudaEventRecord(ctx->ev_parse, ctx->s_aux));
+            ctx->subgroup_pending = false;
+        }
+        if (g == 0 && wait_subgroup) CK(cudaStreamWaitEvent(s_comb, ctx->ev_parse, 0));
+        phase_begin(ctx, kPhReduce, s_comb);
+        msm_combine_kernel<<<1, kCombineThreads, kCombineSmemBytes, s_comb>>>(ctx->d_windows, ctx->d_ry, ctx->d_status, n, ctx->tables, d_out, d_flag, epoch,
+                                                                            w_lo, w_lo + nw, ctx->d_comb_state);
+    }
+    phase_end(ctx, kPhReduce, s_comb);
+    if (pipe) {
+        CK(cudaEventRecord(ctx->ev_comb, s_comb));
+        CK(cudaStreamWaitEvent(ctx->stream, ctx->ev_comb, 0));
+    }
     CK(cudaGetLastError());
     return KZGB200_OK;
 }
@@ -422,12 +445,19 @@
         if (const char* v = getenv("KZGB200_PAGEABLE")) ctx->pageable_mode = !strcmp(v, "direct") ? 1 : (!strcmp(v, "register") ? 2 : 0);
         if (const char* v = getenv("KZGB200_MSM_SLICE")) ctx->msm_slice = atoi(v);
         if (const char* v = getenv("KZGB200_MSM_JOIN")) ctx->msm_join = atoi(v);
+        if (const char* v = getenv("KZGB200_MSM_GROUPS")) { int g = atoi(v); if (g >= 1 && g <= kWindows) ctx->msm_groups = g; }
         if (const char* v = getenv("KZGB200_MSM_OCC")) { int o = atoi(v); if (o >= 2 && o <= 4) ctx->msm_occ = o; }
         if (const char* v = getenv("KZGB200_TRANSCRIPT")) ctx->transcript_mode = !strcmp(v, "tree") ? KZGB200_TRANSCRIPT_TREE : (!strcmp(v, "device") ? KZGB200_TRANSCRIPT_EXACT_DEVICE : KZGB200_TRANSCRIPT_EXACT);
         CK(cudaFuncSetAttribute(g1_subgroup_kernel, cudaFuncAttributeMaxDynamicSharedMemorySize, kTailHogSmem));
         CK(cudaStreamCreateWithFlags(&ctx->s_copy, cudaStreamNonBlocking));
         CK(cudaStreamCreateWithPriority(&ctx->s_d2h, cudaStreamNonBlocking, prio_hi));
         for (auto& w : ctx->s_work) CK(cudaStreamCreateWithPriority(&w, cudaStreamNonBlocking, prio_hi));
+        for (auto& w : ctx->s_msm) CK(cudaStreamCreateWithPriority(&w, cudaStreamNonBlocking, prio_hi));
+        CK(cudaStreamCreateWithPriority(&ctx->s_comb, cudaStreamNonBlocking, prio_hi));
+        for (auto& e : ctx->ev_msm_bk) CK(cudaEventCreateWithFlags(&e, cudaEventDisableTiming));
+        for (auto& e : ctx->ev_msm_win) CK(cudaEventCreateWithFlags(&e, cudaEventDisableTiming));
+        CK(cudaEventCreateWithFlags(&ctx->ev_comb, cudaEventDisableTiming));
+        CK(cudaMalloc(&ctx->d_comb_state, kCombineStateBytes));
         for (cudaEvent_t* e : {&ctx->ev_begin, &ctx->ev_parse, &ctx->ev_decomp, &ctx->ev_bucket, &ctx->ev_sha_all, &ctx->ev_leaf})
             CK(cudaEventCreateWithFlags(e, cudaEventDisableTiming));
         for (auto& e : ctx->ev_h2d) CK(cudaEventCreateWithFlags(&e, cudaEventDisableTiming));
@@ -479,7 +509,11 @@
     cudaDeviceSynchronize();
     cell_destroy(ctx);
     delete ctx->pool;
-    for (cudaStream_t st : {ctx->s_aux, ctx->s_copy, ctx->s_d2h, ctx->s_work[0], ctx->s_work[1], ctx->s_work[2], ctx->s_work[3]}) if (st) cudaStreamDestroy(st);
+    for (cudaStream_t st : {ctx->s_aux, ctx->s_copy, ctx->s_d2h, ctx->s_work[0], ctx->s_work[1], ctx->s_work[2], ctx->s_work[3], ctx->s_comb}) if (st) cudaStreamDestroy(st);
+    for (cudaStream_t st : ctx->s_msm) if (st) cudaStreamDestroy(st);
+    for (auto e : ctx->ev_msm_bk) if (e) cudaEventDestroy(e);
+    for (auto e : ctx->ev_msm_win) if (e) cudaEventDestroy(e);
+    if (ctx->ev_comb) cudaEventDestroy(ctx->ev_comb);
     for (cudaEvent_t e : {ctx->ev_begin, ctx->ev_parse, ctx->ev_decomp, ctx->ev_bucket, ctx->ev_sha_all, ctx->ev_leaf}) if (e) cudaEventDestroy(e);
     for (auto e : ctx->ev_h2d) if (e) cudaEventDestroy(e);
     for (auto e : ctx->ev_zy) if (e) cudaEventDestroy(e);
@@ -490,7 +524,7 @@
     void* ptrs[] = {ctx->tables, ctx->d_blobs, ctx->d_c, ctx->d_p, ctx->d_z_mont, ctx->d_zy, ctx->d_C, ctx->d_P, ctx->d_status,
                     ctx->d_ry, ctx->d_r, ctx->d_partial, ctx->d_result, ctx->d_zout, ctx->d_yout, ctx->d_many, ctx->d_wk,
                     ctx->d_digits, ctx->d_order, ctx->d_start, ctx->d_buckets, ctx->d_halfsum, ctx->d_part, ctx->d_windows, ctx->d_lag_table, ctx->d_scalars, ctx->d_zpow,
-                    ctx->d_chain_state, ctx->d_scratch, ctx->d_digest};
+                    ctx->d_chain_state, ctx->d_scratch, ctx->d_digest, ctx->d_comb_state};
     for (void* p : ptrs) if (p) cudaFree(p);
     void* hptrs[] = {ctx->h_flags, ctx->h_result, ctx->h_digest, ctx->h_partial, ctx->h_zy, ctx->h_c, ctx->h_p, ctx->h_stage[0], ctx->h_stage[1], ctx->h_stage[2], ctx->h_stage[3]};
     for (void* p : hptrs) if (p) cudaFreeHost(p);
@@ -885,6 +919,12 @@
     if (!ctx) return KZGB200_BAD_ARGS;
     std::lock_guard<std::mutex> g(ctx->lock);
     ctx->slab_tail = on != 0;
+    return KZGB200_OK;
+}
+extern "C" int kzgb200_set_msm_groups(kzgb200_ctx* ctx, int groups) {
+    if (!ctx || groups < 0 || groups > kWindows) return KZGB200_BAD_ARGS;
+    std::lock_guard<std::mutex> g(ctx->lock);
+    ctx->msm_groups = groups;
     return KZGB200_OK;
 }
 extern "C" int kzgb200_debug_engine_selftest(kzgb200_ctx* ctx, uint32_t seed, int rounds, uint32_t* mismatches32, int* n_programs) {
diff --git a/kzg_rs_b200/csrc/pipeline.cpp b/kzg_rs_b200/csrc/pipeline.cpp
--- a/kzg_rs_b200/csrc/pipeline.cpp
+++ b/kzg_rs_b200/csrc/pipeline.cpp
@@ -68,6 +68,7 @@
         kzgb200_ctx* c = nullptr;
         int rc = kzgb200_create(&c, device, g2_points, g2_points_len);
         if (rc == KZGB200_OK && depth > 1) kzgb200_set_slab_tail(c, 0);
+        if (rc == KZGB200_OK && depth > 1) kzgb200_set_msm_groups(c, 1);
         if (rc != KZGB200_OK) {
             for (kzgb200_ctx* x : p->ctx) kzgb200_destroy(x);
             delete p;
diff --git a/kzg_rs_b200/csrc/runtime.cuh b/kzg_rs_b200/csrc/runtime.cuh
--- a/kzg_rs_b200/csrc/runtime.cuh
+++ b/kzg_rs_b200/csrc/runtime.cuh
@@ -22,6 +22,7 @@
 
 enum Phase { kPhParse = 0, kPhChallenge, kPhEval, kPhTranscript, kPhLincomb, kPhReduce, kPhFinal, kPhCount };
 constexpr int kMaxChunks = 64, kWorkStreams = 4;
+constexpr int kMsmDefaultGroups = 4, kMsmPipelineMinBlobs = 8192, kMsmStreams = 4;
 constexpr size_t kMinChunk = 1024;
 struct Chunk { size_t lo, cnt; };
 
@@ -114,6 +115,7 @@
     int msm_occ = 3;
     int msm_join = 2;
     int msm_slice = 0;
+    int msm_groups = 0;
     int parse_fused = 0;
     int defer_subgroup = 1;
     bool slab_tail = true;
@@ -124,6 +126,9 @@
     cudaStream_t s_aux = nullptr, s_copy = nullptr, s_d2h = nullptr, s_work[kzgb200::kWorkStreams] = {nullptr, nullptr, nullptr, nullptr};
     cudaEvent_t ev_begin = nullptr, ev_parse = nullptr, ev_decomp = nullptr, ev_bucket = nullptr, ev_sha_all = nullptr, ev_leaf = nullptr;
     cudaEvent_t ev_h2d[kzgb200::kMaxChunks] = {nullptr}, ev_zy[kzgb200::kMaxChunks] = {nullptr}, ev_zyh[kzgb200::kMaxChunks] = {nullptr};
+    cudaStream_t s_msm[kzgb200::kMsmStreams] = {nullptr, nullptr, nullptr, nullptr}, s_comb = nullptr;
+    cudaEvent_t ev_msm_bk[kzgb200::kWindows] = {nullptr}, ev_msm_win[kzgb200::kWindows] = {nullptr}, ev_comb = nullptr;
+    void* d_comb_state = nullptr;
     uint32_t* d_chain_state = nullptr;
     uint8_t* h_flags = nullptr;
     uint8_t* d_scratch = nullptr;
```

Measured after the change: 1.615 million (median of 6 runs). 1.4% higher.
